# leavesnight/VIEO_SLAM

Measured on AMD Instinct MI355X. Metric: frontend+localBA frames/sec on EuRoC MH05 stereo-VIO; ATE vs ref, higher is better.
Workload: dtype u8 (extract/match) + f64 (pose optimisation)

## Files before the change

include/vieo_hot.h:

```cpp
#ifndef VIEO_HOT_H
#define VIEO_HOT_H

#include <stddef.h>
#include <stdint.h>

#ifdef __cplusplus
extern "C" {
#endif

#define VIEO_OK 0
#define VIEO_E_INVALID (-1)
#define VIEO_E_NO_DEVICE (-2)
#define VIEO_E_HIP (-3)
#define VIEO_E_CAPACITY (-4)
#define VIEO_E_EMPTY (-5)

const char* vieo_last_error(void);
int vieo_device_available(void);
int vieo_set_device(int device);
int vieo_get_device(void);
const char* vieo_version(void);

int vieo_dev_malloc(void** d_ptr, size_t bytes);
int vieo_dev_free(void* d_ptr);
// ... 191 lines not shown
  float Xw[3];
  int32_t octave;
  float angle;
  int32_t flags;
  int32_t reserved[2];
  uint8_t desc[32];
} vieo_last_frame_point;

typedef struct vieo_sbp_camera {
  double Tcw_cur[12], Tcw_last[12];
  float fx, fy, cx, cy;
  float bounds[4];
  float bf, baseline;
  float th, th_far;
  int32_t mono, nlevels;
  float scale[16];
} vieo_sbp_camera;

#define VIEO_SBP_LAST_FRAME 0
#define VIEO_SBP_LOCAL_MAP 1
#define VIEO_SBP_RELOC 2
#define VIEO_SBP_UNCHANGED (-1)
#define VIEO_SBP_ERASED (-2)

int vieo_sbp_project_last_frame(const vieo_last_frame_point* h_points, int n,
                                const vieo_sbp_camera* h_cam, vieo_proj_query* h_queries);
int vieo_search_by_projection(int mode, const vieo_proj_query* h_queries, int nq,
                              const vieo_keypoint* h_keys, const float* h_uright,
                              const uint8_t* h_desc, const uint8_t* h_taken, int n_keys,
                              const float* h_bounds , float nn_ratio, int check_orientation,
                              int32_t* h_assign, int32_t* nmatches);
int vieo_search_by_projection_batch_device(int mode, const vieo_proj_query* d_queries,
                                           const int32_t* d_nq, int q_cap, int n_frames,
                                           const vieo_keypoint* d_keys, const float* d_uright,
                                           const uint8_t* d_desc, const uint8_t* d_taken,
                                           const int32_t* d_counts, int key_cap, int img_first,
                                           int img_step, const float* h_bounds, float nn_ratio,
                                           int check_orientation, int32_t* d_assign,
                                           int32_t* d_nmatches, void* stream);
int vieo_sbp_project_last_frame_batch_device(const vieo_last_frame_point* d_points,
                                             const int32_t* d_n, int p_cap, int n_frames,
                                             const vieo_sbp_camera* d_cams,
                                             vieo_proj_query* d_queries, void* stream);

typedef struct vieo_sbp_rig {
  int32_t n_cams;
  int32_t use_distort;
  vieo_camera cams[4];
  double Tcr[4][12];
  double trc[4][3];
  float bounds[4][4];
} vieo_sbp_rig;

typedef struct vieo_keyframe_point {
  float Xw[3];
  int32_t octave;
  float angle;
  int32_t flags;
  float max_distance, min_distance;
  uint8_t desc[32];
} vieo_keyframe_point;

int vieo_sbp_project_last_frame_rig(const vieo_last_frame_point* h_points, int n, const vieo_sbp_camera* h_cam,
                                    const vieo_sbp_rig* h_rig, vieo_proj_query* h_queries );
int vieo_sbp_project_keyframe(const vieo_keyframe_point* h_points, int n, const vieo_sbp_camera* h_cam,
                              const vieo_sbp_rig* h_rig, float log_scale_factor,
                              vieo_proj_query* h_queries );
int vieo_search_by_projection_rig(int mode, const vieo_proj_query* h_queries, int nq, const vieo_keypoint* h_keys,
                                  const float* h_uright, const uint8_t* h_desc, const uint8_t* h_taken, int n_keys,
                                  const int32_t* h_cam_first , const float* h_bounds, int n_cams,
                                  float nn_ratio, int check_orientation, int32_t* h_assign, int32_t* nmatches);
int vieo_sbp_project_last_frame_rig_batch_device(const vieo_last_frame_point* d_points, const int32_t* d_n,
                                                 int p_cap, int n_frames, const vieo_sbp_camera* d_cams,
                                                 const vieo_sbp_rig* d_rigs, int n_cams,
                                                 vieo_proj_query* d_queries ,
                                                 void* stream);
int vieo_search_by_projection_rig_batch_device(int mode, const vieo_proj_query* d_queries, const int32_t* d_nq,
                                               int q_cap, int n_frames, const vieo_keypoint* d_keys,
                                               const float* d_uright, const uint8_t* d_desc,
                                               const uint8_t* d_taken, const int32_t* d_cam_first, int key_cap,
                                               const float* h_bounds, int n_cams, float nn_ratio,
                                               int check_orientation, int32_t* d_assign, int32_t* d_nmatches,
                                               void* stream);

int vieo_sbp_keep_grid(int on);

int vieo_orb_holds(const vieo_orb* e, const vieo_keypoint* h_keys, int n_keys);
int vieo_orb_resident_keys(const vieo_orb* e);
int vieo_stereo_match_rectified_resident(vieo_orb* left, vieo_orb* right, float baseline, float bf,
                                         float* h_uright, float* h_depth);
int vieo_search_by_projection_last_frame_resident(vieo_orb* frame, const vieo_last_frame_point* h_points, int n_points,
                                                  const vieo_sbp_camera* h_cam, const float* h_uright, float nn_ratio,
                                                  int check_orientation, int32_t* h_assign, int32_t* nmatches);
int vieo_search_by_projection_resident(int mode, vieo_orb* frame, const vieo_proj_query* h_queries, int nq,
                                       const float* h_uright, const uint8_t* h_taken, const float* h_bounds ,
                                       float nn_ratio, int check_orientation, int32_t* h_assign, int32_t* nmatches);


typedef struct vieo_navstate {
  double p[3];
  double q[4];
  double v[3];
  double bg[3], ba[3], dbg[3], dba[3];
} vieo_navstate;


typedef struct vieo_pose_obs {
  float Xw[3];
  float u, v, ur;
  float inv_sigma2;
  int32_t flags;
} vieo_pose_obs;

typedef struct vieo_enc_preint {
  double dt;
  double delx[6];
  double Sigma[36];
} vieo_enc_preint;
typedef struct vieo_pose_enc {
  vieo_enc_preint enc;
  double qRbe[4], pbe[3];
  double p_last[3], q_last[4];
} vieo_pose_enc;

typedef struct vieo_pose_frame {
  vieo_navstate nav;
  double Rcb[9], tcb[3];
  float fx, fy, cx, cy;
  float bf;
  int32_t obs_begin;
  int32_t n_obs;
  int32_t n_cams;
  const vieo_camera* cams;
  const vieo_pose_enc* enc;
} vieo_pose_frame;

#define VIEO_POSE_CAMS_AUTO 0
#define VIEO_POSE_CAMS_RECTIFIED 1
#define VIEO_POSE_CAMS_RIG 2
int vieo_pose_set_camera_mode(int mode);
#define VIEO_POSE_ENC_AUTO 0
#define VIEO_POSE_ENC_NONE 1
#define VIEO_POSE_ENC_ALL 2
int vieo_pose_set_encoder_mode(int mode);

#define VIEO_POSE_OK 0
#define VIEO_POSE_TOO_FEW 1
typedef struct vieo_pose_result {
  vieo_navstate nav;
  int32_t n_inliers;
  int32_t status;
  int32_t lm_iterations;
  int32_t reserved;
} vieo_pose_result;

int vieo_pose_optimization(const vieo_pose_frame* h_frame, const vieo_pose_obs* h_obs,
                           uint8_t* h_outlier, vieo_pose_result* h_result);
int vieo_pose_optimization_batch_device(const vieo_pose_frame* d_frames, int n_frames,
                                        const vieo_pose_obs* d_obs, uint8_t* d_outlier,
                                        vieo_pose_result* d_results, void* stream);

typedef struct vieo_imu_preint {
  double dt;
  double Rij[9];
  double vij[3], pij[3];
  double JgR[9], Jgv[9], Jav[9], Jgp[9], Jap[9];
// ... 218 lines not shown
                                            const void* d_frames, const void* d_results, int frames_are_vio, int key_cap,
                                            int n_frames, void* d_next_frames, uint8_t* d_taken, const int32_t* d_counts,
                                            int img_first, int img_step, uint8_t* d_held, int p_cap, void* stream);
int vieo_track_merge_build_obs_batch_device(const int32_t* d_assign, int32_t* d_mp_ref, int point_offset, int reset, int query_div,
                                            const vieo_last_frame_point* d_same_point, const int32_t* d_query_src, int q_cap,
                                            const float* d_point_xyz, const float* d_point_depth, float close_depth, int p_cap,
                                            const vieo_keypoint* d_keys, const float* d_uright, const int32_t* d_counts,
                                            const int32_t* d_cam_first, int n_cams, int key_cap, int n_frames, int img_first,
                                            int img_step, const float* d_inv_sigma2, vieo_pose_obs* d_obs, int32_t* d_obs_key,
                                            void* d_frames, int frames_are_vio, void* stream);
int vieo_track_build_obs_depth_batch_device(const int32_t* d_mp_ref, const float* d_point_xyz,
                                            const float* d_point_depth, float close_depth, int p_cap,
                                            const vieo_keypoint* d_keys, const float* d_uright,
                                            const int32_t* d_counts, int key_cap, int n_frames,
                                            int img_first, int img_step, const float* d_inv_sigma2,
                                            vieo_pose_obs* d_obs, int32_t* d_obs_key, void* d_frames,
                                            int frames_are_vio, void* stream);
int vieo_track_merge_assign_rig_batch_device(const int32_t* d_assign, int32_t* d_mp_ref, const int32_t* d_counts,
                                             int key_cap, int n_frames, int img_first, int img_step, int point_offset,
                                             int reset, int query_div,
                                             const vieo_last_frame_point* d_same_point ,
                                             const int32_t* d_query_src , int q_cap, void* stream);
int vieo_track_compact_queries_batch_device(const vieo_proj_query* d_queries, const int32_t* d_nq, int q_cap, int n_frames,
                                            vieo_proj_query* d_queries_out, int32_t* d_src, int32_t* d_nq_out, void* stream);
int vieo_track_build_obs_rig_batch_device(const int32_t* d_mp_ref, const float* d_point_xyz,
                                          const float* d_point_depth, float close_depth, int p_cap,
                                          const vieo_keypoint* d_keys, const float* d_uright,
                                          const int32_t* d_counts, const int32_t* d_cam_first, int n_cams, int key_cap,
                                          int n_frames, const float* d_inv_sigma2, vieo_pose_obs* d_obs,
                                          int32_t* d_obs_key, void* d_frames, int frames_are_vio, void* stream);
int vieo_track_mark_held_batch_device(const int32_t* d_mp_ref, const int32_t* d_counts, int key_cap,
                                      int n_frames, int img_first, int img_step, uint8_t* d_held, int p_cap,
                                      void* stream);
void* vieo_orb_stream(vieo_orb* e);

int vieo_orb_tap_plane(vieo_orb* e, int image_index, int level, int which, uint8_t* h_dst,
                       int dst_stride);
int vieo_orb_tap_candidates(vieo_orb* e, int image_index, int level, int32_t* h_dst, int cap);
int vieo_orb_tap_level_keys(vieo_orb* e, int image_index, int level, vieo_keypoint* h_dst,
                            int cap);


typedef struct vieo_frustum_frame {
  float Rcrw[9], tcrw[3];
  float Ow[3];
  int32_t n_cams;
  int32_t use_distort;
  const struct vieo_camera* cams;
  float Tcr[4][12];
  float trc[4][3];
  float bounds[4][4];
  float bf;
  float log_scale_factor;
  int32_t n_levels;
  float viewing_cos_limit;
} vieo_frustum_frame;

typedef struct vieo_frustum_point {
  float Xw[3], normal[3];
  float max_distance, min_distance;
} vieo_frustum_point;

typedef struct vieo_track_info {
  float u[4], v[4], ur[4], viewcos[4];
  int32_t level[4], cam[4];
  int32_t n;
  float track_depth;
} vieo_track_info;

int vieo_is_in_frustum_batch(const vieo_frustum_frame* h_frame, const vieo_frustum_point* h_points, int n_points,
                             vieo_track_info* h_info);
int vieo_track_local_queries_device(const vieo_frustum_frame* h_frame, const vieo_vio_frame* d_frame,
                                    const vieo_vio_result* d_result, const vieo_frustum_point* d_points,
                                    const uint8_t* d_desc, const int32_t* d_alias, const uint8_t* d_held, int held_cap,
                                    int n_points, float th, float th_far, const float* d_scale, vieo_proj_query* d_queries,
                                    float* d_track_depth, int32_t* d_nq, void* stream);

int vieo_track_local_queries_batch_device(const vieo_frustum_frame* h_frame, const vieo_vio_frame* d_frames,
                                          const vieo_vio_result* d_results, int n_frames, const vieo_frustum_point* d_points,
                                          const uint8_t* d_desc, const int32_t* d_alias, const int32_t* d_counts, int p_cap,
                                          const uint8_t* d_held, int held_cap, float th, float th_far, const float* d_scale,
                                          vieo_proj_query* d_queries, float* d_track_depth, size_t depth_stride,
                                          int32_t* d_nq, void* stream);
int vieo_track_local_queries_slot_batch_device(const vieo_frustum_frame* h_frame, const void* d_frames, size_t frame_stride,
                                               const void* d_results, size_t result_stride, int n_frames,
                                               const int32_t* d_pos_slot, const vieo_frustum_point* d_points,
                                               const uint8_t* d_desc, const int32_t* d_alias, const int32_t* d_counts,
                                               int p_cap, const uint8_t* d_held, int held_cap, float th, float th_far,
                                               const float* d_scale, vieo_proj_query* d_queries, float* d_track_depth,
                                               size_t depth_stride, int32_t* d_nq, void* stream);

int vieo_distinctive_descriptors_batch(const uint8_t* h_descriptors, const int32_t* h_first, int n_points,
                                       int32_t* h_best);

int vieo_update_normal_and_depth_batch(const float* h_points , const int32_t* h_first,
                                       const int32_t* h_obs_centre, const float* h_centres, int n_centres,
                                       const int32_t* h_ref_centre, const float* h_ref_scale,
                                       float scale_last_level, int n_points, float* h_normal ,
                                       float* h_max_distance, float* h_min_distance);

typedef struct vieo_fuse_frame {
  vieo_frustum_frame base;
  float scale_factors[16];
  float inv_level_sigma2[16];
  float th_radius;
  int32_t check_viewing_angle;
  int32_t use_bf;
  int32_t reserved;
} vieo_fuse_frame;

typedef struct vieo_fuse_point {
  float Xw[3], normal[3];
  float max_distance, min_distance;
  uint8_t desc[32];
  int32_t skip_mask;
  int32_t reserved;
} vieo_fuse_point;

int vieo_fuse_search(const vieo_fuse_frame* h_frame, const vieo_keypoint* const* h_keys ,
                     const float* const* h_uright ,
                     const uint8_t* const* h_descriptors , const int32_t* n_keys ,
                     const vieo_fuse_point* h_points, int n_points, int32_t* h_best_idx ,
                     int32_t* h_best_dist );

#define VIEO_PREINT_OK 0
#define VIEO_PREINT_EMPTY 1
#define VIEO_PREINT_GAP 2
#define VIEO_PREINT_UNSUPPORTED 3
typedef struct vieo_imu_sample {
  double t;
  double w[3], a[3];
} vieo_imu_sample;
typedef struct vieo_imu_noise {
  double sigma_g[9], sigma_a[9];
  double freq_ref;
  int32_t dt_cov_noise_fixed;
  int32_t reserved;
} vieo_imu_noise;
int vieo_imu_preintegrate_batch(const vieo_imu_noise* noise, const vieo_imu_sample* h_samples,
                                const int32_t* h_first, const double* h_ti, const double* h_tj,
                                const double* h_bg , const double* h_ba , int n,
                                vieo_imu_preint* h_out, double* h_sigma_prv ,
                                int32_t* h_status);

int vieo_imu_preintegrate_batch_device(const vieo_imu_noise* d_noise, const vieo_imu_sample* d_samples,
                                       const int32_t* d_first, const double* d_ti, const double* d_tj,
                                       const double* d_bg, const double* d_ba, int n, vieo_imu_preint* d_out,
                                       double* d_sigma_prv, int32_t* d_status, void* stream);

int vieo_imu_preintegrate_batch_ex(const vieo_imu_noise* noise, const vieo_imu_sample* h_samples,
                                   const int32_t* h_first, const double* h_ti, const double* h_tj,
                                   const double* h_bg , const double* h_ba , int n,
                                   const vieo_imu_preint* h_seed ,
                                   const double* h_seed_sigma_prv , const int32_t* h_breset ,
                                   vieo_imu_preint* h_out, double* h_sigma_prv ,
                                   int32_t* h_status);
int vieo_imu_preintegrate_batch_device_ex(const vieo_imu_noise* d_noise, const vieo_imu_sample* d_samples,
                                          const int32_t* d_first, const double* d_ti, const double* d_tj,
                                          const double* d_bg, const double* d_ba, int n,
                                          const vieo_imu_preint* d_seed, const double* d_seed_sigma_prv,
                                          const int32_t* d_breset, vieo_imu_preint* d_out, double* d_sigma_prv,
                                          int32_t* d_status, void* stream);

typedef struct vieo_tracker vieo_tracker;
typedef struct vieo_tracker_params {
  int32_t width, height;
// ... 354 lines not shown
```

vieo_slam_amd/_lib.py:

```python
import ctypes
import os

_HERE = os.path.dirname(os.path.abspath(__file__))
LIB_PATH = os.environ.get("VIEO_LIB_PATH") or os.path.join(_HERE, "libvieo_hot.so")

VIEO_OK = 0
VIEO_E_INVALID, VIEO_E_NO_DEVICE, VIEO_E_HIP, VIEO_E_CAPACITY, VIEO_E_EMPTY = -1, -2, -3, -4, -5

c_p = ctypes.c_void_p
c_i = ctypes.c_int
c_f = ctypes.c_float
c_sz = ctypes.c_size_t
P = ctypes.POINTER

_SIGS = {
    "vieo_last_error": (ctypes.c_char_p, []),
    "vieo_device_available": (c_i, []),
    "vieo_set_device": (c_i, [c_i]),
    "vieo_pose_set_camera_mode": (c_i, [c_i]),
    "vieo_pose_set_replicas": (c_i, [c_i]),
    "vieo_search_for_triangulation": (c_i, [c_p, c_p, c_i, c_i, c_i, c_i, c_i, c_p, c_p, c_p]),
    "vieo_pose_set_encoder_mode": (c_i, [c_i]),
    "vieo_triangulate_new_points": (c_i, [c_p, c_p, c_p, c_p, c_i, c_f, c_i, c_i, c_p, c_p, c_p, c_p, c_p, c_p]),
    "vieo_create_new_map_points": (c_i, [c_p, c_p, c_p, c_p, c_i, c_i, c_i, c_f, c_i, c_i, c_p, c_p, c_p, c_p, c_p, c_p, c_p]),
    "vieo_is_in_frustum_batch": (c_i, [c_p, c_p, c_i, c_p]),
    "vieo_imu_preintegrate_batch": (c_i, [c_p, c_p, c_p, c_p, c_p, c_p, c_p, c_i, c_p, c_p, c_p]),
    "vieo_imu_preintegrate_batch_ex": (c_i, [c_p] * 7 + [c_i] + [c_p] * 6),
    "vieo_fuse_search": (c_i, [c_p, c_p, c_p, c_p, c_p, c_p, c_i, c_p, c_p]),
    "vieo_distinctive_descriptors_batch": (c_i, [c_p, c_p, c_i, c_p]),
    "vieo_update_normal_and_depth_batch": (c_i, [c_p, c_p, c_p, c_p, c_i, c_p, c_p, ctypes.c_float, c_i, c_p, c_p,
                                                 c_p]),
    "vieo_bundle_adjustment": (c_i, [c_p, c_i, c_i, c_p, c_i, c_p, c_i, c_p, c_i, c_p, c_p, c_p, c_p]),
    "vieo_bundle_adjustment_enc": (c_i, [c_p, c_i, c_i, c_p, c_i, c_p, c_i, c_p, c_i, c_p, c_p, c_p, c_p, c_p]),
    "vieo_local_bundle_adjustment_batch_enc": (c_i, [c_i, c_p, c_p, c_p, c_p, c_p, c_p, c_p, c_p, c_p, c_p, c_p, c_p,
                                                      c_p]),
    "vieo_local_bundle_adjustment_enc": (c_i, [c_p, c_p, c_i, c_p, c_i, c_p, c_i, c_p, c_p, c_p, c_p, c_p, c_p]),
    "vieo_global_bundle_adjustment_vio": (c_i, [c_p, c_i, c_i, c_p, c_i, c_p, c_i, c_p, c_i, c_p, c_i, c_p, c_p, c_p,
                                                c_p]),
    "vieo_global_bundle_adjustment_vio_scale": (c_i, [c_p, c_i, c_i, c_i, c_p, c_i, c_p, c_i, c_p, c_i, c_p, c_i, c_p, c_p,
                                                      c_p, c_p, c_p]),
    "vieo_global_bundle_adjustment_vio_sharded_scale": (c_i, [c_p, c_i, c_i, c_i, c_p, c_i, c_p, c_i, c_p, c_i, c_p, c_i,
                                                              c_p, ctypes.c_size_t, c_p, c_p, c_p, c_p, c_p, c_p]),
    "vieo_track_local_queries_batch_device": (c_i, [c_p, c_p, c_p, c_i, c_p, c_p, c_p, c_p, c_i, c_p, c_i, c_f, c_f, c_p, c_p,
                                                    c_p, c_sz, c_p, c_p]),
    "vieo_pose_optimization_vio_batch_device_ex": (c_i, [c_p, c_i, c_p, c_p, c_p, c_i, c_i, c_p]),
    "vieo_pose_optimization_batch_device_ex": (c_i, [c_p, c_i, c_p, c_p, c_p, c_i, c_p]),
    "vieo_get_device": (c_i, []),
    "vieo_version": (ctypes.c_char_p, []),
    "vieo_dev_malloc": (c_i, [P(c_p), c_sz]),
    "vieo_dev_free": (c_i, [c_p]),
    "vieo_memcpy_h2d": (c_i, [c_p, c_p, c_sz]),
    "vieo_memcpy_d2h": (c_i, [c_p, c_p, c_sz]),
    "vieo_device_synchronize": (c_i, []),
    "vieo_stream_create": (c_i, [P(c_p)]),
    "vieo_stream_destroy": (c_i, [c_p]),
    "vieo_stream_synchronize": (c_i, [c_p]),
    "vieo_stream_wait_event": (c_i, [c_p, c_p]),
    "vieo_host_alloc_pinned": (c_i, [P(c_p), c_sz]),
    "vieo_host_free_pinned": (c_i, [c_p]),
    "vieo_memcpy_h2d_async": (c_i, [c_p, c_p, c_sz, c_p]),
    "vieo_memcpy_d2h_async": (c_i, [c_p, c_p, c_sz, c_p]),
    "vieo_event_create": (c_i, [P(c_p)]),
    "vieo_event_destroy": (c_i, [c_p]),
    "vieo_event_record": (c_i, [c_p, c_p]),
    "vieo_event_elapsed_ms": (c_i, [c_p, c_p, P(c_f)]),
    "vieo_orb_create": (c_i, [P(c_p), c_i, c_f, c_i, c_i, c_i]),
    "vieo_orb_destroy": (None, [c_p]),
    "vieo_orb_levels": (c_i, [c_p]),
    "vieo_orb_scale_factor": (c_f, [c_p]),
    "vieo_orb_scale_factors": (c_i, [c_p, c_p]),
    "vieo_orb_inv_scale_factors": (c_i, [c_p, c_p]),
    "vieo_orb_level_sigma2": (c_i, [c_p, c_p]),
    "vieo_orb_inv_level_sigma2": (c_i, [c_p, c_p]),
    "vieo_orb_features_per_level": (c_i, [c_p, c_p]),
    "vieo_orb_max_keypoints": (c_i, [c_p]),
    "vieo_orb_extract": (c_i, [c_p, c_p, c_i, c_i, c_i, c_p, c_p, c_p, c_i, P(c_i), P(c_i)]),
    "vieo_orb_extract_batch_device": (c_i, [c_p, c_p, c_i, c_i, c_i, c_i, c_sz, c_p, c_p, c_p, c_i, c_p]),
    "vieo_orb_sync": (c_i, [c_p]),
    "vieo_orb_level_size": (c_i, [c_p, c_i, P(c_i), P(c_i)]),
    "vieo_orb_get_level": (c_i, [c_p, c_i, c_i, c_i, c_p, c_i]),
    "vieo_orb_level_device": (c_i, [c_p, c_i, c_i, P(c_p), P(c_i)]),
    "vieo_orb_last_stage_ms": (c_i, [c_p, c_p]),
    "vieo_orb_enable_timing": (c_i, [c_p, c_i]),
    "vieo_orb_timed_steps": (c_i, [c_p]),
    "vieo_orb_stage_ms": (c_i, [c_p, c_i, c_p]),
    "vieo_hamming_knn2": (c_i, [c_p, c_i, c_p, c_i, c_p, c_p]),
    "vieo_stereo_fisheye_match": (c_i, [c_p, c_p, c_p, c_p, c_p, c_i, c_p, c_p, c_p, c_p, c_p, c_p, c_p]),
    "vieo_hamming_knn2_rig_batch_device": (c_i, [c_p, c_p, c_i, c_i, c_i, c_p, c_p, c_p]),
    "vieo_fisheye_create": (c_i, [P(c_p), c_p, c_i, c_i]),
    "vieo_fisheye_destroy": (None, [c_p]),
    "vieo_fisheye_group_capacity": (c_i, [c_p]),
    "vieo_stereo_fisheye_match_batch_device": (c_i, [c_p, c_p, c_p, c_p, c_i] + [c_p] * 12),
    "vieo_stereo_fisheye_match_batch_device_part": (c_i, [c_p, c_p, c_p, c_p, c_i] + [c_p] * 11 + [c_i, c_p]),
    "vieo_track_merge_assign_rig_batch_device": (c_i, [c_p, c_p, c_p, c_i, c_i, c_i, c_i, c_i, c_i, c_i, c_p, c_p, c_i, c_p]),
    "vieo_track_compact_queries_batch_device": (c_i, [c_p, c_p, c_i, c_i, c_p, c_p, c_p, c_p]),
    "vieo_track_build_obs_rig_batch_device": (c_i, [c_p, c_p, c_p, c_f, c_i, c_p, c_p, c_p, c_p, c_i, c_i, c_i, c_p, c_p, c_p,
                                                     c_p, c_i, c_p]),
    "vieo_fisheye_last_walk": (None, [c_p, c_p]),
    "vieo_hamming_knn2_batch_device": (c_i, [c_p, c_p, c_i, c_p, c_i, c_p, c_p, c_p]),
    "vieo_stereo_match_rectified": (c_i, [c_p, c_p, c_p, c_p, c_i, c_p, c_p, c_i, c_f, c_f, c_p, c_p]),
    "vieo_stereo_match_rectified_batch_device": (c_i, [c_p, c_i, c_p, c_p, c_p, c_i, c_f, c_f, c_p, c_p]),
    "vieo_sbp_project_last_frame": (c_i, [c_p, c_i, c_p, c_p]),
    "vieo_sbp_project_last_frame_rig": (c_i, [c_p, c_i, c_p, c_p, c_p]),
    "vieo_sbp_project_keyframe": (c_i, [c_p, c_i, c_p, c_p, c_f, c_p]),
    "vieo_search_by_projection_rig": (c_i, [c_i, c_p, c_i, c_p, c_p, c_p, c_p, c_i, c_p, c_p, c_i, c_f, c_i, c_p, c_p]),
    "vieo_sbp_keep_grid": (c_i, [c_i]),
    "vieo_orb_holds": (c_i, [c_p, c_p, c_i]),
    "vieo_orb_resident_keys": (c_i, [c_p]),
    "vieo_stereo_match_rectified_resident": (c_i, [c_p, c_p, c_f, c_f, c_p, c_p]),
    "vieo_search_by_projection_last_frame_resident": (c_i, [c_p, c_p, c_i, c_p, c_p, c_f, c_i, c_p, c_p]),
    "vieo_search_by_projection_resident": (c_i, [c_i, c_p, c_p, c_i, c_p, c_p, c_p, c_f, c_i, c_p, c_p]),
    "vieo_sbp_project_last_frame_rig_batch_device": (c_i, [c_p, c_p, c_i, c_i, c_p, c_p, c_i, c_p, c_p]),
    "vieo_search_by_projection_rig_batch_device": (c_i, [c_i, c_p, c_p, c_i, c_i, c_p, c_p, c_p, c_p, c_p, c_i, c_p, c_i,
                                                          c_f, c_i, c_p, c_p, c_p]),
    "vieo_search_by_projection": (c_i, [c_i, c_p, c_i, c_p, c_p, c_p, c_p, c_i, c_p, c_f, c_i, c_p, c_p]),
    "vieo_search_by_projection_batch_device": (c_i, [c_i, c_p, c_p, c_i, c_i, c_p, c_p, c_p, c_p, c_p, c_i, c_i, c_i, c_p, c_f, c_i, c_p, c_p, c_p]),
    "vieo_sbp_project_last_frame_batch_device": (c_i, [c_p, c_p, c_i, c_i, c_p, c_p, c_p]),
    "vieo_pose_optimization": (c_i, [c_p, c_p, c_p, c_p]),
    "vieo_pose_optimization_batch_device": (c_i, [c_p, c_i, c_p, c_p, c_p, c_p]),
    "vieo_pose_optimization_vio": (c_i, [c_p, c_p, c_p, c_p]),
    "vieo_pose_optimization_vio_batch_device": (c_i, [c_p, c_i, c_p, c_p, c_p, c_p]),
    "vieo_track_merge_assign_batch_device": (c_i, [c_p, c_p, c_p, c_i, c_i, c_i, c_i, c_i, c_i, c_p]),
    "vieo_track_build_obs_batch_device": (c_i, [c_p, c_p, c_i, c_p, c_p, c_p, c_i, c_i, c_i, c_i, c_p, c_p, c_p, c_p, c_i, c_p]),
    "vieo_track_after_pose_batch_device": (c_i, [c_p, c_p, c_p, c_p, c_p, c_i, c_i, c_i, c_p, c_p, c_p]),
    "vieo_track_build_obs_depth_batch_device": (c_i, [c_p, c_p, c_p, c_f, c_i, c_p, c_p, c_p, c_i, c_i, c_i, c_i, c_p, c_p, c_p,
                                                       c_p, c_i, c_p]),
    "vieo_track_mark_held_batch_device": (c_i, [c_p, c_p, c_i, c_i, c_i, c_i, c_p, c_i, c_p]),
    "vieo_track_after_pose_held_batch_device": (c_i, [c_p, c_p, c_p, c_p, c_p, c_i, c_i, c_i, c_p, c_p, c_p, c_i, c_i, c_p, c_i, c_p]),
    "vieo_track_merge_build_obs_batch_device": (c_i, [c_p, c_p, c_i, c_i, c_i, c_p, c_p, c_i, c_p, c_p, c_f, c_i, c_p, c_p, c_p, c_p, c_i,
                                                       c_i, c_i, c_i, c_i, c_p, c_p, c_p, c_p, c_i, c_p]),
    "vieo_track_local_queries_device": (c_i, [c_p, c_p, c_p, c_p, c_p, c_p, c_p, c_i, c_i, c_f, c_f, c_p, c_p, c_p, c_p, c_p]),
    "vieo_orb_stream": (c_p, [c_p]),
    "vieo_local_bundle_adjustment": (c_i, [c_p, c_p, c_i, c_p, c_i, c_p, c_i, c_p, c_p, c_p, c_p, c_p]),
    "vieo_local_bundle_adjustment_batch": (c_i, [c_i, c_p, c_p, c_p, c_p, c_p, c_p, c_p, c_p, c_p, c_p, c_p,
                                                  c_p]),
    "vieo_local_bundle_adjustment_vio": (c_i, [c_p, c_p, c_i, c_p, c_p, c_i, c_p, c_i, c_p, c_i, c_p, c_p, c_p,
                                                c_p, c_p]),
    "vieo_local_bundle_adjustment_vio_batch": (c_i, [c_i] + [c_p] * 15),
    "vieo_lba_sharded_buffer_doubles": (ctypes.c_size_t, [c_i, c_p]),
    "vieo_lba_enable_timing": (None, [c_i]),
    "vieo_lba_set_stream_priority": (c_i, [c_i]),
    "vieo_lba_kernel_classes": (c_i, []),
    "vieo_lba_kernel_class_name": (ctypes.c_char_p, [c_i]),
    "vieo_lba_kernel_times": (None, [c_p, c_p, c_p]),
    "vieo_lba_sparse_stats": (None, [c_p]),
    "vieo_rccl_available": (c_i, []),
    "vieo_rccl_unique_id": (c_i, [c_p]),
    "vieo_rccl_comm_create": (c_i, [P(c_p), c_p, c_i, c_i]),
    "vieo_rccl_comm_destroy": (c_i, [c_p]),
    "vieo_global_bundle_adjustment_vio_sharded": (c_i, [c_p, c_i, c_i, c_p, c_i, c_p, c_i, c_p, c_i, c_p, c_i, c_p,
                                                        ctypes.c_size_t, c_p, c_p, c_p, c_p, c_p]),
    "vieo_local_bundle_adjustment_vio_sharded": (c_i, [c_i] + [c_p] * 10 + [c_p, ctypes.c_size_t, c_p, c_p] +
                                                 [c_p] * 4),
    "vieo_local_bundle_adjustment_vio_sharded_stop": (c_i, [c_i] + [c_p] * 10 + [c_p, ctypes.c_size_t, c_p, c_p, c_p] +
                                                      [c_p] * 4),
    "vieo_orb_tap_plane": (c_i, [c_p, c_i, c_i, c_i, c_p, c_i]),
    "vieo_orb_tap_candidates": (c_i, [c_p, c_i, c_i, c_p, c_i]),
    "vieo_orb_tap_level_keys": (c_i, [c_p, c_i, c_i, c_p, c_i]),
    "vieo_imu_preintegrate_batch_device": (c_i, [c_p] * 7 + [c_i] + [c_p] * 4),
    "vieo_imu_preintegrate_batch_device_ex": (c_i, [c_p] * 7 + [c_i] + [c_p] * 7),
    "vieo_tracker_create": (c_i, [P(c_p), c_p]),
    "vieo_tracker_create_rig": (c_i, [P(c_p), c_p, c_p]),
    "vieo_tracker_key_capacity": (c_i, [c_p]),
    "vieo_tracker_group_capacity": (c_i, [c_p]),
    "vieo_tracker_image_buffer": (c_i, [c_p, c_i, P(c_p)]),
    "vieo_tracker_destroy": (None, [c_p]),
    "vieo_tracker_image_buffers": (c_i, [c_p, P(c_p), P(c_p)]),
    "vieo_tracker_scale_factors": (c_i, [c_p, c_p]),
    "vieo_track_frame": (c_i, [c_p, c_p, c_p]),
    "vieo_tracker_get_stats": (c_i, [c_p, c_p]),
    "vieo_tracker_reprobe": (c_i, [c_p]),
    "vieo_tracker_get_level": (c_i, [c_p, c_i, c_i, c_i, c_p, c_i]),
    "vieo_tracker_multi_create": (c_i, [P(c_p), c_p, c_i]),
    "vieo_tracker_multi_destroy": (None, [c_p]),
    "vieo_tracker_multi_image_buffer": (c_i, [c_p, c_i, c_i, P(c_p)]),
    "vieo_tracker_multi_reset_slot": (c_i, [c_p, c_i]),
    "vieo_track_frames": (c_i, [c_p, c_i, c_p, c_p, c_p]),
    "vieo_track_local_queries_slot_batch_device": (c_i, [c_p, c_p, c_sz, c_p, c_sz, c_i, c_p, c_p, c_p, c_p, c_p, c_i, c_p, c_i,
                                                         c_f, c_f, c_p, c_p, c_p, c_sz, c_p, c_p]),
    "vieo_search_by_bow": (c_i, [c_p, c_p, c_i, c_f, c_i, c_p, c_p]),
    "vieo_relocalize": (c_i, [c_p, c_p, c_i, c_p, c_i, ctypes.c_uint64, c_p, c_p, c_p, c_p, c_i]),
    "vieo_pnp_create": (c_i, [P(c_p), c_p, c_i, c_p, c_p, c_i, ctypes.c_uint64]),
    "vieo_pnp_destroy": (None, [c_p]),
    "vieo_pnp_get_info": (c_i, [c_p, c_i, c_p]),
    "vieo_pnp_iterate": (c_i, [c_p, c_i, c_i, c_p, c_p, c_p, c_p, c_p, c_p]),
    "vieo_pnp_tap_rows": (c_i, [c_p, c_i, c_p, c_p, c_p, c_p]),
    "vieo_pnp_tap_records": (c_i, [c_p, c_i, c_p, c_p, c_p, c_p]),
    "vieo_pnp_tap_refine": (c_i, [c_p, c_p, c_p, c_i, c_p, c_p, c_p]),
    "vieo_vocabulary_create": (c_i, [P(c_p), c_i, c_i, c_i, c_i, c_p, c_i]),
    "vieo_vocabulary_load": (c_i, [P(c_p), ctypes.c_char_p]),
    "vieo_vocabulary_info": (c_i, [c_p, c_p]),
    "vieo_vocabulary_destroy": (None, [c_p]),
    "vieo_bow_transform": (c_i, [c_p, c_p, c_i, c_i, c_p]),
    "vieo_kfdb_create": (c_i, [P(c_p), c_p]),
    "vieo_kfdb_destroy": (None, [c_p]),
    "vieo_kfdb_clear": (c_i, [c_p]),
    "vieo_kfdb_size": (c_i, [c_p]),
    "vieo_kfdb_add": (c_i, [c_p, ctypes.c_int64, c_p, c_p, c_i]),
    "vieo_kfdb_erase": (c_i, [c_p, ctypes.c_int64]),
    "vieo_kfdb_set_covisible": (c_i, [c_p, ctypes.c_int64, c_p, c_i]),
# ... 80 lines not shown
```

vieo_slam_amd/csrc/mappoint.hip:

```cpp
#include <climits>

#include "ba_device.h"

namespace vieo {

struct FrustumDev {
  vieo_frustum_frame F;
  CamD cams[4];
};

__device__ __forceinline__ void frustum_eval(const vieo_frustum_frame& F, const CamD* cams, const vieo_frustum_point& P,
                                             vieo_track_info& T) {
  memset(&T, 0, sizeof(T));
  const float maxDistance = 1.2f * P.max_distance, minDistance = 0.8f * P.min_distance;
  const float* R = F.Rcrw;
  float Pcr[3];
  for (int r = 0; r < 3; ++r) Pcr[r] = (R[r * 3] * P.Xw[0] + R[r * 3 + 1] * P.Xw[1] + R[r * 3 + 2] * P.Xw[2]) + F.tcrw[r];
  float sum_depth = 0;
  int cnt = 0;
  for (int cami = 0; cami < F.n_cams; ++cami) {
    const float* Tc = F.Tcr[cami];
    float Pc[3], twc[3];
    for (int r = 0; r < 3; ++r)
      Pc[r] = (Tc[r * 4] * Pcr[0] + Tc[r * 4 + 1] * Pcr[1] + Tc[r * 4 + 2] * Pcr[2]) + Tc[r * 4 + 3];
    const float* t = F.trc[cami];
    for (int r = 0; r < 3; ++r) twc[r] = F.Ow[r] + (R[r] * t[0] + R[3 + r] * t[1] + R[6 + r] * t[2]);
    const float PcZ = Pc[2];
    if (PcZ < 0.0f) continue;
    const float invz = 1.0f / PcZ;
    float u, v;
    const CamD& C = cams[cami];
    if (!F.use_distort) {
      const float fx = (float)C.fx, fy = (float)C.fy, cx = (float)C.cx, cy = (float)C.cy;
      const float p0 = Pc[0] * invz, p1 = Pc[1] * invz;
      u = (fx * p0 + 0.f * p1) + cx * 1.f;
      v = (0.f * p0 + fy * p1) + cy * 1.f;
    } else {
      const double Pd[3] = {Pc[0], Pc[1], Pc[2]};
      double uv[2];
      cam_project(C, Pd, uv, nullptr);
      u = (float)uv[0], v = (float)uv[1];
    }
    const float* b = F.bounds[cami];
    if (u < b[0] || u > b[1]) continue;
    if (v < b[2] || v > b[3]) continue;
    const float PO[3] = {P.Xw[0] - twc[0], P.Xw[1] - twc[1], P.Xw[2] - twc[2]};
    const float dist3D = sqrtf(PO[0] * PO[0] + PO[1] * PO[1] + PO[2] * PO[2]);
    if (dist3D < minDistance || dist3D > maxDistance) continue;
    const float viewCos = (PO[0] * P.normal[0] + PO[1] * P.normal[1] + PO[2] * P.normal[2]) / dist3D;
    if (viewCos < F.viewing_cos_limit) continue;
    const float ratio = P.max_distance / dist3D;
    int nscale = (int)ceilf((float)log((double)ratio) / F.log_scale_factor);
    if (nscale < 0)
      nscale = 0;
    else if (nscale >= F.n_levels)
      nscale = F.n_levels - 1;
#pragma unroll
    for (int k = 0; k < 4; ++k)
      if (k == cnt) {
        T.u[k] = u, T.v[k] = v, T.ur[k] = u - F.bf * invz;
        T.level[k] = nscale, T.viewcos[k] = viewCos, T.cam[k] = cami;
      }
    ++cnt;
    sum_depth += dist3D;
  }
  T.n = cnt;
  T.track_depth = cnt ? sum_depth / cnt : -1.f;
}

__global__ void __launch_bounds__(256)
k_in_frustum(const FrustumDev* __restrict__ fd, const vieo_frustum_point* __restrict__ pts, int n,
             vieo_track_info* __restrict__ out) {
  const int m = blockIdx.x * 256 + threadIdx.x;
  if (m >= n) return;
  const vieo_frustum_point P = pts[m];
  vieo_track_info T;
  frustum_eval(fd->F, fd->cams, P, T);
  out[m] = T;
}

__device__ __forceinline__ void track_local_queries_body(vieo_frustum_frame& sF, const FrustumDev& tmpl,
                                                         const vieo_pose_frame* __restrict__ frame,
                                                         const vieo_pose_result* __restrict__ result,
                                                         const vieo_frustum_point* __restrict__ pts, const uint8_t* __restrict__ desc,
                                                         const int32_t* __restrict__ alias, const uint8_t* __restrict__ held,
                                                         int held_cap, int n, float th, float th_far, const float* __restrict__ scale,
                                                         vieo_proj_query* __restrict__ queries, float* __restrict__ track_depth,
                                                         int32_t* __restrict__ nq) {
  if (threadIdx.x == 0) {
    sF = tmpl.F;
    const vieo_navstate& nav = result->status == 0 ? result->nav : frame->nav;
    double Rwb[9];
    {
      const double qw = nav.q[0], qx = nav.q[1], qy = nav.q[2], qz = nav.q[3];
      const double tx = 2 * qx, ty = 2 * qy, tz = 2 * qz;
      const double twx = tx * qw, twy = ty * qw, twz = tz * qw, txx = tx * qx, txy = ty * qx, txz = tz * qx;
      const double tyy = ty * qy, tyz = tz * qy, tzz = tz * qz;
      Rwb[0] = 1 - (tyy + tzz), Rwb[1] = txy - twz, Rwb[2] = txz + twy;
      Rwb[3] = txy + twz, Rwb[4] = 1 - (txx + tzz), Rwb[5] = tyz - twx;
      Rwb[6] = txz - twy, Rwb[7] = tyz + twx, Rwb[8] = 1 - (txx + tyy);
    }
    const double* Rcb = frame->Rcb;
    double Rcw[9], tcw[3];
    for (int r = 0; r < 3; ++r)
      for (int c = 0; c < 3; ++c) Rcw[r * 3 + c] = Rcb[r * 3] * Rwb[c * 3] + Rcb[r * 3 + 1] * Rwb[c * 3 + 1] + Rcb[r * 3 + 2] * Rwb[c * 3 + 2];
    for (int r = 0; r < 3; ++r)
      tcw[r] = frame->tcb[r] - (Rcw[r * 3] * nav.p[0] + Rcw[r * 3 + 1] * nav.p[1] + Rcw[r * 3 + 2] * nav.p[2]);
    for (int i = 0; i < 9; ++i) sF.Rcrw[i] = (float)Rcw[i];
    for (int r = 0; r < 3; ++r) {
      sF.tcrw[r] = (float)tcw[r];
      sF.Ow[r] = (float)(-(Rcw[r] * tcw[0] + Rcw[3 + r] * tcw[1] + Rcw[6 + r] * tcw[2]));
    }
    if (blockIdx.x == 0) *nq = n * tmpl.F.n_cams;
  }
  __syncthreads();
  const int m = blockIdx.x * 256 + threadIdx.x;
  if (m >= n) return;
  const vieo_frustum_point P = pts[m];
  vieo_track_info T;
  frustum_eval(sF, tmpl.cams, P, T);
  const int S = sF.n_cams;
  int cnt = T.n;
  if (th_far > 0.f && T.track_depth > th_far) cnt = 0;
  if (alias && alias[m] >= 0 && alias[m] < held_cap && held[alias[m]]) cnt = 0;
  track_depth[m] = T.track_depth;
  const uint4* d = (const uint4*)(desc + (size_t)m * 32);
  const uint4 d0 = d[0], d1 = d[1];
  for (int k = 0; k < S; ++k) {
    vieo_proj_query q;
    memset(&q, 0, sizeof(q));
    if (k < cnt) {
      float u = 0, v = 0, ur = 0, vc = 0;
      int lvl = 0, cam = 0;
#pragma unroll
      for (int j = 0; j < 4; ++j)
        if (j == k) u = T.u[j], v = T.v[j], ur = T.ur[j], vc = T.viewcos[j], lvl = T.level[j], cam = T.cam[j];
      float r = vc > 0.998f ? 2.5f : 4.0f;
      if (th != 1.0f) r = r * th;
      q.u = u, q.v = v, q.ur = ur;
      q.radius = r * scale[lvl];
      q.level_min = lvl - 1, q.level_max = lvl, q.angle = 0.f;
      q.flags = 3 | (cam << 8);
      ((uint4*)q.desc)[0] = d0, ((uint4*)q.desc)[1] = d1;
    }
    queries[(size_t)m * S + k] = q;
  }
}

__global__ void __launch_bounds__(256)
k_track_local_queries(FrustumDev tmpl, const vieo_vio_frame* __restrict__ frame, const vieo_vio_result* __restrict__ result,
                      const vieo_frustum_point* __restrict__ pts, const uint8_t* __restrict__ desc,
                      const int32_t* __restrict__ alias, const uint8_t* __restrict__ held, int held_cap, int n, float th, float th_far,
                      const float* __restrict__ scale, vieo_proj_query* __restrict__ queries,
                      float* __restrict__ track_depth, int32_t* __restrict__ nq, int p_cap, const int32_t* __restrict__ counts,
                      size_t depth_stride) {
  __shared__ vieo_frustum_frame sF;
  {
    const size_t f = blockIdx.y;
    frame += f, result += f, nq += f;
    pts += f * p_cap, desc += f * p_cap * 32;
    if (alias) alias += f * p_cap, held += f * held_cap;
    queries += f * p_cap * tmpl.F.n_cams, track_depth += f * depth_stride;
    if (counts) n = min(counts[f], p_cap);
    if (blockIdx.x * 256 >= (unsigned)max(n, 1)) return;
  }
  track_local_queries_body(sF, tmpl, &frame->base, &result->base, pts, desc, alias, held, held_cap, n, th, th_far, scale,
                           queries, track_depth, nq);
}

__global__ void __launch_bounds__(256)
k_track_local_queries_slot(FrustumDev tmpl, const uint8_t* __restrict__ frames, size_t frame_stride,
                           const uint8_t* __restrict__ results, size_t result_stride, const int32_t* __restrict__ pos_slot,
                           const vieo_frustum_point* __restrict__ pts, const uint8_t* __restrict__ desc,
                           const int32_t* __restrict__ alias, const uint8_t* __restrict__ held, int held_cap, float th,
                           float th_far, const float* __restrict__ scale, vieo_proj_query* __restrict__ queries,
                           float* __restrict__ track_depth, int32_t* __restrict__ nq, int p_cap,
                           const int32_t* __restrict__ counts, size_t depth_stride) {
  __shared__ vieo_frustum_frame sF;
  const size_t f = blockIdx.y, s = (size_t)pos_slot[f];
  const int n = min(counts[f], p_cap);
  if (blockIdx.x * 256 >= (unsigned)max(n, 1)) return;
  track_local_queries_body(sF, tmpl, (const vieo_pose_frame*)(frames + f * frame_stride),
                           (const vieo_pose_result*)(results + f * result_stride), pts + s * p_cap, desc + s * p_cap * 32,
                           alias ? alias + f * p_cap : nullptr, alias ? held + f * held_cap : held, held_cap, n, th, th_far,
                           scale, queries + f * p_cap * tmpl.F.n_cams, track_depth + f * depth_stride, nq + f);
}

static const int kMaxObsLds = 128;
static const int kMaxObsPerPoint = 65535;

__device__ __forceinline__ int hamming256(const uint4& a0, const uint4& a1, const uint4& b0, const uint4& b1) {
  return __popc(a0.x ^ b0.x) + __popc(a0.y ^ b0.y) + __popc(a0.z ^ b0.z) + __popc(a0.w ^ b0.w) +
         __popc(a1.x ^ b1.x) + __popc(a1.y ^ b1.y) + __popc(a1.z ^ b1.z) + __popc(a1.w ^ b1.w);
}

__global__ void __launch_bounds__(256)
k_distinctive(const uint8_t* __restrict__ desc, const int32_t* __restrict__ first, int n, int32_t* __restrict__ best,
              int cap, int slice) {
  extern __shared__ unsigned short s_all[];
  const int wv = __builtin_amdgcn_readfirstlane((int)(threadIdx.x >> 6)), lane = threadIdx.x & 63;
  const int p = blockIdx.x * 4 + wv;
  if (p >= n) return;
  const int N = first[p + 1] - first[p];
  if (N <= 0) {
    if (lane == 0) best[p] = -1;
    return;
  }
  unsigned short* sd = s_all + (size_t)wv * slice;
  const uint8_t* D = desc + (size_t)first[p] * 32;
  const int k = (int)(0.5 * (N - 1));
  int bm = INT_MAX, bi = INT_MAX;
  if (N <= cap) {
    for (int i = lane; i < N; i += 64) {
      const uint4 a0 = ((const uint4*)(D + (size_t)i * 32))[0], a1 = ((const uint4*)(D + (size_t)i * 32))[1];
      for (int j = 0; j < N; ++j) {
        const uint4 b0 = ((const uint4*)(D + (size_t)j * 32))[0], b1 = ((const uint4*)(D + (size_t)j * 32))[1];
        sd[i * N + j] = (unsigned short)hamming256(a0, a1, b0, b1);
      }
    }
    for (int i = lane; i < N; i += 64) {
      int lo = 0, hi = 256;
      while (lo < hi) {
        const int mid = (lo + hi) >> 1;
        int c = 0;
        for (int j = 0; j < N; ++j) c += sd[i * N + j] <= mid;
        if (c >= k + 1)
          hi = mid;
        else
          lo = mid + 1;
      }
      if (lo < bm) bm = lo, bi = i;
    }
  } else {
    unsigned short* h = sd + lane * 258;
    for (int i = lane; i < N; i += 64) {
      for (int v = 0; v < 257; ++v) h[v] = 0;
      const uint4 a0 = ((const uint4*)(D + (size_t)i * 32))[0], a1 = ((const uint4*)(D + (size_t)i * 32))[1];
      for (int j = 0; j < N; ++j) {
        const uint4 b0 = ((const uint4*)(D + (size_t)j * 32))[0], b1 = ((const uint4*)(D + (size_t)j * 32))[1];
        h[hamming256(a0, a1, b0, b1)]++;
      }
      int c = 0, v = 0;
      for (; v < 257; ++v) {
        c += h[v];
        if (c >= k + 1) break;
      }
      if (v < bm) bm = v, bi = i;
    }
  }
#pragma unroll
  for (int o = 32; o > 0; o >>= 1) {
    const int m2 = __shfl_xor(bm, o), i2 = __shfl_xor(bi, o);
// ... 57 lines not shown
  }
  int rc = require_device();
  if (rc != VIEO_OK) return rc;
  if (n_points == 0) return VIEO_OK;
  FrustumDev fd;
  memset(&fd, 0, sizeof(fd));
  fd.F = *h_frame;
  fd.F.cams = nullptr;
  for (int c = 0; c < h_frame->n_cams; ++c)
    if (!cam_from_abi(h_frame->cams[c], fd.cams[c])) {
      set_error("isInFrustum: camera %d has an unknown model or coefficient count", c);
      return VIEO_E_INVALID;
    }
  MpScratch& S = g_mp;
  ENS(S.a, sizeof(fd));
  ENS(S.b, (size_t)n_points * sizeof(vieo_frustum_point));
  ENS(S.c, (size_t)n_points * sizeof(vieo_track_info));
  H2D(S.a, &fd, sizeof(fd));
  H2D(S.b, h_points, (size_t)n_points * sizeof(vieo_frustum_point));
  hipLaunchKernelGGL(k_in_frustum, dim3((n_points + 255) / 256), dim3(256), 0, 0, S.a.as<FrustumDev>(),
                     S.b.as<vieo_frustum_point>(), n_points, S.c.as<vieo_track_info>());
  VIEO_HIP_CHECK(hipGetLastError());
  VIEO_HIP_CHECK(hipMemcpy(h_info, S.c.p, (size_t)n_points * sizeof(vieo_track_info), hipMemcpyDeviceToHost));
  return VIEO_OK;
}

int vieo_track_local_queries_device(const vieo_frustum_frame* h_frame, const vieo_vio_frame* d_frame,
                                    const vieo_vio_result* d_result, const vieo_frustum_point* d_points,
                                    const uint8_t* d_desc, const int32_t* d_alias, const uint8_t* d_held, int held_cap,
                                    int n_points, float th, float th_far, const float* d_scale, vieo_proj_query* d_queries,
                                    float* d_track_depth, int32_t* d_nq, void* stream) {
  if (!h_frame || !d_frame || !d_result || n_points < 0 || !d_scale || !d_nq ||
      (n_points > 0 && (!d_points || !d_desc || !d_queries || !d_track_depth)) || (d_alias && (!d_held || held_cap <= 0)))
    return VIEO_E_INVALID;
  if (h_frame->n_cams < 1 || h_frame->n_cams > 4 || !h_frame->cams || h_frame->n_levels <= 0) {
    set_error("SearchLocalPoints: n_cams = %d (1..4) with cameras and n_levels > 0", h_frame->n_cams);
    return VIEO_E_INVALID;
  }
  int rc = require_device();
  if (rc != VIEO_OK) return rc;
  FrustumDev fd;
  memset(&fd, 0, sizeof(fd));
  fd.F = *h_frame;
  fd.F.cams = nullptr;
  for (int c = 0; c < h_frame->n_cams; ++c)
    if (!cam_from_abi(h_frame->cams[c], fd.cams[c])) {
      set_error("SearchLocalPoints: camera %d has an unknown model or coefficient count", c);
      return VIEO_E_INVALID;
    }
  hipLaunchKernelGGL(k_track_local_queries, dim3(std::max(1, (n_points + 255) / 256)), dim3(256), 0, (hipStream_t)stream, fd,
                     d_frame, d_result, d_points, d_desc, d_alias, d_held, held_cap, n_points, th, th_far, d_scale, d_queries,
                     d_track_depth, d_nq, n_points, (const int32_t*)nullptr, (size_t)0);
  VIEO_HIP_CHECK(hipGetLastError());
  return VIEO_OK;
}

int vieo_track_local_queries_batch_device(const vieo_frustum_frame* h_frame, const vieo_vio_frame* d_frames,
                                          const vieo_vio_result* d_results, int n_frames, const vieo_frustum_point* d_points,
                                          const uint8_t* d_desc, const int32_t* d_alias, const int32_t* d_counts, int p_cap,
                                          const uint8_t* d_held, int held_cap, float th, float th_far, const float* d_scale,
                                          vieo_proj_query* d_queries, float* d_track_depth, size_t depth_stride,
                                          int32_t* d_nq, void* stream) {
  if (!h_frame || !d_frames || !d_results || n_frames <= 0 || p_cap <= 0 || !d_counts || !d_scale || !d_nq || !d_points ||
      !d_desc || !d_queries || !d_track_depth || (d_alias && (!d_held || held_cap <= 0)))
    return VIEO_E_INVALID;
  if (h_frame->n_cams < 1 || h_frame->n_cams > 4 || !h_frame->cams || h_frame->n_levels <= 0) {
    set_error("SearchLocalPoints: n_cams = %d (1..4) with cameras and n_levels > 0", h_frame->n_cams);
    return VIEO_E_INVALID;
  }
  int rc = require_device();
  if (rc != VIEO_OK) return rc;
  FrustumDev fd;
  memset(&fd, 0, sizeof(fd));
  fd.F = *h_frame;
  fd.F.cams = nullptr;
  for (int c = 0; c < h_frame->n_cams; ++c)
    if (!cam_from_abi(h_frame->cams[c], fd.cams[c])) {
      set_error("SearchLocalPoints: camera %d has an unknown model or coefficient count", c);
      return VIEO_E_INVALID;
    }
  hipLaunchKernelGGL(k_track_local_queries, dim3((p_cap + 255) / 256, n_frames), dim3(256), 0, (hipStream_t)stream, fd, d_frames,
                     d_results, d_points, d_desc, d_alias, d_held, held_cap, 0, th, th_far, d_scale, d_queries, d_track_depth,
                     d_nq, p_cap, d_counts, depth_stride);
  VIEO_HIP_CHECK(hipGetLastError());
  return VIEO_OK;
}

int vieo_track_local_queries_slot_batch_device(const vieo_frustum_frame* h_frame, const void* d_frames, size_t frame_stride,
                                               const void* d_results, size_t result_stride, int n_frames,
                                               const int32_t* d_pos_slot, const vieo_frustum_point* d_points,
                                               const uint8_t* d_desc, const int32_t* d_alias, const int32_t* d_counts,
                                               int p_cap, const uint8_t* d_held, int held_cap, float th, float th_far,
                                               const float* d_scale, vieo_proj_query* d_queries, float* d_track_depth,
                                               size_t depth_stride, int32_t* d_nq, void* stream) {
  if (!h_frame || !d_frames || !d_results || n_frames <= 0 || p_cap <= 0 || !d_pos_slot || !d_counts || !d_scale || !d_nq ||
      !d_points || !d_desc || !d_queries || !d_track_depth || (d_alias && (!d_held || held_cap <= 0)) ||
      frame_stride < sizeof(vieo_pose_frame) || result_stride < sizeof(vieo_pose_result))
    return VIEO_E_INVALID;
  if (h_frame->n_cams < 1 || h_frame->n_cams > 4 || !h_frame->cams || h_frame->n_levels <= 0) {
    set_error("SearchLocalPoints: n_cams = %d (1..4) with cameras and n_levels > 0", h_frame->n_cams);
    return VIEO_E_INVALID;
  }
  int rc = require_device();
  if (rc != VIEO_OK) return rc;
  FrustumDev fd;
  memset(&fd, 0, sizeof(fd));
  fd.F = *h_frame;
  fd.F.cams = nullptr;
  for (int c = 0; c < h_frame->n_cams; ++c)
    if (!cam_from_abi(h_frame->cams[c], fd.cams[c])) {
      set_error("SearchLocalPoints: camera %d has an unknown model or coefficient count", c);
      return VIEO_E_INVALID;
    }
  hipLaunchKernelGGL(k_track_local_queries_slot, dim3((p_cap + 255) / 256, n_frames), dim3(256), 0, (hipStream_t)stream, fd,
                     (const uint8_t*)d_frames, frame_stride, (const uint8_t*)d_results, result_stride, d_pos_slot, d_points,
                     d_desc, d_alias, d_held, held_cap, th, th_far, d_scale, d_queries, d_track_depth, d_nq, p_cap, d_counts,
                     depth_stride);
  VIEO_HIP_CHECK(hipGetLastError());
  return VIEO_OK;
}

int vieo_distinctive_descriptors_batch(const uint8_t* h_descriptors, const int32_t* h_first, int n_points,
                                       int32_t* h_best) {
  if (n_points < 0 || (n_points > 0 && (!h_first || !h_best))) return VIEO_E_INVALID;
  int rc = require_device();
  if (rc != VIEO_OK) return rc;
  if (n_points == 0) return VIEO_OK;
  const int total = h_first[n_points];
  if (total < 0 || (total > 0 && !h_descriptors)) return VIEO_E_INVALID;
  int n_max = 0;
  for (int p = 0; p < n_points; ++p) {
    const int N = h_first[p + 1] - h_first[p];
    if (N < 0) return VIEO_E_INVALID;
    if (N > kMaxObsPerPoint) {
      set_error("ComputeDistinctiveDescriptors: point %d has %d observations (limit %d)", p, N, kMaxObsPerPoint);
      return VIEO_E_CAPACITY;
    }
    n_max = std::max(n_max, N);
  }
  MpScratch& S = g_mp;
  ENS(S.a, (size_t)total * 32);
  ENS(S.b, (size_t)(n_points + 1) * 4);
  ENS(S.c, (size_t)n_points * 4);
  H2D(S.a, h_descriptors, (size_t)total * 32);
  H2D(S.b, h_first, (size_t)(n_points + 1) * 4);
  const int cap = std::min(n_max, kMaxObsLds);
  const int slice = std::max(cap * cap, n_max > kMaxObsLds ? 64 * 258 : 0);
  const size_t lds = (size_t)4 * slice * sizeof(unsigned short);
  VIEO_HIP_CHECK(hipFuncSetAttribute((const void*)k_distinctive, hipFuncAttributeMaxDynamicSharedMemorySize, (int)lds));
  hipLaunchKernelGGL(k_distinctive, dim3((n_points + 3) / 4), dim3(256), lds, 0, S.a.as<uint8_t>(),
                     S.b.as<int32_t>(), n_points, S.c.as<int32_t>(), cap, slice);
  VIEO_HIP_CHECK(hipGetLastError());
  VIEO_HIP_CHECK(hipMemcpy(h_best, S.c.p, (size_t)n_points * 4, hipMemcpyDeviceToHost));
  return VIEO_OK;
}

int vieo_update_normal_and_depth_batch(const float* h_points, const int32_t* h_first, const int32_t* h_obs_centre,
                                       const float* h_centres, int n_centres, const int32_t* h_ref_centre,
                                       const float* h_ref_scale, float scale_last_level, int n_points,
                                       float* h_normal, float* h_max_distance, float* h_min_distance) {
  if (n_points < 0 || n_centres < 0 ||
      (n_points > 0 && (!h_points || !h_first || !h_ref_centre || !h_ref_scale || !h_normal || !h_max_distance ||
                        !h_min_distance)))
    return VIEO_E_INVALID;
  int rc = require_device();
  if (rc != VIEO_OK) return rc;
// ... 38 lines not shown
```

vieo_slam_amd/csrc/proj_search.hip:

```cpp
#include <climits>
#include <cstring>

#include "ba_device.h"
#include "orb_internal.h"
#include "wave_ops.h"

namespace vieo {

static const int kGridRows = 48, kGridCols = 64;
static const int kThHigh = 100, kHistoLen = 30;
static const int kCandCap = 128;
static const int kMaxKeys = 8192;
static const int kMaxCams = 4;

__device__ __forceinline__ void rig_uv(const vieo_sbp_rig& R, int cam, const double* x3Dc, float invzc, float* u, float* v) {
  const vieo_camera& c = R.cams[cam];
  if (R.use_distort) {
    CamD d;
    cam_from_abi(c, d);
    double uv[2];
    cam_project(d, x3Dc, uv, nullptr);
    *u = (float)uv[0], *v = (float)uv[1];
  } else {
    const float xc = (float)x3Dc[0], yc = (float)x3Dc[1];
    const float pnx = xc * invzc, pny = yc * invzc;
    *u = c.fx * pnx + 0.f * pny + c.cx * 1.f;
    *v = 0.f * pnx + c.fy * pny + c.cy * 1.f;
  }
}

__global__ void __launch_bounds__(256)
k_sbp_project(const vieo_last_frame_point* __restrict__ pts, const int* __restrict__ n_pts,
              int p_cap, const vieo_sbp_camera* __restrict__ cams, const vieo_sbp_rig* __restrict__ rigs,
              int n_cams, vieo_proj_query* __restrict__ out) {
  const int f = blockIdx.y;
  const int t = blockIdx.x * blockDim.x + threadIdx.x;
  if (t >= p_cap * n_cams) return;
  const int i = t / n_cams, camj = t - i * n_cams;
  vieo_proj_query q;
  memset(&q, 0, sizeof(q));
  vieo_proj_query* dst = out + (size_t)f * p_cap * n_cams + t;
  if (i >= n_pts[f]) {
    *dst = q;
    return;
  }
  const vieo_sbp_camera& C = cams[f];
  const vieo_last_frame_point p = pts[(size_t)f * p_cap + i];
  bool ok = p.flags & 1;
  const double* Tc = C.Tcw_cur;
  const double* Tl = C.Tcw_last;
  const double r6 = Tl[8] * Tc[0] + Tl[9] * Tc[1] + Tl[10] * Tc[2];
  const double r7 = Tl[8] * Tc[4] + Tl[9] * Tc[5] + Tl[10] * Tc[6];
  const double r8 = Tl[8] * Tc[8] + Tl[9] * Tc[9] + Tl[10] * Tc[10];
  const double tz = Tl[11] - (r6 * Tc[3] + r7 * Tc[7] + r8 * Tc[11]);
  const bool bForward = tz > C.baseline && !C.mono;
  const bool bBackward = -tz > C.baseline && !C.mono;
  const double X = p.Xw[0], Y = p.Xw[1], Z = p.Xw[2];
  double x3[3];
  x3[0] = Tc[0] * X + Tc[1] * Y + Tc[2] * Z + Tc[3];
  x3[1] = Tc[4] * X + Tc[5] * Y + Tc[6] * Z + Tc[7];
  x3[2] = Tc[8] * X + Tc[9] * Y + Tc[10] * Z + Tc[11];
  if (C.th_far > 0 && x3[2] > C.th_far) ok = false;
  float u, v, invzc;
  const float* bnd = C.bounds;
  if (!rigs) {
    const float xc = (float)x3[0], yc = (float)x3[1];
    invzc = (float)(1.0 / x3[2]);
    const float pnx = xc * invzc, pny = yc * invzc;
    u = C.fx * pnx + 0.f * pny + C.cx * 1.f;
    v = 0.f * pnx + C.fy * pny + C.cy * 1.f;
  } else {
    const vieo_sbp_rig& R = rigs[f];
    const double* T = R.Tcr[camj];
    double xc[3];
    for (int r = 0; r < 3; ++r) xc[r] = T[r * 4] * x3[0] + T[r * 4 + 1] * x3[1] + T[r * 4 + 2] * x3[2] + T[r * 4 + 3];
    invzc = (float)(1.0 / xc[2]);
    u = v = 0.f;
    if (!(invzc < 0)) rig_uv(R, camj, xc, invzc, &u, &v);
    bnd = R.bounds[camj];
  }
  if (invzc < 0) ok = false;
  if (!(u >= bnd[0] && u < bnd[1] && v >= bnd[2] && v < bnd[3])) ok = false;
  if (ok) {
    const int oct = p.octave;
    q.u = u, q.v = v;
    q.ur = u - C.bf * invzc;
    q.radius = C.th * C.scale[oct];
    if (bForward)
      q.level_min = 0, q.level_max = oct;
    else if (bBackward)
      q.level_min = oct, q.level_max = -1;
    else
      q.level_min = oct - 1, q.level_max = oct + 1;
    q.angle = p.angle;
    q.flags = 1 | (p.flags & 2) | (camj << 8);
    for (int k = 0; k < 32; k++) q.desc[k] = p.desc[k];
  }
  *dst = q;
}

__global__ void __launch_bounds__(256)
k_sbp_project_kf(const vieo_keyframe_point* __restrict__ pts, int n, const vieo_sbp_camera* __restrict__ cam,
                 const vieo_sbp_rig* __restrict__ rig, int n_cams, float log_scale_factor,
                 vieo_proj_query* __restrict__ out) {
  const int t = blockIdx.x * blockDim.x + threadIdx.x;
  if (t >= n * n_cams) return;
  const int i = t / n_cams, cami = t - i * n_cams;
  vieo_proj_query q;
  memset(&q, 0, sizeof(q));
  const vieo_sbp_camera& C = *cam;
  const vieo_keyframe_point p = pts[i];
  bool ok = p.flags & 1;
  const double* Tc = C.Tcw_cur;
  const double Xw[3] = {p.Xw[0], p.Xw[1], p.Xw[2]};
  double x3[3];
  for (int r = 0; r < 3; ++r) x3[r] = Tc[r * 4] * Xw[0] + Tc[r * 4 + 1] * Xw[1] + Tc[r * 4 + 2] * Xw[2] + Tc[r * 4 + 3];
  if (C.th_far > 0 && x3[2] > C.th_far) ok = false;
  double tw[3];
  for (int r = 0; r < 3; ++r) tw[r] = Tc[r] * (Tc[3] * -1.0) + Tc[4 + r] * (Tc[7] * -1.0) + Tc[8 + r] * (Tc[11] * -1.0);
  double Pc[3], twc[3];
  float u, v, invzc;
  const float* bnd = C.bounds;
  if (!rig) {
    for (int r = 0; r < 3; ++r) Pc[r] = x3[r], twc[r] = tw[r];
    invzc = (float)(1.0 / Pc[2]);
    const float xc = (float)Pc[0], yc = (float)Pc[1];
    const float pnx = xc * invzc, pny = yc * invzc;
    u = C.fx * pnx + 0.f * pny + C.cx * 1.f;
    v = 0.f * pnx + C.fy * pny + C.cy * 1.f;
  } else {
    const double* T = rig->Tcr[cami];
    for (int r = 0; r < 3; ++r) Pc[r] = T[r * 4] * x3[0] + T[r * 4 + 1] * x3[1] + T[r * 4 + 2] * x3[2] + T[r * 4 + 3];
    const double* tr = rig->trc[cami];
    for (int r = 0; r < 3; ++r) twc[r] = tw[r] + (Tc[r] * tr[0] + Tc[4 + r] * tr[1] + Tc[8 + r] * tr[2]);
    invzc = (float)(1.0 / Pc[2]);
    rig_uv(*rig, cami, Pc, invzc, &u, &v);
    bnd = rig->bounds[cami];
  }
  if (!(u >= bnd[0] && u < bnd[1] && v >= bnd[2] && v < bnd[3])) ok = false;
  const double PO[3] = {Xw[0] - twc[0], Xw[1] - twc[1], Xw[2] - twc[2]};
  const float dist3D = (float)sqrt(PO[0] * PO[0] + PO[1] * PO[1] + PO[2] * PO[2]);
  if (dist3D < 0.8f * p.min_distance || dist3D > 1.2f * p.max_distance) ok = false;
  if (ok) {
    const float ratio = p.max_distance / dist3D;
    int lvl = (int)ceilf((float)log((double)ratio) / log_scale_factor);
    if (lvl < 0)
      lvl = 0;
    else if (lvl >= C.nlevels)
      lvl = C.nlevels - 1;
    q.u = u, q.v = v, q.ur = u - C.bf * invzc;
    q.radius = C.th * C.scale[lvl];
    q.level_min = lvl - 1, q.level_max = lvl + 1;
    q.angle = p.angle;
    q.flags = 1 | (p.flags & 2) | (cami << 8);
    for (int k = 0; k < 32; k++) q.desc[k] = p.desc[k];
  }
  out[t] = q;
}

struct SbpArgs {
  int mode;
  const vieo_proj_query* queries;
  const int* nq;
  int q_cap;
  const vieo_keypoint* keys;
  const float* uright;
  const uint8_t* desc;
  const uint8_t* taken;
  const int* counts;
  int key_cap, img_first, img_step;
  int n_cams;
  const int* cam_first;
  float bounds[kMaxCams][4];
  float nn_ratio;
  int check_ori;
  const int* cell_start;
  const float4* cell_rec;
  const float* cell_ang;
  unsigned* pool;
  int* cursor;
  int2* qrec;
  int pool_cap, pool_lds;
  int* assign;
  int* nmatches;
  int* claim;
  int* need_seq;
  int max_rounds;
};

__device__ __forceinline__ int hamming32q(const uint4 a0, const uint4 a1, const uint8_t* b) {
  const uint4 b0 = ((const uint4*)b)[0], b1 = ((const uint4*)b)[1];
  return __popc(a0.x ^ b0.x) + __popc(a0.y ^ b0.y) + __popc(a0.z ^ b0.z) + __popc(a0.w ^ b0.w) +
         __popc(a1.x ^ b1.x) + __popc(a1.y ^ b1.y) + __popc(a1.z ^ b1.z) + __popc(a1.w ^ b1.w);
}

static const int kGridCells = kGridCols * kGridRows;

__device__ __forceinline__ void cam_range(const SbpArgs& A, int f, int cam, int* k0, int* k1) {
  if (A.cam_first) {
    const int* cf = A.cam_first + (size_t)f * (A.n_cams + 1);
    *k0 = min(cf[cam], A.key_cap), *k1 = min(cf[cam + 1], A.key_cap);
  } else {
    *k0 = 0, *k1 = min(A.counts[2 * (A.img_first + f * A.img_step)], A.key_cap);
  }
}

template <int NT>
__global__ void __launch_bounds__(NT) k_sbp_grid(SbpArgs A, int* __restrict__ cell_start,
                                                  float4* __restrict__ cell_rec,
                                                  float* __restrict__ cell_ang) {
  __shared__ int s_cnt[kGridCells + 1];
  __shared__ int s_cur[kGridCells];
  __shared__ unsigned short s_list[kMaxKeys];
  __shared__ int s_part[16];
  const int f = blockIdx.x / A.n_cams, cam = blockIdx.x - f * A.n_cams, tid = threadIdx.x;
  const int img = A.img_first + f * A.img_step;
  int k0, k1;
  cam_range(A, f, cam, &k0, &k1);
  const int N = k1 - k0;
  const vieo_keypoint* K = A.keys + (size_t)img * A.key_cap + k0;
  const float minx = A.bounds[cam][0], miny = A.bounds[cam][2];
  const float winv = (float)kGridCols / (A.bounds[cam][1] - minx), hinv = (float)kGridRows / (A.bounds[cam][3] - miny);
  for (int c = tid; c <= kGridCells; c += NT) s_cnt[c] = 0;
  __syncthreads();
  for (int j = tid; j < N; j += NT) {
    const int posX = (int)roundf((K[j].x - minx) * winv), posY = (int)roundf((K[j].y - miny) * hinv);
    if (posX >= 0 && posX < kGridCols && posY >= 0 && posY < kGridRows) atomicAdd(&s_cnt[posX * kGridRows + posY], 1);
  }
  __syncthreads();
  const int per = kGridCells / NT, c0 = tid * per;
  int sum = 0;
  for (int c = c0; c < c0 + per; c++) sum += s_cnt[c];
  int inc = sum;
  for (int o = 1; o < 64; o <<= 1) {
    const int t = __shfl_up(inc, o);
    if ((tid & 63) >= o) inc += t;
  }
  if ((tid & 63) == 63) s_part[tid >> 6] = inc;
  __syncthreads();
  int acc = inc - sum;
  for (int w = 0; w < (tid >> 6); w++) acc += s_part[w];
  int* cs = cell_start + (size_t)blockIdx.x * (kGridCells + 1);
  for (int c = c0; c < c0 + per; c++) {
    const int v = s_cnt[c];
    cs[c] = acc, s_cur[c] = acc;
    acc += v;
  }
  if (tid == NT - 1) {
    cs[kGridCells] = acc;
    if (cam == 0) A.cursor[f] = 0;
  }
  __syncthreads();
  for (int j = tid; j < N; j += NT) {
    const int posX = (int)roundf((K[j].x - minx) * winv), posY = (int)roundf((K[j].y - miny) * hinv);
    if (posX >= 0 && posX < kGridCols && posY >= 0 && posY < kGridRows)
      s_list[atomicAdd(&s_cur[posX * kGridRows + posY], 1)] = (unsigned short)j;
  }
  __syncthreads();
  for (int c = c0; c < c0 + per; c++) {
    const int e = s_cur[c], b = e - s_cnt[c];
    for (int i = b + 1; i < e; i++) {
      const unsigned short v = s_list[i];
      int k = i - 1;
      while (k >= b && s_list[k] > v) s_list[k + 1] = s_list[k], k--;
      s_list[k + 1] = v;
    }
  }
  __syncthreads();
  const int n_in = s_cur[kGridCells - 1];
  const float* uright = A.uright + (size_t)f * A.key_cap + k0;
  float4* rec = cell_rec + (size_t)f * A.key_cap + k0;
  float* ang = cell_ang + (size_t)f * A.key_cap + k0;
  for (int i = tid; i < n_in; i += NT) {
    const int j = s_list[i];
    const vieo_keypoint k = K[j];
    rec[i] = make_float4(k.x, k.y, uright[j], __int_as_float((j + k0) | (k.octave << 16)));
    ang[i] = k.angle;
  }
}

__device__ __forceinline__ int wave_excl_scan_i(int v, int lane, int* total) {
  int x = v;
  x += __builtin_amdgcn_update_dpp(0, x, 0x111, 0xF, 0xF, true);
  x += __builtin_amdgcn_update_dpp(0, x, 0x112, 0xF, 0xF, true);
  x += __builtin_amdgcn_update_dpp(0, x, 0x114, 0xF, 0xF, true);
  x += __builtin_amdgcn_update_dpp(0, x, 0x118, 0xF, 0xF, true);
  x += VIEO_DPP(0, x, VIEO_DPP_ROW_BCAST15, 0xA);
  x += VIEO_DPP(0, x, VIEO_DPP_ROW_BCAST31, 0xC);
  (void)lane;
  *total = __builtin_amdgcn_readlane(x, 63);
  return x - v;
}

static const int kSbpBlocks = 8;
static const int kSbpBlocksFew = 128;

__global__ void __launch_bounds__(256) k_sbp_candidates(SbpArgs A) {
  extern __shared__ unsigned short s_cs[];
  constexpr int kBigCap = 1024;
  __shared__ int s_big[kBigCap];
  __shared__ int s_nbig;
  if (threadIdx.x == 0) s_nbig = 0;
  const int f = blockIdx.y, wave = __builtin_amdgcn_readfirstlane((int)(threadIdx.x >> 6)), lane = threadIdx.x & 63;
  const int nq = min(A.nq[f], A.q_cap);
  const int img = A.img_first + f * A.img_step;
  {
    const int* cs = A.cell_start + (size_t)f * A.n_cams * (kGridCells + 1);
    for (int i = threadIdx.x; i < A.n_cams * (kGridCells + 1); i += 256) s_cs[i] = (unsigned short)cs[i];
  }
  const int n_blocks = gridDim.x;
  for (int q = nq + blockIdx.x * 256 + threadIdx.x; q < A.q_cap; q += n_blocks * 256)
    A.qrec[(size_t)f * A.q_cap + q] = make_int2(0, 0);
  __syncthreads();
  const uint8_t* D = A.desc + (size_t)img * A.key_cap * 32;
  const float4* rec_f = A.cell_rec + (size_t)f * A.key_cap;
  const float* ang_f = A.cell_ang + (size_t)f * A.key_cap;
  unsigned* pool = A.pool + (size_t)f * A.pool_cap;
  const float factor = 1.0f / kHistoLen;
  const uint4* QQ = (const uint4*)(A.queries + (size_t)f * A.q_cap);
  int slab_cur = 0, slab_end = 0;
  auto reserve = [&](int total) -> int {
    if (slab_cur + total > slab_end) {
      int b = 0;
      if (lane == 0) b = atomicAdd(&A.cursor[f], kCandCap);
      slab_cur = __builtin_amdgcn_readfirstlane(b), slab_end = slab_cur + kCandCap;
    }
    const int base = slab_cur;
    slab_cur += total;
    return base;
  };
  {
    const int g = lane >> 4, gl = lane & 15;
    const int stride4 = n_blocks * 16;
    uint4 n0 = {0, 0, 0, 0}, n1 = n0, n2 = n0, n3 = n0;
    {
      const int qf = (blockIdx.x * 4 + wave) * 4 + g;
      if (qf < nq) n0 = QQ[4 * (size_t)qf], n1 = QQ[4 * (size_t)qf + 1], n2 = QQ[4 * (size_t)qf + 2], n3 = QQ[4 * (size_t)qf + 3];
    }
    for (int q0 = (blockIdx.x * 4 + wave) * 4; q0 < nq; q0 += stride4) {
      const int qg = q0 + g;
      const bool qin = qg < nq;
      const uint4 g0 = n0, g1 = n1, e0 = n2, e1 = n3;
      {
        const int qn = qg + stride4;
        if (qn < nq) n0 = QQ[4 * (size_t)qn], n1 = QQ[4 * (size_t)qn + 1], n2 = QQ[4 * (size_t)qn + 2], n3 = QQ[4 * (size_t)qn + 3];
      }
      const float x = __uint_as_float(g0.x), y = __uint_as_float(g0.y), q_ur = __uint_as_float(g0.z);
      const float r = __uint_as_float(g0.w);
      const int minlevel = (int)g1.x, maxlevel = (int)g1.y, flags = (int)g1.w;
      const float q_angle = __uint_as_float(g1.z);
      const int cam = (flags >> 8) & 15;
      bool valid = qin && (flags & 1) && cam < A.n_cams;
      const int camc = valid ? cam : 0;
      const float minx = A.bounds[camc][0], miny = A.bounds[camc][2];
      const float winv = (float)kGridCols / (A.bounds[camc][1] - minx), hinv = (float)kGridRows / (A.bounds[camc][3] - miny);
      int k0 = 0;
      if (A.cam_first) k0 = min(A.cam_first[(size_t)f * (A.n_cams + 1) + camc], A.key_cap);
      const unsigned short* cs = s_cs + camc * (kGridCells + 1);
      const int min_cellx = max(0, (int)floorf((x - minx - r) * winv));
      const int max_cellx = min(kGridCols - 1, (int)ceilf((x - minx + r) * winv));
      const int min_celly = max(0, (int)floorf((y - miny - r) * hinv));
      const int max_celly = min(kGridRows - 1, (int)ceilf((y - miny + r) * hinv));
      const bool empty = min_cellx >= kGridCols || max_cellx < 0 || min_celly >= kGridRows || max_celly < 0 ||
                         min_cellx > max_cellx || min_celly > max_celly;
      const int nx = max_cellx - min_cellx + 1;
      const bool narrow = valid && !empty && nx <= 16;
      int seg_s = 0, seg_l = 0;
      if (narrow && gl < nx) {
        const int col = (min_cellx + gl) * kGridRows;
        seg_s = cs[col + min_celly];
        seg_l = cs[col + max_celly + 1] - seg_s;
      }
      int inc = seg_l;
      inc += __builtin_amdgcn_update_dpp(0, inc, 0x111, 0xF, 0xF, true);
// ... 54 lines not shown
          base = __builtin_amdgcn_readfirstlane(bb);
        } else
          base = reserve(tot_all);
        over = base + tot_all > A.pool_cap;
      }
      int wpos = base + off_g;
#pragma unroll
      for (int it = 0; it < 4; it++) {
        if (it >= nit) continue;
        const unsigned gm = (unsigned)((m_it[it] >> sh) & 0xFFFFull);
        if (((gm >> gl) & 1u) && !over) {
          const int packed = pk_it[it], sl = sl_it[it];
          const int j = packed & 0xFFFF, oct = packed >> 16;
          const int d = hamming32q(e0, e1, D + (size_t)j * 32);
          float rot = q_angle - (ang_f + k0)[sl];
          if (rot < 0.0f) rot += 360.0f;
          int bin = (int)roundf(rot * factor);
          if (bin == kHistoLen) bin = 0;
          pool[wpos + __popc(gm & ((1u << gl) - 1u))] =
              (unsigned)j | ((unsigned)d << 13) | ((unsigned)(oct & 15) << 22) | ((unsigned)(bin & 31) << 26);
        }
        wpos += tg[it];
      }
      if (gl == 0 && qin) {
        int2* out = A.qrec + (size_t)f * A.q_cap + qg;
        if (!valid || empty)
          *out = make_int2(0, 0);
        else if (small)
          *out = tot_g == 0 ? make_int2(0, 0) : (over ? make_int2(0, -1) : make_int2(base + off_g, tot_g | ((flags & 2) ? 1 << 16 : 0)));
        else {
          const int k = atomicAdd(&s_nbig, 1);
          if (k < kBigCap) s_big[k] = qg;
        }
      }
    }
  }
  __syncthreads();
  const int nbig = s_nbig;
  const bool listed = nbig <= kBigCap;
  const int own0 = (blockIdx.x * 4 + wave) * 4;
  for (int k2 = listed ? wave : 0;; k2 += listed ? 4 : 1) {
    int q;
    if (listed) {
      if (k2 >= nbig) break;
      q = s_big[k2];
    } else {
      const int q0 = own0 + (k2 >> 2) * (n_blocks * 16);
      if (q0 >= nq) break;
      q = q0 + (k2 & 3);
      if (q >= nq) continue;
    }
    const uint4 h0 = QQ[4 * (size_t)q], h1 = QQ[4 * (size_t)q + 1];
    const uint4 d0 = QQ[4 * (size_t)q + 2], d1 = QQ[4 * (size_t)q + 3];
    const float x = __uint_as_float(h0.x), y = __uint_as_float(h0.y), q_ur = __uint_as_float(h0.z);
    const float r = __uint_as_float(h0.w);
    const int minlevel = (int)h1.x, maxlevel = (int)h1.y, flags = (int)h1.w;
    const float q_angle = __uint_as_float(h1.z);
    int2* out = A.qrec + (size_t)f * A.q_cap + q;
    const int cam = (flags >> 8) & 15;
    if (!(flags & 1) || cam >= A.n_cams) continue;
    const float minx = A.bounds[cam][0], miny = A.bounds[cam][2];
    const float winv = (float)kGridCols / (A.bounds[cam][1] - minx), hinv = (float)kGridRows / (A.bounds[cam][3] - miny);
    int k0 = 0;
    if (A.cam_first) k0 = min(A.cam_first[(size_t)f * (A.n_cams + 1) + cam], A.key_cap);
    const float4* rec = rec_f + k0;
    const float* ang = ang_f + k0;
    const unsigned short* cs = s_cs + cam * (kGridCells + 1);
    const int min_cellx = max(0, (int)floorf((x - minx - r) * winv));
    const int max_cellx = min(kGridCols - 1, (int)ceilf((x - minx + r) * winv));
    const int min_celly = max(0, (int)floorf((y - miny - r) * hinv));
    const int max_celly = min(kGridRows - 1, (int)ceilf((y - miny + r) * hinv));
    if (min_cellx >= kGridCols || max_cellx < 0 || min_celly >= kGridRows || max_celly < 0 ||
        min_cellx > max_cellx || min_celly > max_celly)
      continue;
    const bool bchecklevel = (minlevel > 0) || (maxlevel >= 0);
    const int nx = max_cellx - min_cellx + 1;
    int seg_s = 0, seg_l = 0;
    if (lane < nx) {
      const int col = (min_cellx + lane) * kGridRows;
      seg_s = cs[col + min_celly];
      seg_l = cs[col + max_celly + 1] - seg_s;
    }
    int n_ent;
    const int seg_o = wave_excl_scan_i(seg_l, lane, &n_ent);
    if (nx <= 16 && n_ent <= 64) continue;
    auto test = [&](int t, int* slot, int* packed) -> bool {
      int sl = -1;
      for (int i = 0; i < nx; i++) {
        const int o = __builtin_amdgcn_readlane(seg_o, i), l = __builtin_amdgcn_readlane(seg_l, i), s0 = __builtin_amdgcn_readlane(seg_s, i);
        if (t >= o && t < o + l) sl = s0 + (t - o);
      }
      *slot = sl;
      if (t >= n_ent || sl < 0) return false;
      const float4 k = rec[sl];
      const int pk = __float_as_int(k.w), oct = pk >> 16;
      *packed = pk;
      if (bchecklevel) {
        if (oct < minlevel) return false;
        if (maxlevel >= 0 && oct > maxlevel) return false;
      }
      if (!(fabsf(k.x - x) < r && fabsf(k.y - y) < r)) return false;
      if (A.mode != VIEO_SBP_RELOC && k.z > 0 && fabsf(q_ur - k.z) > r) return false;
      return true;
    };
    auto encode = [&](int slot, int packed) -> unsigned {
      const int j = packed & 0xFFFF, oct = packed >> 16;
      const int d = hamming32q(d0, d1, D + (size_t)j * 32);
      float rot = q_angle - ang[slot];
      if (rot < 0.0f) rot += 360.0f;
      int bin = (int)roundf(rot * factor);
      if (bin == kHistoLen) bin = 0;
      return (unsigned)j | ((unsigned)d << 13) | ((unsigned)(oct & 15) << 22) | ((unsigned)(bin & 31) << 26);
    };
    const int obs_bit = (flags & 2) ? 1 << 16 : 0;
    if (n_ent <= 64) {
      int slot, packed = 0;
      const bool pass = test(lane, &slot, &packed);
      const unsigned long long m = __ballot(pass);
      const int total = __popcll(m);
      if (total == 0) {
        if (lane == 0) *out = make_int2(0, 0);
        continue;
      }
      const int base = reserve(total);
      if (base + total > A.pool_cap) {
        if (lane == 0) *out = make_int2(0, -1);
        continue;
      }
      if (pass) pool[base + __popcll(m & ((1ull << lane) - 1ull))] = encode(slot, packed);
      if (lane == 0) *out = make_int2(base, total | obs_bit);
      continue;
    }
    int total = 0;
    for (int t0 = 0; t0 < n_ent; t0 += 64) {
      int slot, packed = 0;
      total += __popcll(__ballot(test(t0 + lane, &slot, &packed)));
    }
    if (total == 0 || total > kCandCap) {
      if (lane == 0) *out = make_int2(0, total == 0 ? 0 : -1);
      continue;
    }
    const int base = reserve(total);
    if (base + total > A.pool_cap) {
      if (lane == 0) *out = make_int2(0, -1);
      continue;
    }
    int w = base;
    for (int t0 = 0; t0 < n_ent; t0 += 64) {
      int slot, packed = 0;
      const bool pass = test(t0 + lane, &slot, &packed);
      const unsigned long long m = __ballot(pass);
      if (pass) pool[w + __popcll(m & ((1ull << lane) - 1ull))] = encode(slot, packed);
      w += __popcll(m);
    }
    if (lane == 0) *out = make_int2(base, total | obs_bit);
  }
}

__global__ void __launch_bounds__(1024) k_sbp_assign_par(SbpArgs A) {
  extern __shared__ unsigned s_pool[];
  int* s_min0 = (int*)(s_pool + A.pool_lds);
  int* s_min1 = s_min0 + A.key_cap;
  unsigned* s_bins = (unsigned*)(s_min1 + A.key_cap);
  uint8_t* s_taken = (uint8_t*)(s_bins + A.key_cap);
  __shared__ int s_hist[kHistoLen];
  __shared__ int s_changed[2], s_nm, s_overflow;
  const int f = blockIdx.x, tid = threadIdx.x;
// ... 40 lines not shown
      else if (key < b1)
        b1 = key, c1 = c;
    }
    if (b0 == 0xFFFFFFFFu) return -1;
    const int bestDist = b0 >> 8, bestLevel = (c0 >> 22) & 15;
    if (bestDist > (reloc ? (int)A.nn_ratio : kThHigh)) return -1;
    if (A.mode == VIEO_SBP_LOCAL_MAP && b1 != 0xFFFFFFFFu) {
      const int bestDist2 = b1 >> 8, bestLevel2 = (c1 >> 22) & 15;
      if (bestLevel == bestLevel2 && (float)bestDist > A.nn_ratio * (float)bestDist2) return -1;
    }
    *word = c0;
    *blocker = reloc || (ny >> 16);
    return (int)(c0 & 0x1FFF);
  };
  bool settled = false;
  for (int round = 0; round < A.max_rounds; round++) {
    int* prev = (round & 1) ? s_min1 : s_min0;
    int* cur = (round & 1) ? s_min0 : s_min1;
    int changed = 0;
    for (int q = tid; q < nq; q += 1024) {
      unsigned w;
      int blk = 0;
      const int k = eval(q, prev, &w, &blk);
      if (k != claim[q]) claim[q] = k, changed = 1;
      if (k >= 0 && blk) atomicMin(&cur[k], q);
    }
    if (changed) s_changed[round & 1] = 1;
    __syncthreads();
    const int any = s_changed[round & 1];
    if (tid == 0) s_changed[(round + 1) & 1] = 0;
    for (int i = tid; i < N; i += 1024) prev[i] = INT_MAX;
    __syncthreads();
    if (!any) {
      settled = true;
      const bool ori = A.mode != VIEO_SBP_LOCAL_MAP && A.check_ori;
      int* s_asg = prev;
      for (int i = tid; i < N; i += 1024) s_asg[i] = -1;
      __syncthreads();
      int nm = 0;
      for (int q = tid; q < nq; q += 1024) {
        const int k = claim[q];
        if (k < 0) continue;
        unsigned w = 0;
        int blk = 0;
        (void)eval(q, cur, &w, &blk);
        atomicMax(&s_asg[k], q);
        nm++;
        if (ori) {
          const int bin = (w >> 26) & 31;
          atomicOr(&s_bins[k], 1u << bin);
          atomicAdd(&s_hist[bin], 1);
        }
      }
      if (nm) atomicAdd(&s_nm, nm);
      __syncthreads();
      int nmatches = s_nm;
      unsigned losers = 0;
      if (ori) {
        int max1 = 0, max2 = 0, max3 = 0, ind1 = -1, ind2 = -1, ind3 = -1;
        for (int i = 0; i < kHistoLen; i++) {
          const int sv = s_hist[i];
          if (sv > max1) {
            max3 = max2, max2 = max1, max1 = sv;
            ind3 = ind2, ind2 = ind1, ind1 = i;
          } else if (sv > max2) {
            max3 = max2, max2 = sv;
            ind3 = ind2, ind2 = i;
          } else if (sv > max3) {
            max3 = sv, ind3 = i;
          }
        }
        if (max2 < 0.1f * (float)max1) {
          ind2 = -1, ind3 = -1;
        } else if (max3 < 0.1f * (float)max1) {
          ind3 = -1;
        }
        losers = (1u << kHistoLen) - 1u;
        if (ind1 >= 0) losers &= ~(1u << ind1);
        if (ind2 >= 0) losers &= ~(1u << ind2);
        if (ind3 >= 0) losers &= ~(1u << ind3);
        for (int i = 0; i < kHistoLen; i++)
          if (i != ind1 && i != ind2 && i != ind3) nmatches -= s_hist[i];
      }
      for (int k = tid; k < N; k += 1024) assign[k] = (s_bins[k] & losers) ? VIEO_SBP_ERASED : s_asg[k];
      if (tid == 0) A.nmatches[f] = s_overflow ? -1 : nmatches;
      break;
    }
  }
  if (tid == 0) A.need_seq[f] = settled ? 0 : 1;
}

__device__ __forceinline__ void seq_sync() {
  __builtin_amdgcn_fence(__ATOMIC_ACQ_REL, "workgroup");
  __builtin_amdgcn_wave_barrier();
}
__device__ void sbp_assign_seq(const SbpArgs& A, int f, unsigned* s_pool, int lane) {
  unsigned* s_bins = s_pool + A.pool_lds;
  uint8_t* s_state = (uint8_t*)(s_bins + A.key_cap);
  __shared__ int s_hist[kHistoLen];
  int N;
  {
    int k0;
    cam_range(A, f, A.n_cams - 1, &k0, &N);
  }
  const int nq = min(A.nq[f], A.q_cap);
  int* assign = A.assign + (size_t)f * A.key_cap;
  const uint8_t* taken = A.taken ? A.taken + (size_t)f * A.key_cap : nullptr;
  const unsigned* pool = A.pool + (size_t)f * A.pool_cap;
  const int2* qrec = A.qrec + (size_t)f * A.q_cap;
  const int n_lds = min(min(A.cursor[f], A.pool_cap), A.pool_lds);
  for (int i0 = lane; i0 < n_lds; i0 += 16 * 64) {
    unsigned v[16];
#pragma unroll
    for (int u = 0; u < 16; u++) v[u] = i0 + 64 * u < n_lds ? pool[i0 + 64 * u] : 0u;
#pragma unroll
    for (int u = 0; u < 16; u++)
      if (i0 + 64 * u < n_lds) s_pool[i0 + 64 * u] = v[u];
  }
  for (int i0 = lane; i0 < N; i0 += 8 * 64) {
    uint8_t t[8];
#pragma unroll
    for (int u = 0; u < 8; u++) t[u] = (taken && i0 + 64 * u < N) ? taken[i0 + 64 * u] : (uint8_t)0;
#pragma unroll
    for (int u = 0; u < 8; u++)
      if (i0 + 64 * u < N) {
        assign[i0 + 64 * u] = VIEO_SBP_UNCHANGED;
        s_state[i0 + 64 * u] = t[u] ? 3 : 0;
        s_bins[i0 + 64 * u] = 0u;
      }
  }
  if (lane < kHistoLen) s_hist[lane] = 0;
  seq_sync();
  int nmatches = 0, overflow = 0;
  const bool ori = A.mode != VIEO_SBP_LOCAL_MAP && A.check_ori;
  for (int q0 = 0; q0 < nq; q0 += 64) {
    const int2 mine = q0 + lane < nq ? qrec[q0 + lane] : make_int2(0, 0);
    const int qn = min(64, nq - q0);
    for (int qq = 0; qq < qn; qq++) {
      const int off = __builtin_amdgcn_readlane(mine.x, qq), ny = __builtin_amdgcn_readlane(mine.y, qq);
      if (ny == 0) continue;
      if (ny < 0) {
        overflow = 1;
        continue;
      }
      const int n = ny & 0xFFFF, q = q0 + qq;
      unsigned b0 = 0xFFFFFFFFu, b1 = 0xFFFFFFFFu;
      unsigned cand2[2] = {0u, 0u};
#pragma unroll
      for (int h = 0; h < 2; h++) {
        const int pos = lane + 64 * h;
        if (pos < n) {
          const unsigned c = off + pos < n_lds ? s_pool[off + pos] : pool[off + pos];
          cand2[h] = c;
          const int idx = c & 0x1FFF, d = (c >> 13) & 0x1FF;
          const int st = s_state[idx];
          if (A.mode == VIEO_SBP_RELOC ? !(st & 1) : !((st & 1) && (st & 2))) {
            const unsigned key = ((unsigned)d << 8) | (unsigned)pos;
            if (key < b0)
              b1 = b0, b0 = key;
            else
              b1 = key;
          }
        }
      }
      const unsigned m0 = wave_min_u32(b0);
      const unsigned m1 = wave_min_u32(b0 == m0 ? b1 : b0);
      b0 = m0, b1 = m1;
      unsigned c0 = 0, c1 = 0;
      if (b0 != 0xFFFFFFFFu) c0 = (unsigned)__builtin_amdgcn_readlane((int)((b0 & 64u) ? cand2[1] : cand2[0]), (int)(b0 & 63u));
      if (b1 != 0xFFFFFFFFu) c1 = (unsigned)__builtin_amdgcn_readlane((int)((b1 & 64u) ? cand2[1] : cand2[0]), (int)(b1 & 63u));
      if (b0 == 0xFFFFFFFFu) continue;
      const int bestDist = b0 >> 8;
      const int bestIdx = c0 & 0x1FFF, bestLevel = (c0 >> 22) & 15;
      if (bestDist > (A.mode == VIEO_SBP_RELOC ? (int)A.nn_ratio : kThHigh)) continue;
      if (A.mode == VIEO_SBP_LOCAL_MAP && b1 != 0xFFFFFFFFu) {
        const int bestDist2 = b1 >> 8;
        const int bestLevel2 = (c1 >> 22) & 15;
        if (bestLevel == bestLevel2 && (float)bestDist > A.nn_ratio * (float)bestDist2) continue;
      }
      if (lane == 0) {
        s_state[bestIdx] = 1 | ((ny >> 16) ? 2 : 0);
        assign[bestIdx] = q;
      }
      nmatches++;
      if (ori) {
        const int bin = (c0 >> 26) & 31;
        if (lane == 0) {
          s_bins[bestIdx] |= 1u << bin;
          s_hist[bin]++;
        }
      }
      seq_sync();
    }
  }
  if (ori) {
    seq_sync();
    int max1 = 0, max2 = 0, max3 = 0, ind1 = -1, ind2 = -1, ind3 = -1;
    for (int i = 0; i < kHistoLen; i++) {
      const int s = s_hist[i];
      if (s > max1) {
        max3 = max2, max2 = max1, max1 = s;
        ind3 = ind2, ind2 = ind1, ind1 = i;
      } else if (s > max2) {
        max3 = max2, max2 = s;
        ind3 = ind2, ind2 = i;
      } else if (s > max3) {
        max3 = s, ind3 = i;
      }
    }
    if (max2 < 0.1f * (float)max1) {
      ind2 = -1, ind3 = -1;
    } else if (max3 < 0.1f * (float)max1) {
      ind3 = -1;
    }
    unsigned losers = (1u << kHistoLen) - 1u;
    if (ind1 >= 0) losers &= ~(1u << ind1);
    if (ind2 >= 0) losers &= ~(1u << ind2);
    if (ind3 >= 0) losers &= ~(1u << ind3);
    for (int k = lane; k < N; k += 64)
      if (s_bins[k] & losers) assign[k] = VIEO_SBP_ERASED;
    for (int i = 0; i < kHistoLen; i++)
      if (i != ind1 && i != ind2 && i != ind3) nmatches -= s_hist[i];
  }
  if (lane == 0) A.nmatches[f] = overflow ? -1 : nmatches;
}

static const int kFinStride = 48, kCamQ = 4096;
__global__ void __launch_bounds__(1024) k_sbp_assign_cam(SbpArgs A, int cam_cap, int* __restrict__ fin, unsigned* __restrict__ kbins,
                                                        int lds_bytes) {
  extern __shared__ unsigned s_pool[];
  unsigned* s_best = s_pool + A.pool_lds;
  unsigned* s_second = s_best + kCamQ;
  int* s_min0 = (int*)(s_second + kCamQ);
  int* s_min1 = s_min0 + cam_cap;
  unsigned* s_bins = (unsigned*)(s_min1 + cam_cap);
  unsigned short* s_qof = (unsigned short*)(s_bins + cam_cap);
  unsigned short* s_qid = s_qof + A.pool_lds;
  unsigned short* s_qstart = s_qid + kCamQ;
  uint8_t* s_taken = (uint8_t*)(s_qstart + kCamQ);
  __shared__ int s_hist[kHistoLen];
  __shared__ int s_changed[2], s_nm, s_overflow, s_fill, s_nql, s_last;
  const int f = blockIdx.x, cam = blockIdx.y, tid = threadIdx.x;
  int k0, k1;
  cam_range(A, f, cam, &k0, &k1);
  const int Nc = k1 - k0;
  const int nq = min(A.nq[f], A.q_cap);
  int* assign = A.assign + (size_t)f * A.key_cap;
  const uint8_t* taken = A.taken ? A.taken + (size_t)f * A.key_cap : nullptr;
  const unsigned* pool = A.pool + (size_t)f * A.pool_cap;
  const int2* qrec = A.qrec + (size_t)f * A.q_cap;
  int* F = fin + (size_t)f * kFinStride;
  unsigned* KB = kbins + (size_t)f * A.key_cap;
  const bool ori = A.mode != VIEO_SBP_LOCAL_MAP && A.check_ori;
  const bool reloc = A.mode == VIEO_SBP_RELOC, second = A.mode == VIEO_SBP_LOCAL_MAP;
  constexpr int kOwn = kCamQ / 1024;
  bool settled = false;
  if (Nc <= cam_cap && nq < 65536) {
    for (int i = tid; i < Nc; i += 1024) {
      s_taken[i] = taken ? taken[k0 + i] : (uint8_t)0;
      s_min0[i] = INT_MAX, s_min1[i] = INT_MAX, s_bins[i] = 0u;
    }
    for (int i = tid; i < kCamQ; i += 1024) s_best[i] = 0xFFFFFFFFu, s_second[i] = 0xFFFFFFFFu;
    if (tid < kHistoLen) s_hist[tid] = 0;
    if (tid == 0) s_nm = 0, s_overflow = 0, s_fill = 0, s_nql = 0, s_changed[0] = s_changed[1] = 0;
    __syncthreads();
// ... 30 lines not shown
    }
    __syncthreads();
    int lq[kOwn], cny[kOwn], cl[kOwn];
    unsigned wl[kOwn];
    {
      const int nql = min(s_nql, kCamQ);
#pragma unroll
      for (int j = 0; j < kOwn; j++) {
        const int me = tid + 1024 * j;
        cl[j] = -1, wl[j] = 0, lq[j] = me < nql ? me : -1, cny[j] = 0;
        if (me < nql) cny[j] = (int)s_second[me], s_second[me] = 0xFFFFFFFFu;
      }
    }
    __syncthreads();
    const int n_pairs = s_fill;
    const bool fits = n_pairs <= A.pool_lds && s_nql <= kCamQ && n_pairs < 65536;
    for (int round = 0; fits && round < A.max_rounds; round++) {
      int* prev = (round & 1) ? s_min1 : s_min0;
      int* cur = (round & 1) ? s_min0 : s_min1;
      for (int p = tid; p < n_pairs; p += 1024) {
        const unsigned c = s_pool[p];
        const int me = s_qof[p], idx = (int)(c & 0x1FFF) - k0;
        const int q = s_qid[me], pos = p - s_qstart[me];
        if (!(s_taken[idx] || prev[idx] < q)) atomicMin(&s_best[me], (((c >> 13) & 0x1FFu) << 8) | (unsigned)pos);
      }
      __syncthreads();
      if (second) {
        for (int p = tid; p < n_pairs; p += 1024) {
          const unsigned c = s_pool[p];
          const int me = s_qof[p], idx = (int)(c & 0x1FFF) - k0;
          const int q = s_qid[me], pos = p - s_qstart[me];
          const unsigned key = (((c >> 13) & 0x1FFu) << 8) | (unsigned)pos;
          if (key != s_best[me] && !(s_taken[idx] || prev[idx] < q)) atomicMin(&s_second[me], key);
        }
        __syncthreads();
      }
      int changed = 0;
#pragma unroll
      for (int j = 0; j < kOwn; j++)
        if (lq[j] >= 0) {
          const int me = lq[j], q = s_qid[me], ny = cny[j];
          const unsigned b0 = s_best[me], b1 = s_second[me];
          s_best[me] = 0xFFFFFFFFu, s_second[me] = 0xFFFFFFFFu;
          int k = -1;
          if (b0 != 0xFFFFFFFFu) {
            const unsigned c0 = s_pool[s_qstart[me] + (b0 & 0xFF)];
            const int bestDist = b0 >> 8, bestLevel = (c0 >> 22) & 15;
            bool ok = bestDist <= (reloc ? (int)A.nn_ratio : kThHigh);
            if (ok && second && b1 != 0xFFFFFFFFu) {
              const unsigned c1 = s_pool[s_qstart[me] + (b1 & 0xFF)];
              const int bestDist2 = b1 >> 8, bestLevel2 = (c1 >> 22) & 15;
              if (bestLevel == bestLevel2 && (float)bestDist > A.nn_ratio * (float)bestDist2) ok = false;
            }
            if (ok) k = (int)(c0 & 0x1FFF) - k0, wl[j] = c0;
          }
          if (k != cl[j]) cl[j] = k, changed = 1;
          if (k >= 0 && (reloc || (ny >> 16))) atomicMin(&cur[k], q);
        }
      if (changed) s_changed[round & 1] = 1;
      __syncthreads();
      const int any = s_changed[round & 1];
      if (tid == 0) s_changed[(round + 1) & 1] = 0;
      for (int i = tid; i < Nc; i += 1024) prev[i] = INT_MAX;
      __syncthreads();
      if (!any) {
        settled = true;
        int* s_asg = prev;
        for (int i = tid; i < Nc; i += 1024) s_asg[i] = -1;
        __syncthreads();
        int nm = 0;
#pragma unroll
        for (int j = 0; j < kOwn; j++)
          if (lq[j] >= 0 && cl[j] >= 0) {
            atomicMax(&s_asg[cl[j]], (int)s_qid[lq[j]]);
            nm++;
            if (ori) {
              const int bin = (wl[j] >> 26) & 31;
              atomicOr(&s_bins[cl[j]], 1u << bin);
              atomicAdd(&s_hist[bin], 1);
            }
          }
        if (nm) atomicAdd(&s_nm, nm);
        __syncthreads();
        for (int i = tid; i < Nc; i += 1024) assign[k0 + i] = s_asg[i], KB[k0 + i] = s_bins[i];
        if (ori && tid < kHistoLen && s_hist[tid]) atomicAdd(&F[tid], s_hist[tid]);
        if (tid == 0 && s_nm) atomicAdd(&F[32], s_nm);
        break;
      }
    }
    if (tid == 0 && s_overflow == 1) atomicOr(&F[33], 1);
  }
  if (tid == 0 && !settled) atomicOr(&F[34], 1);
  asm volatile("s_waitcnt vmcnt(0)" ::: "memory");
  __syncthreads();
  if (A.n_cams > 1) {
    if (tid == 0) {
      __builtin_amdgcn_fence(__ATOMIC_RELEASE, "agent");
      asm volatile("s_waitcnt vmcnt(0)" ::: "memory");
      const int old = __hip_atomic_fetch_add(&F[35], 1, __ATOMIC_RELAXED, __HIP_MEMORY_SCOPE_AGENT);
      s_last = old == A.n_cams - 1;
      if (s_last) __builtin_amdgcn_fence(__ATOMIC_ACQUIRE, "agent");
    }
    __syncthreads();
    if (!s_last) return;
  }
  if (tid < kHistoLen) s_hist[tid] = __hip_atomic_load(&F[tid], __ATOMIC_RELAXED, __HIP_MEMORY_SCOPE_AGENT);
  if (tid == 0) {
    s_nm = __hip_atomic_load(&F[32], __ATOMIC_RELAXED, __HIP_MEMORY_SCOPE_AGENT);
    s_overflow = __hip_atomic_load(&F[33], __ATOMIC_RELAXED, __HIP_MEMORY_SCOPE_AGENT);
    s_fill = __hip_atomic_load(&F[34], __ATOMIC_RELAXED, __HIP_MEMORY_SCOPE_AGENT);
  }
  __syncthreads();
  int nmatches = s_nm;
  if (ori && !s_fill) {
    int max1 = 0, max2 = 0, max3 = 0, ind1 = -1, ind2 = -1, ind3 = -1;
    for (int i = 0; i < kHistoLen; i++) {
      const int sv = s_hist[i];
      if (sv > max1) {
        max3 = max2, max2 = max1, max1 = sv;
        ind3 = ind2, ind2 = ind1, ind1 = i;
      } else if (sv > max2) {
        max3 = max2, max2 = sv;
        ind3 = ind2, ind2 = i;
      } else if (sv > max3) {
        max3 = sv, ind3 = i;
      }
    }
    if (max2 < 0.1f * (float)max1) {
      ind2 = -1, ind3 = -1;
    } else if (max3 < 0.1f * (float)max1) {
      ind3 = -1;
    }
    unsigned losers = (1u << kHistoLen) - 1u;
    if (ind1 >= 0) losers &= ~(1u << ind1);
    if (ind2 >= 0) losers &= ~(1u << ind2);
    if (ind3 >= 0) losers &= ~(1u << ind3);
    for (int i = 0; i < kHistoLen; i++)
      if (i != ind1 && i != ind2 && i != ind3) nmatches -= s_hist[i];
    int kend;
    {
      int kb;
      cam_range(A, f, A.n_cams - 1, &kb, &kend);
    }
    for (int k = tid; k < kend; k += 1024)
      if (KB[k] & losers) assign[k] = VIEO_SBP_ERASED;
  }
  const bool replay = s_fill != 0;
  if (tid == 0) {
    A.nmatches[f] = s_overflow ? -1 : nmatches;
    A.need_seq[f] = 0;
  }
  if (tid < kFinStride) F[tid] = 0;
  __syncthreads();
  if (replay && tid < 64) {
    SbpArgs S = A;
    S.pool_lds = max(0, min(A.pool_cap, (lds_bytes - A.key_cap * 5 - 64) / 4));
    sbp_assign_seq(S, f, s_pool, tid);
  }
}

__global__ void __launch_bounds__(64) k_sbp_assign(SbpArgs A) {
  extern __shared__ unsigned s_pool[];
  if (A.need_seq && !A.need_seq[blockIdx.x]) return;
  sbp_assign_seq(A, blockIdx.x, s_pool, threadIdx.x);
}

struct FuseDev {
// ... 43 lines not shown
  const float* b = F.bounds[cami];
  if (!(u >= b[0] && u < b[1] && v >= b[2] && v < b[3])) return;
  const float PO[3] = {X0 - twc[0], X1 - twc[1], X2 - twc[2]};
  const float dist3D = sqrtf(PO[0] * PO[0] + PO[1] * PO[1] + PO[2] * PO[2]);
  if (dist3D < 0.8f * P.min_distance || dist3D > 1.2f * P.max_distance) return;
  if (FF.check_viewing_angle &&
      (double)(PO[0] * P.normal[0] + PO[1] * P.normal[1] + PO[2] * P.normal[2]) < 0.5 * (double)dist3D)
    return;
  const float ratio = P.max_distance / dist3D;
  int lvl = (int)ceilf((float)log((double)ratio) / F.log_scale_factor);
  if (lvl < 0)
    lvl = 0;
  else if (lvl >= F.n_levels)
    lvl = F.n_levels - 1;
  const float radius = FF.th_radius * FF.scale_factors[lvl];
  const float winv = (float)kGridCols / (b[1] - b[0]), hinv = (float)kGridRows / (b[3] - b[2]);
  const int min_cellx = max(0, (int)floorf((u - b[0] - radius) * winv));
  const int max_cellx = min(kGridCols - 1, (int)ceilf((u - b[0] + radius) * winv));
  const int min_celly = max(0, (int)floorf((v - b[2] - radius) * hinv));
  const int max_celly = min(kGridRows - 1, (int)ceilf((v - b[2] + radius) * hinv));
  if (min_cellx >= kGridCols || max_cellx < 0 || min_celly >= kGridRows || max_celly < 0) return;
  const uint4 d0 = ((const uint4*)P.desc)[0], d1 = ((const uint4*)P.desc)[1];
  unsigned best = 0xFFFFFFFFu;
  int bidx = -1, order = 0;
  for (int ix = min_cellx; ix <= max_cellx; ++ix) {
    const int s0 = cell_start[ix * kGridRows + min_celly], s1 = cell_start[ix * kGridRows + max_celly + 1];
    for (int e0 = s0; e0 < s1; e0 += 64) {
      const int e = e0 + lane;
      if (e < s1) {
        const float4 k = cell_rec[e];
        const int pk = __float_as_int(k.w), j = pk & 0xFFFF, oct = pk >> 16;
        bool ok = fabsf(k.x - u) < radius && fabsf(k.y - v) < radius && oct >= lvl - 1 && oct <= lvl;
        if (ok && FF.use_bf) {
          const float ex = u - k.x, ey = v - k.y;
          if (k.z >= 0) {
            const float er = (u - F.bf * invz) - k.z;
            ok = !((double)((ex * ex + ey * ey + er * er) * FF.inv_level_sigma2[oct]) > 7.8);
          } else
            ok = !((double)((ex * ex + ey * ey) * FF.inv_level_sigma2[oct]) > 5.99);
        }
        if (ok) {
          const unsigned d = (unsigned)hamming32q(d0, d1, desc + (size_t)j * 32);
          const unsigned key = (d << 20) | (unsigned)min(order + (e - s0), (1 << 20) - 1);
          if (key < best) best = key, bidx = j;
        }
      }
    }
    order += s1 - s0;
  }
#pragma unroll
  for (int o = 32; o > 0; o >>= 1) {
    const unsigned e = __shfl_xor(best, o);
    const int j = __shfl_xor(bidx, o);
    if (e < best) best = e, bidx = j;
  }
  if (lane == 0 && bidx >= 0) *oi = bidx, *od = (int)(best >> 20);
}

struct SbpScratch {
  DevBuf pool, cursor, qrec, q, nq, keys, ur, desc, taken, counts, assign, nm, pts, cam, cell_start, cell_rec, cell_ang, claim, need, fin, kbins;
};
static thread_local SbpScratch g_sbp;
static thread_local struct {
  bool valid = false;
  const void *keys = nullptr, *ur = nullptr, *counts = nullptr, *rec = nullptr;
  int n_frames = 0, key_cap = 0, n_cams = 0;
  hipStream_t st = nullptr;
  float bounds[kMaxCams][4] = {};
} g_grid;
static thread_local bool g_grid_keep = false;
static bool take_grid_keep() {
  const bool k = g_grid_keep;
  g_grid_keep = false;
  return k;
}

struct SbpGridRef {
  int* cell_start;
  float4* cell_rec;
  float* cell_ang;
  bool built;
};

static int run_search(SbpArgs& A, int n_frames, hipStream_t st, bool keep_grid, SbpGridRef* ext_grid = nullptr) {
  int rc;
  SbpScratch& S = g_sbp;
  if (A.n_cams < 1 || A.n_cams > kMaxCams) {
    set_error("search_by_projection: n_cams = %d (1..%d)", A.n_cams, kMaxCams);
    return VIEO_E_INVALID;
  }
  A.pool_cap = std::max(std::min(A.q_cap, 2 * kMaxKeys) * 32, 2 * kCandCap) + kSbpBlocksFew * 4 * kCandCap;
  static const int pool_lds_env = [] {
    const char* e = getenv("VIEO_SBP_POOL_LDS");
    return e ? atoi(e) : 0;
  }();
  A.pool_lds = std::min(A.pool_cap, pool_lds_env > 0 ? pool_lds_env : 5120);
  if ((rc = S.pool.ensure((size_t)n_frames * A.pool_cap * 4)) != VIEO_OK) return rc;
  if ((rc = S.cursor.ensure((size_t)n_frames * 4)) != VIEO_OK) return rc;
  if ((rc = S.qrec.ensure((size_t)n_frames * A.q_cap * sizeof(int2))) != VIEO_OK) return rc;
  A.pool = S.pool.as<unsigned>(), A.cursor = S.cursor.as<int>(), A.qrec = S.qrec.as<int2>();
  if (A.q_cap > (1 << 20)) {
    set_error("search_by_projection: more than %d queries per frame", 1 << 20);
    return VIEO_E_CAPACITY;
  }
  if (A.key_cap > kMaxKeys) {
    set_error("search_by_projection: more than %d keypoints per frame", kMaxKeys);
    return VIEO_E_CAPACITY;
  }
  if (ext_grid) {
    A.cell_start = ext_grid->cell_start, A.cell_rec = ext_grid->cell_rec, A.cell_ang = ext_grid->cell_ang;
  } else {
    if ((rc = S.cell_start.ensure((size_t)n_frames * A.n_cams * (kGridCells + 1) * 4)) != VIEO_OK) return rc;
    if ((rc = S.cell_rec.ensure((size_t)n_frames * A.key_cap * sizeof(float4))) != VIEO_OK) return rc;
    if ((rc = S.cell_ang.ensure((size_t)n_frames * A.key_cap * 4)) != VIEO_OK) return rc;
    A.cell_start = S.cell_start.as<int>(), A.cell_rec = S.cell_rec.as<float4>(), A.cell_ang = S.cell_ang.as<float>();
  }
  const bool same = ext_grid ? ext_grid->built
                             : (keep_grid && g_grid.valid && g_grid.keys == (const void*)A.keys && g_grid.ur == (const void*)A.uright &&
                                g_grid.counts == (const void*)(A.cam_first ? (const void*)A.cam_first : (const void*)A.counts) &&
                                g_grid.n_frames == n_frames && g_grid.key_cap == A.key_cap && g_grid.n_cams == A.n_cams &&
                                g_grid.st == st && g_grid.rec == S.cell_rec.p && !memcmp(g_grid.bounds, A.bounds, sizeof(g_grid.bounds)));
  if (!same) {
    if (n_frames * A.n_cams <= 16)
      hipLaunchKernelGGL(k_sbp_grid<1024>, dim3(n_frames * A.n_cams), dim3(1024), 0, st, A, (int*)A.cell_start, (float4*)A.cell_rec,
                         (float*)A.cell_ang);
    else
      hipLaunchKernelGGL(k_sbp_grid<256>, dim3(n_frames * A.n_cams), dim3(256), 0, st, A, (int*)A.cell_start, (float4*)A.cell_rec,
                         (float*)A.cell_ang);
  }
  else if (ext_grid)
    VIEO_HIP_CHECK(hipMemsetAsync(A.cursor, 0, (size_t)n_frames * 4, st));
  if (!ext_grid) {
    g_grid.valid = true, g_grid.keys = A.keys, g_grid.ur = A.uright;
    g_grid.counts = A.cam_first ? (const void*)A.cam_first : (const void*)A.counts;
    g_grid.n_frames = n_frames, g_grid.key_cap = A.key_cap, g_grid.n_cams = A.n_cams, g_grid.st = st, g_grid.rec = S.cell_rec.p;
    memcpy(g_grid.bounds, A.bounds, sizeof(g_grid.bounds));
  }
  const char* e_blocks = getenv("VIEO_SBP_BLOCKS");
  const int n_blocks = e_blocks && atoi(e_blocks) > 0 ? std::min(atoi(e_blocks), kSbpBlocksFew) : (n_frames <= 2 ? kSbpBlocksFew : kSbpBlocks);
  hipLaunchKernelGGL(k_sbp_candidates, dim3(n_blocks, n_frames), dim3(256),
                     (size_t)A.n_cams * (kGridCells + 1) * sizeof(unsigned short), st, A);
  const char* e_mode = getenv("VIEO_SBP_ASSIGN");
  const bool seq_only = e_mode && !strcmp(e_mode, "seq");
  const char* e_rounds = getenv("VIEO_SBP_MAX_ROUNDS");
  const int max_rounds = e_rounds && atoi(e_rounds) > 0 ? atoi(e_rounds) : 48;
  const size_t lds = (size_t)A.pool_lds * 4 + (size_t)A.key_cap * 5;
  A.need_seq = nullptr, A.claim = nullptr, A.max_rounds = max_rounds;
  if (!seq_only) {
    if ((rc = S.claim.ensure((size_t)n_frames * A.q_cap * 4)) != VIEO_OK) return rc;
    if ((rc = S.need.ensure((size_t)n_frames * 4)) != VIEO_OK) return rc;
    A.claim = S.claim.as<int>(), A.need_seq = S.need.as<int>();
    SbpArgs P = A;
    size_t lds_par = (size_t)P.pool_lds * 4 + (size_t)P.key_cap * 13;
    if (lds_par > 150 * 1024) P.pool_lds = 0, lds_par = (size_t)P.key_cap * 13;
    if (lds_par > 64 * 1024)
      VIEO_HIP_CHECK(hipFuncSetAttribute((const void*)k_sbp_assign_par, hipFuncAttributeMaxDynamicSharedMemorySize, 150 * 1024));
    const char* e_flat = getenv("VIEO_SBP_FLAT");
    const int cam_cap = (((A.key_cap + A.n_cams - 1) / A.n_cams) + 3) & ~3;
    const size_t state = (size_t)cam_cap * 13 + (size_t)kCamQ * 12;
    const bool flat = (e_flat ? atoi(e_flat) != 0 : (P.n_cams > 1 || n_frames <= 16)) && state + 64 + 6 * 4096 <= 150 * 1024;
    if (flat) {
      P.pool_lds = (int)(std::min<size_t>((size_t)P.pool_cap, (150 * 1024 - state - 64) / 6) & ~(size_t)1);
      const size_t lds_cam = (size_t)P.pool_lds * 6 + state;
      const void* fin_was = S.fin.p;
      if ((rc = S.fin.ensure((size_t)n_frames * kFinStride * 4)) != VIEO_OK) return rc;
      if ((rc = S.kbins.ensure((size_t)n_frames * A.key_cap * 4)) != VIEO_OK) return rc;
      if (S.fin.p != fin_was) VIEO_HIP_CHECK(hipMemsetAsync(S.fin.p, 0, S.fin.cap, st));
      VIEO_HIP_CHECK(hipFuncSetAttribute((const void*)k_sbp_assign_cam, hipFuncAttributeMaxDynamicSharedMemorySize, 150 * 1024));
      hipLaunchKernelGGL(k_sbp_assign_cam, dim3(n_frames, P.n_cams), dim3(1024), lds_cam, st, P, cam_cap, S.fin.as<int>(),
                         S.kbins.as<unsigned>(), (int)lds_cam);
      VIEO_HIP_CHECK(hipGetLastError());
      return VIEO_OK;
    }
    hipLaunchKernelGGL(k_sbp_assign_par, dim3(n_frames), dim3(1024), lds_par, st, P);
  }
  hipLaunchKernelGGL(k_sbp_assign, dim3(n_frames), dim3(64), lds, st, A);
  VIEO_HIP_CHECK(hipGetLastError());
  return VIEO_OK;
}

}

using namespace vieo;

extern "C" {

int vieo_sbp_keep_grid(int on) {
  g_grid_keep = on != 0;
  return VIEO_OK;
}

int vieo_sbp_project_last_frame_rig_batch_device(const vieo_last_frame_point* d_points, const int32_t* d_n,
                                                 int p_cap, int n_frames, const vieo_sbp_camera* d_cams,
                                                 const vieo_sbp_rig* d_rigs, int n_cams,
                                                 vieo_proj_query* d_queries, void* stream) {
  if (!d_points || !d_n || p_cap <= 0 || n_frames <= 0 || !d_cams || !d_queries || n_cams < 1 || n_cams > kMaxCams ||
      (!d_rigs && n_cams != 1))
    return VIEO_E_INVALID;
  int rc = require_device();
  if (rc != VIEO_OK) return rc;
  hipLaunchKernelGGL(k_sbp_project, dim3((p_cap * n_cams + 255) / 256, n_frames), dim3(256), 0,
                     (hipStream_t)stream, d_points, d_n, p_cap, d_cams, d_rigs, n_cams, d_queries);
  VIEO_HIP_CHECK(hipGetLastError());
  return VIEO_OK;
}

int vieo_sbp_project_last_frame_batch_device(const vieo_last_frame_point* d_points,
                                             const int32_t* d_n, int p_cap, int n_frames,
                                             const vieo_sbp_camera* d_cams,
                                             vieo_proj_query* d_queries, void* stream) {
  return vieo_sbp_project_last_frame_rig_batch_device(d_points, d_n, p_cap, n_frames, d_cams, nullptr, 1, d_queries,
                                                      stream);
}

static int search_batch(int mode, const vieo_proj_query* d_queries, const int32_t* d_nq, int q_cap, int n_frames,
                        const vieo_keypoint* d_keys, const float* d_uright, const uint8_t* d_desc,
                        const uint8_t* d_taken, const int32_t* d_counts, const int32_t* d_cam_first, int key_cap,
                        int img_first, int img_step, const float* h_bounds, int n_cams, float nn_ratio,
                        int check_orientation, int32_t* d_assign, int32_t* d_nmatches, void* stream) {
  const bool keep_grid = take_grid_keep();
  if (!d_queries || !d_nq || q_cap <= 0 || n_frames <= 0 || !d_keys || !d_uright || !d_desc ||
      (!d_counts && !d_cam_first) || !h_bounds || !d_assign || !d_nmatches || key_cap <= 0 ||
      (mode != VIEO_SBP_LAST_FRAME && mode != VIEO_SBP_LOCAL_MAP && mode != VIEO_SBP_RELOC))
    return VIEO_E_INVALID;
  int rc = require_device();
  if (rc != VIEO_OK) return rc;
  SbpArgs A;
  memset(&A, 0, sizeof(A));
  A.mode = mode;
  A.queries = d_queries, A.nq = d_nq, A.q_cap = q_cap;
  A.keys = d_keys, A.uright = d_uright, A.desc = d_desc, A.taken = d_taken, A.counts = d_counts;
  A.key_cap = key_cap, A.img_first = img_first, A.img_step = img_step;
  A.n_cams = n_cams, A.cam_first = d_cam_first;
  if (n_cams >= 1 && n_cams <= kMaxCams) memcpy(A.bounds, h_bounds, sizeof(float) * 4 * n_cams);
  A.nn_ratio = nn_ratio, A.check_ori = check_orientation;
  A.assign = d_assign, A.nmatches = d_nmatches;
  return run_search(A, n_frames, (hipStream_t)stream, keep_grid);
}

int vieo_search_by_projection_batch_device(int mode, const vieo_proj_query* d_queries,
                                           const int32_t* d_nq, int q_cap, int n_frames,
                                           const vieo_keypoint* d_keys, const float* d_uright,
                                           const uint8_t* d_desc, const uint8_t* d_taken,
                                           const int32_t* d_counts, int key_cap, int img_first,
                                           int img_step, const float* h_bounds, float nn_ratio,
                                           int check_orientation, int32_t* d_assign,
                                           int32_t* d_nmatches, void* stream) {
  if (!d_counts) return VIEO_E_INVALID;
  return search_batch(mode, d_queries, d_nq, q_cap, n_frames, d_keys, d_uright, d_desc, d_taken, d_counts, nullptr,
                      key_cap, img_first, img_step, h_bounds, 1, nn_ratio, check_orientation, d_assign, d_nmatches,
                      stream);
}

int vieo_search_by_projection_rig_batch_device(int mode, const vieo_proj_query* d_queries, const int32_t* d_nq,
                                               int q_cap, int n_frames, const vieo_keypoint* d_keys,
                                               const float* d_uright, const uint8_t* d_desc,
                                               const uint8_t* d_taken, const int32_t* d_cam_first, int key_cap,
                                               const float* h_bounds, int n_cams, float nn_ratio,
                                               int check_orientation, int32_t* d_assign, int32_t* d_nmatches,
                                               void* stream) {
  if (!d_cam_first) return VIEO_E_INVALID;
  return search_batch(mode, d_queries, d_nq, q_cap, n_frames, d_keys, d_uright, d_desc, d_taken, nullptr, d_cam_first,
                      key_cap, 0, 1, h_bounds, n_cams, nn_ratio, check_orientation, d_assign, d_nmatches, stream);
}

static int project_host(const void* h_points, int n, const vieo_sbp_camera* h_cam, const vieo_sbp_rig* h_rig,
                        int keyframe, float log_scale_factor, vieo_proj_query* h_queries) {
  if (n < 0 || !h_cam || (n > 0 && (!h_points || !h_queries))) return VIEO_E_INVALID;
  const int nc = h_rig ? h_rig->n_cams : 1;
  if (nc < 1 || nc > kMaxCams) {
    set_error("sbp_project: n_cams = %d (1..%d)", nc, kMaxCams);
    return VIEO_E_INVALID;
  }
  if (h_rig)
    for (int c = 0; c < nc; ++c) {
      CamD d;
      if (!cam_from_abi(h_rig->cams[c], d)) {
        set_error("sbp_project: camera %d has an unknown model or coefficient count", c);
        return VIEO_E_INVALID;
      }
    }
  if (h_cam->nlevels < 1 || h_cam->nlevels > 16) {
    set_error("sbp_project: nlevels = %d (1..16)", h_cam->nlevels);
    return VIEO_E_INVALID;
  }
  int rc = require_device();
  if (rc != VIEO_OK) return rc;
  if (n == 0) return VIEO_OK;
  SbpScratch& S = g_sbp;
  static thread_local DevBuf dRig;
  if ((rc = S.pts.ensure((size_t)n * 64)) != VIEO_OK) return rc;
  if ((rc = S.cam.ensure(sizeof(vieo_sbp_camera))) != VIEO_OK) return rc;
  if ((rc = S.q.ensure((size_t)n * nc * sizeof(vieo_proj_query))) != VIEO_OK) return rc;
  if ((rc = S.nq.ensure(4)) != VIEO_OK) return rc;
  if ((rc = dRig.ensure(sizeof(vieo_sbp_rig))) != VIEO_OK) return rc;
  VIEO_HIP_CHECK(hipMemcpy(S.pts.p, h_points, (size_t)n * 64, hipMemcpyHostToDevice));
  VIEO_HIP_CHECK(hipMemcpy(S.cam.p, h_cam, sizeof(vieo_sbp_camera), hipMemcpyHostToDevice));
  VIEO_HIP_CHECK(hipMemcpy(S.nq.p, &n, 4, hipMemcpyHostToDevice));
  if (h_rig) VIEO_HIP_CHECK(hipMemcpy(dRig.p, h_rig, sizeof(vieo_sbp_rig), hipMemcpyHostToDevice));
  const vieo_sbp_rig* d_rig = h_rig ? dRig.as<vieo_sbp_rig>() : nullptr;
  if (keyframe) {
    hipLaunchKernelGGL(k_sbp_project_kf, dim3((n * nc + 255) / 256), dim3(256), 0, 0, S.pts.as<vieo_keyframe_point>(),
                       n, S.cam.as<vieo_sbp_camera>(), d_rig, nc, log_scale_factor, S.q.as<vieo_proj_query>());
    VIEO_HIP_CHECK(hipGetLastError());
  } else {
    rc = vieo_sbp_project_last_frame_rig_batch_device(S.pts.as<vieo_last_frame_point>(), S.nq.as<int>(), n, 1,
                                                      S.cam.as<vieo_sbp_camera>(), d_rig, nc,
                                                      S.q.as<vieo_proj_query>(), nullptr);
    if (rc != VIEO_OK) return rc;
  }
  VIEO_HIP_CHECK(hipMemcpy(h_queries, S.q.p, (size_t)n * nc * sizeof(vieo_proj_query), hipMemcpyDeviceToHost));
  return VIEO_OK;
}

int vieo_sbp_project_last_frame(const vieo_last_frame_point* h_points, int n,
                                const vieo_sbp_camera* h_cam, vieo_proj_query* h_queries) {
  return project_host(h_points, n, h_cam, nullptr, 0, 0.f, h_queries);
}

int vieo_sbp_project_last_frame_rig(const vieo_last_frame_point* h_points, int n, const vieo_sbp_camera* h_cam,
                                    const vieo_sbp_rig* h_rig, vieo_proj_query* h_queries) {
  if (!h_rig) return VIEO_E_INVALID;
  return project_host(h_points, n, h_cam, h_rig, 0, 0.f, h_queries);
}

int vieo_sbp_project_keyframe(const vieo_keyframe_point* h_points, int n, const vieo_sbp_camera* h_cam,
                              const vieo_sbp_rig* h_rig, float log_scale_factor, vieo_proj_query* h_queries) {
  if (!(log_scale_factor > 0)) return VIEO_E_INVALID;
  return project_host(h_points, n, h_cam, h_rig, 1, log_scale_factor, h_queries);
}

int vieo_search_by_projection_rig(int mode, const vieo_proj_query* h_queries, int nq, const vieo_keypoint* h_keys,
                                  const float* h_uright, const uint8_t* h_desc, const uint8_t* h_taken, int n_keys,
                                  const int32_t* h_cam_first, const float* h_bounds, int n_cams, float nn_ratio,
                                  int check_orientation, int32_t* h_assign, int32_t* nmatches) {
  if (nq < 0 || n_keys < 0 || !h_bounds || !nmatches || n_cams < 1 || n_cams > kMaxCams || !h_cam_first ||
      (n_keys > 0 && (!h_keys || !h_uright || !h_desc || !h_assign)) || (nq > 0 && !h_queries))
    return VIEO_E_INVALID;
  if (h_cam_first[0] != 0 || h_cam_first[n_cams] != n_keys) {
    set_error("search_by_projection: cam_first must run from 0 to n_keys");
    return VIEO_E_INVALID;
  }
  for (int c = 0; c < n_cams; ++c)
    if (h_cam_first[c] > h_cam_first[c + 1]) {
      set_error("search_by_projection: cam_first is not ascending");
      return VIEO_E_INVALID;
// ... 231 lines not shown
```

vieo_slam_amd/csrc/wave_ops.h:

```cpp
#pragma once
#include <hip/hip_runtime.h>

namespace vieo {

#define VIEO_DPP_QUAD_XOR1 0xB1
#define VIEO_DPP_QUAD_XOR2 0x4E
#define VIEO_DPP_ROW_HALF_MIRROR 0x141
#define VIEO_DPP_ROW_MIRROR 0x140
#define VIEO_DPP_ROW_BCAST15 0x142
#define VIEO_DPP_ROW_BCAST31 0x143

#define VIEO_DPP(old, v, ctrl, row_mask) __builtin_amdgcn_update_dpp((int)(old), (int)(v), ctrl, row_mask, 0xF, false)

__device__ __forceinline__ int wave_sum_i32(int v) {
  v += VIEO_DPP(0, v, VIEO_DPP_QUAD_XOR1, 0xF);
  v += VIEO_DPP(0, v, VIEO_DPP_QUAD_XOR2, 0xF);
  v += VIEO_DPP(0, v, VIEO_DPP_ROW_HALF_MIRROR, 0xF);
  v += VIEO_DPP(0, v, VIEO_DPP_ROW_MIRROR, 0xF);
  v += VIEO_DPP(0, v, VIEO_DPP_ROW_BCAST15, 0xA);
  v += VIEO_DPP(0, v, VIEO_DPP_ROW_BCAST31, 0xC);
  return __builtin_amdgcn_readlane(v, 63);
}

__device__ __forceinline__ unsigned wave_min_u32(unsigned v) {
  v = min(v, (unsigned)VIEO_DPP(v, v, VIEO_DPP_QUAD_XOR1, 0xF));
  v = min(v, (unsigned)VIEO_DPP(v, v, VIEO_DPP_QUAD_XOR2, 0xF));
  v = min(v, (unsigned)VIEO_DPP(v, v, VIEO_DPP_ROW_HALF_MIRROR, 0xF));
  v = min(v, (unsigned)VIEO_DPP(v, v, VIEO_DPP_ROW_MIRROR, 0xF));
  v = min(v, (unsigned)VIEO_DPP(v, v, VIEO_DPP_ROW_BCAST15, 0xA));
  v = min(v, (unsigned)VIEO_DPP(v, v, VIEO_DPP_ROW_BCAST31, 0xC));
  return (unsigned)__builtin_amdgcn_readlane((int)v, 63);
}

__device__ __forceinline__ double wave_sum_f64(double v) {
#define VIEO_DPP_ADD_F64(ctrl, row_mask)                                  \
  {                                                                       \
    const int lo = __double2loint(v), hi = __double2hiint(v);             \
    const int l2 = VIEO_DPP(0, lo, ctrl, row_mask), h2 = VIEO_DPP(0, hi, ctrl, row_mask); \
    v += __hiloint2double(h2, l2);                                        \
  }
  VIEO_DPP_ADD_F64(VIEO_DPP_QUAD_XOR1, 0xF)
  VIEO_DPP_ADD_F64(VIEO_DPP_QUAD_XOR2, 0xF)
  VIEO_DPP_ADD_F64(VIEO_DPP_ROW_HALF_MIRROR, 0xF)
  VIEO_DPP_ADD_F64(VIEO_DPP_ROW_MIRROR, 0xF)
  VIEO_DPP_ADD_F64(VIEO_DPP_ROW_BCAST15, 0xA)
  VIEO_DPP_ADD_F64(VIEO_DPP_ROW_BCAST31, 0xC)
#undef VIEO_DPP_ADD_F64
  return __hiloint2double(__builtin_amdgcn_readlane(__double2hiint(v), 63), __builtin_amdgcn_readlane(__double2loint(v), 63));
}

__device__ __forceinline__ double quad_sum_f64(double v) {
  {
    const int l2 = VIEO_DPP(0, __double2loint(v), VIEO_DPP_QUAD_XOR1, 0xF), h2 = VIEO_DPP(0, __double2hiint(v), VIEO_DPP_QUAD_XOR1, 0xF);
    v += __hiloint2double(h2, l2);
  }
  {
    const int l2 = VIEO_DPP(0, __double2loint(v), VIEO_DPP_QUAD_XOR2, 0xF), h2 = VIEO_DPP(0, __double2hiint(v), VIEO_DPP_QUAD_XOR2, 0xF);
    v += __hiloint2double(h2, l2);
  }
  return v;
}

__device__ __forceinline__ double wave_max_f64(double v) {
#define VIEO_DPP_MAX_F64(ctrl, row_mask)                                                      \
  {                                                                                           \
    const int lo = __double2loint(v), hi = __double2hiint(v);                                 \
    const int l2 = VIEO_DPP(lo, lo, ctrl, row_mask), h2 = VIEO_DPP(hi, hi, ctrl, row_mask);   \
    v = fmax(v, __hiloint2double(h2, l2));                                                    \
  }
  VIEO_DPP_MAX_F64(VIEO_DPP_QUAD_XOR1, 0xF)
  VIEO_DPP_MAX_F64(VIEO_DPP_QUAD_XOR2, 0xF)
  VIEO_DPP_MAX_F64(VIEO_DPP_ROW_HALF_MIRROR, 0xF)
  VIEO_DPP_MAX_F64(VIEO_DPP_ROW_MIRROR, 0xF)
  VIEO_DPP_MAX_F64(VIEO_DPP_ROW_BCAST15, 0xA)
  VIEO_DPP_MAX_F64(VIEO_DPP_ROW_BCAST31, 0xC)
#undef VIEO_DPP_MAX_F64
  return __hiloint2double(__builtin_amdgcn_readlane(__double2hiint(v), 63), __builtin_amdgcn_readlane(__double2loint(v), 63));
}

}
```

vieo_slam_amd/pipeline.py:

```python
import ctypes

import numpy as np

from . import frontend, synth, synth_ba
from . import synth_scene as sc
from ._lib import DeviceBuffer, check, lib
from .ba_types import (LAST_FRAME_POINT_DTYPE, POSE_OBS_DTYPE, PROJ_QUERY_DTYPE, SBP_CAMERA_DTYPE,
                       VIO_FRAME_DTYPE, VIO_RESULT_DTYPE)
from .orb_extractor import KEYPOINT_DTYPE, ORBextractor

W, H = sc.W, sc.H
K = (sc.FX, sc.FY, sc.CX, sc.CY)
BOUNDS = np.array([0, W, 0, H], np.float32)
NFEAT, SCALE, NLEVELS, INI_TH, MIN_TH = 1200, 1.2, 8, 20, 7


def make_cases(n_base, seed0=1, verbose=False, workload="r2"):
    if workload == "r2":
        scene = sc.Scene(seed0)
        return [sc.make_tracking_case(seed0 + i, scene=scene) for i in range(n_base)]
    n_tex = min(8, n_base)
    texs = [sc.Scene(seed0 + 100 * t, relief=(seed0 + 100 * t, 12), low_contrast=True) for t in range(n_tex)]
    cases = []
    for i in range(n_base):
        scene = texs[i % n_tex] if i < n_tex else texs[i % n_tex].with_relief((seed0 + 7 * i, 12))
        c = sc.make_tracking_case(seed0 + i, scene=scene)
        c["scene"] = scene
        cases.append(c)
    return cases

N_EXTRA = 3072


class FramePipeline:
    STAGES = ("extract", "stereo", "sbp_last", "pose1", "sbp_local", "pose2", "total")

    def __init__(self, cases, batch, seed=0, noise=True, workload="r2"):
        self.workload = workload
        self.B = B = batch
        self.ext = ORBextractor(NFEAT, SCALE, NLEVELS, INI_TH, MIN_TH)
        self.stream = lib().vieo_orb_stream(self.ext._h)
        self.cap = cap = self.ext.max_keypoints()
        ext0 = [ORBextractor(NFEAT, SCALE, NLEVELS, INI_TH, MIN_TH) for _ in range(2)]
        scf = self.ext.GetScaleFactors()
        self.inv_sigma2 = (np.float32(1.0) / (scf * scf)).astype(np.float32)
        rng = np.random.default_rng(seed)
        imgs = np.zeros((B, 2, H, W), np.uint8)
        pts = np.zeros((B, cap), LAST_FRAME_POINT_DTYPE)
        npts = np.zeros(B, np.int32)
        cams = np.zeros(B, SBP_CAMERA_DTYPE)
        q2 = np.zeros((B, cap), PROJ_QUERY_DTYPE)
        xyz = np.zeros((B, 2 * cap, 3), np.float32)
        f1 = np.zeros(B, VIO_FRAME_DTYPE)
        self.truth = []
        from .matching import compute_stereo_matches
        for b in range(B):
            case = cases[b % len(cases)]

            def jitter(im):
                if not noise or b < len(cases):
                    return im
                return np.clip(im.astype(np.int16) + rng.integers(-2, 3, im.shape), 0, 255).astype(np.uint8)
            L0, R0 = [jitter(x) for x in case["images0"]]
            imgs[b, 0], imgs[b, 1] = [jitter(x) for x in case["images1"]]
            _, k0, d0 = ext0[0](L0)
            _, k0r, d0r = ext0[1](R0)
            ur0, dp0 = compute_stereo_matches(ext0[0], ext0[1], k0, d0, k0r, d0r, sc.BASELINE, sc.BF)
            Ri, pi, Rwc0, twc0 = case["pose0"]
            Xw, valid = frontend.unproject_stereo(k0, dp0, K, Rwc0, twc0)
            n0 = len(k0)
            pts[b, :n0] = frontend.make_last_frame_points(k0, d0, Xw, valid, True)
            npts[b] = n0
            xyz[b, :n0] = Xw
            xyz[b, cap:cap + n0] = Xw
            F = case["vio"].copy()
            F[0]["base"]["nav"]["p"] += rng.normal(0, 0.01, 3)
            F[0]["base"]["nav"]["q"] = synth_ba.quat_mul(
                F[0]["base"]["nav"]["q"], synth_ba.quat_from_rotvec(rng.normal(0, 0.003, 3)))
            f1[b] = F[0]
            Rwb = synth_ba.quat_to_R(F[0]["base"]["nav"]["q"])
            Tbc = synth_ba.EUROC_TBC
            Rwc = Rwb @ Tbc[:3, :3]
            twc = F[0]["base"]["nav"]["p"] + Rwb @ Tbc[:3, 3]
            Tcw = frontend.pose_to_Tcw(Rwc, twc)
            cams[b] = frontend.make_sbp_camera(Tcw, frontend.pose_to_Tcw(Rwc0, twc0), K, BOUNDS,
                                               sc.BF, sc.BASELINE, 7.0, scf)[0]
            Xc = Xw.astype(np.float64) @ Tcw[:, :3].T + Tcw[:, 3]
            z = np.where(Xc[:, 2] > 0.1, Xc[:, 2], 1.0)
            u = (sc.FX * Xc[:, 0] / z + sc.CX).astype(np.float32)
            v = (sc.FY * Xc[:, 1] / z + sc.CY).astype(np.float32)
            inimg = valid & (Xc[:, 2] > 0.1) & (u >= 0) & (u < W) & (v >= 0) & (v < H)
            q = q2[b, :n0]
            q["u"], q["v"] = u, v
            q["ur"] = u - np.float32(sc.BF) / z.astype(np.float32)
            q["radius"] = np.float32(4.0) * scf[k0["octave"]]
            q["level_min"], q["level_max"] = k0["octave"] - 1, k0["octave"]
            q["angle"] = k0["angle"]
            q["flags"] = inimg.astype(np.int32) * 3
            q["desc"] = d0
            self.truth.append(case["truth"])
        if workload == "r3":
            self._local_candidates(cases, pts, npts, xyz_last=xyz, rng=rng)
        f2 = f1.copy()
        f2["compute_marg"] = 1
        self.imgs_host = imgs
        self.n_img = 2 * B
        D = DeviceBuffer
        self.d_img = D(imgs.nbytes)
        self.d_img.upload(imgs)
        self.d_kp, self.d_desc, self.d_cnt = D(2 * B * cap * 28), D(2 * B * cap * 32), D(2 * B * 8)
        self.d_ur, self.d_dp = D(B * cap * 4), D(B * cap * 4)
        self.d_pts, self.d_npts, self.d_cams = D(pts.nbytes), D(npts.nbytes), D(cams.nbytes)
        self.d_pts.upload(pts), self.d_npts.upload(npts), self.d_cams.upload(cams)
        if workload == "r3":
            self.d_q1, self.d_q2 = D(B * cap * 64), D(B * self.ccap * 64)
        else:
            self.d_q1, self.d_q2 = D(B * cap * 64), D(q2.nbytes)
            self.d_q2.upload(q2)
        self.d_assign, self.d_nm = D(B * cap * 4), D(B * 4)
        self.d_mpref, self.d_taken = D(B * cap * 4), D(B * cap)
        if workload == "r3":
            xyz = self.xyz3
        self.d_xyz, self.d_isig = D(xyz.nbytes), D(self.inv_sigma2.nbytes)
        self.d_xyz.upload(xyz), self.d_isig.upload(self.inv_sigma2)
        self.d_obs, self.d_obskey, self.d_outl = D(B * cap * 32), D(B * cap * 4), D(B * cap)
        self.d_f1, self.d_f2 = D(f1.nbytes), D(f2.nbytes)
        self.d_f1.upload(f1), self.d_f2.upload(f2)
        self.d_r1, self.d_r2 = D(B * VIO_RESULT_DTYPE.itemsize), D(B * VIO_RESULT_DTYPE.itemsize)
        self.bounds = (ctypes.c_float * 4)(*BOUNDS.tolist())
        self.f1_host, self.pts_host, self.q2_host = f1, pts, q2
        check(lib().vieo_device_synchronize())

    def _local_candidates(self, cases, pts, npts, xyz_last, rng):
        from .ba_types import CAMERA_DTYPE
        from .map_point import FRUSTUM_FRAME_DTYPE, FRUSTUM_POINT_DTYPE
        B, cap = self.B, self.cap
        self.ccap = ccap = cap + N_EXTRA
        self.pcap = cap + ccap
        scf = self.ext.GetScaleFactors()
        cpt = np.zeros((B, ccap), FRUSTUM_POINT_DTYPE)
        cdesc = np.zeros((B, ccap, 32), np.uint8)
        alias = np.full((B, ccap), -1, np.int32)
        ncand = np.zeros(B, np.int32)
        self.xyz3 = np.zeros((B, self.pcap, 3), np.float32)
        for b in range(B):
            case = cases[b % len(cases)]
            n0 = int(npts[b])
            Xw = pts[b, :n0]["Xw"].astype(np.float64)
            valid = (pts[b, :n0]["flags"] & 1) > 0
            Ow0 = case["pose0"][3]
            d = Xw - Ow0
            dist = np.linalg.norm(d, axis=1)
            dist = np.where(valid, dist, 1.0)
            c = cpt[b, :n0]
            c["Xw"], c["normal"] = Xw, (d / dist[:, None])
            maxd = (dist * scf[pts[b, :n0]["octave"]]).astype(np.float32)
            c["max_distance"] = np.where(valid, maxd, 0)
            c["min_distance"] = np.where(valid, maxd / scf[NLEVELS - 1], 0)
            cdesc[b, :n0] = pts[b, :n0]["desc"]
            alias[b, :n0] = np.arange(n0)
            Xe = case["scene"].surface_points(rng, N_EXTRA)
            Ow1 = case["pose1"][3]
            de = Xe - Ow1
            diste = np.linalg.norm(de, axis=1)
            e = cpt[b, n0:n0 + N_EXTRA]
            e["Xw"], e["normal"] = Xe, de / diste[:, None]
            md = (diste * scf[rng.integers(0, NLEVELS, N_EXTRA)]).astype(np.float32)
            e["max_distance"], e["min_distance"] = md, md / scf[NLEVELS - 1]
            cdesc[b, n0:n0 + N_EXTRA] = rng.integers(0, 256, (N_EXTRA, 32), dtype=np.uint8)
            ncand[b] = n0 + N_EXTRA
            self.xyz3[b, :n0] = xyz_last[b, :n0]
            self.xyz3[b, cap:cap + n0 + N_EXTRA] = cpt[b, :n0 + N_EXTRA]["Xw"]
        D = DeviceBuffer
        self.d_cpt, self.d_cdesc, self.d_alias, self.d_ncand = D(cpt.nbytes), D(cdesc.nbytes), D(alias.nbytes), D(ncand.nbytes)
        self.d_cpt.upload(cpt), self.d_cdesc.upload(cdesc), self.d_alias.upload(alias), self.d_ncand.upload(ncand)
        self.d_held, self.d_cdep, self.d_nq = D(B * self.pcap), D(B * ccap * 4), D(B * 4)
        self.d_scale = D(scf.nbytes)
        self.d_scale.upload(np.ascontiguousarray(scf, np.float32))
        self._cam = np.zeros(1, CAMERA_DTYPE)
        self._cam[0]["fx"], self._cam[0]["fy"], self._cam[0]["cx"], self._cam[0]["cy"] = sc.FX, sc.FY, sc.CX, sc.CY
        self.ff = np.zeros(1, FRUSTUM_FRAME_DTYPE)
        ff = self.ff[0]
        ff["n_cams"], ff["use_distort"], ff["cams"] = 1, 0, self._cam.ctypes.data
        ff["Tcr"][0] = np.eye(4)[:3].reshape(-1)
        ff["bounds"][0] = BOUNDS
        ff["bf"], ff["n_levels"], ff["viewing_cos_limit"] = sc.BF, NLEVELS, 0.5
        ff["log_scale_factor"] = np.float32(np.log(np.float32(SCALE)))
        self.ncand_host = ncand

    def enable_timing(self, on=True):
        self._ev = None
        self._ev_steps = 0
        if on:
            self._ev = []
            for _ in range(64):
                row = []
                for _ in range(len(self.STAGES)):
                    e = ctypes.c_void_p()
                    check(lib().vieo_event_create(ctypes.byref(e)))
                    row.append(e)
                self._ev.append(row)

    def _stamp(self, k):
        if getattr(self, "_ev", None):
            check(lib().vieo_event_record(self._ev[self._ev_steps % 64][k], self.stream))

    def stage_ms_all(self):
        out = []
        n = min(self._ev_steps, 64)
        for s in range(self._ev_steps - n, self._ev_steps):
            row = self._ev[s % 64]
            ms = {}
            for k, name in enumerate(self.STAGES[:-1]):
                v = ctypes.c_float()
                check(lib().vieo_event_elapsed_ms(row[k], row[k + 1], ctypes.byref(v)))
                ms[name] = v.value
            v = ctypes.c_float()
            check(lib().vieo_event_elapsed_ms(row[0], row[-1], ctypes.byref(v)))
            ms["total"] = v.value
            out.append(ms)
        return out

    def step(self):
        self._step()

    def _step(self):
        L, B, cap, st = lib(), self.B, self.cap, self.stream
        self._stamp(0)
        self.ext.extract_batch_device(self.d_img.ptr, self.n_img, W, H, W, W * H, self.d_kp.ptr,
                                      self.d_desc.ptr, cap, self.d_cnt.ptr)
        self._stamp(1)
        check(L.vieo_stereo_match_rectified_batch_device(self.ext._h, B, self.d_kp.ptr, self.d_desc.ptr,
                                                         self.d_cnt.ptr, cap, sc.BASELINE, sc.BF,
                                                         self.d_ur.ptr, self.d_dp.ptr), "stereo")
        self._stamp(2)
        check(L.vieo_sbp_project_last_frame_batch_device(self.d_pts.ptr, self.d_npts.ptr, cap, B,
                                                         self.d_cams.ptr, self.d_q1.ptr, st), "project")
        check(L.vieo_search_by_projection_batch_device(0, self.d_q1.ptr, self.d_npts.ptr, cap, B,
                                                       self.d_kp.ptr, self.d_ur.ptr, self.d_desc.ptr,
                                                       None, self.d_cnt.ptr, cap, 0, 2, self.bounds, 0.9,
                                                       1, self.d_assign.ptr, self.d_nm.ptr, st), "sbp1")
        self._stamp(3)
        check(L.vieo_track_merge_assign_batch_device(self.d_assign.ptr, self.d_mpref.ptr, self.d_cnt.ptr,
                                                     cap, B, 0, 2, 0, 1, st))
        check(L.vieo_track_build_obs_batch_device(self.d_mpref.ptr, self.d_xyz.ptr,
                                                  self.pcap if self.workload == "r3" else 2 * cap, self.d_kp.ptr,
                                                  self.d_ur.ptr, self.d_cnt.ptr, cap, B, 0, 2,
                                                  self.d_isig.ptr, self.d_obs.ptr, self.d_obskey.ptr,
                                                  self.d_f1.ptr, 1, st))
        check(L.vieo_pose_optimization_vio_batch_device_ex(self.d_f1.ptr, B, self.d_obs.ptr, self.d_outl.ptr,
                                                           self.d_r1.ptr, 1, 1, st), "pose1")
        self._stamp(4)
        check(L.vieo_track_after_pose_batch_device(self.d_mpref.ptr, self.d_obskey.ptr, self.d_outl.ptr,
                                                   self.d_f1.ptr, self.d_r1.ptr, 1, cap, B, self.d_f2.ptr,
                                                   self.d_taken.ptr, st))
        if self.workload == "r3":
            check(L.vieo_track_mark_held_batch_device(self.d_mpref.ptr, self.d_cnt.ptr, cap, B, 0, 2, self.d_held.ptr,
                                                      self.pcap, st))
            check(L.vieo_track_local_queries_batch_device(self.ff.ctypes.data, self.d_f1.ptr, self.d_r1.ptr, B, self.d_cpt.ptr,
                                                          self.d_cdesc.ptr, self.d_alias.ptr, self.d_ncand.ptr, self.ccap,
                                                          self.d_held.ptr, self.pcap, 2.0, 0.0, self.d_scale.ptr,
                                                          self.d_q2.ptr, self.d_cdep.ptr, self.ccap, self.d_nq.ptr, st),
                  "local queries")
            nq, qcap, ptab = self.d_nq.ptr, self.ccap, self.pcap
        else:
            nq, qcap, ptab = self.d_npts.ptr, cap, 2 * cap
        check(L.vieo_search_by_projection_batch_device(1, self.d_q2.ptr, nq, qcap, B,
                                                       self.d_kp.ptr, self.d_ur.ptr, self.d_desc.ptr,
                                                       self.d_taken.ptr, self.d_cnt.ptr, cap, 0, 2,
                                                       self.bounds, 0.8, 1, self.d_assign.ptr,
                                                       self.d_nm.ptr, st), "sbp2")
        self._stamp(5)
        check(L.vieo_track_merge_assign_batch_device(self.d_assign.ptr, self.d_mpref.ptr, self.d_cnt.ptr,
                                                     cap, B, 0, 2, cap, 0, st))
        check(L.vieo_track_build_obs_batch_device(self.d_mpref.ptr, self.d_xyz.ptr, ptab, self.d_kp.ptr,
                                                  self.d_ur.ptr, self.d_cnt.ptr, cap, B, 0, 2,
                                                  self.d_isig.ptr, self.d_obs.ptr, self.d_obskey.ptr,
                                                  self.d_f2.ptr, 1, st))
        check(L.vieo_pose_optimization_vio_batch_device_ex(self.d_f2.ptr, B, self.d_obs.ptr, self.d_outl.ptr,
                                                           self.d_r2.ptr, 1, 1, st), "pose2")
        self._stamp(6)
        if getattr(self, "_ev", None):
            self._ev_steps += 1

    def sync(self):
        self.ext.sync()

    def results(self):
        self.sync()
        B, cap = self.B, self.cap
        return dict(r1=self.d_r1.download(VIO_RESULT_DTYPE, (B,)),
                    r2=self.d_r2.download(VIO_RESULT_DTYPE, (B,)),
                    counts=self.d_cnt.download(np.int32, (2 * B, 2)),
                    f2=self.d_f2.download(VIO_FRAME_DTYPE, (B,)),
                    mp_ref=self.d_mpref.download(np.int32, (B, cap)),
                    uright=self.d_ur.download(np.float32, (B, cap)),
                    kps=self.d_kp.download(KEYPOINT_DTYPE, (2 * B, cap)),
                    desc=self.d_desc.download(np.uint8, (2 * B, cap, 32)))
```

vieo_slam_amd/pipeline_rig_batch.py:

```python
import ctypes

import numpy as np

from . import frontend, synth_ba
from . import synth_fisheye as sf
from ._lib import DeviceBuffer, check, lib
from .ba_types import (FISHEYE_PARAMS_DTYPE, LAST_FRAME_POINT_DTYPE, SBP_CAMERA_DTYPE, VIO_FRAME_DTYPE, VIO_RESULT_DTYPE)
from .map_point import FRUSTUM_POINT_DTYPE
from .matching import FisheyeStereoDevice
from .orb_extractor import KEYPOINT_DTYPE, ORBextractor
from .pipeline_rig import NLEVELS, RigFrontEnd


class RigFramePipeline:
    STAGES = ("extract", "stereo", "sbp_last", "pose1", "sbp_local", "pose2", "total")

    def __init__(self, scene, cases, nfeatures, batch, seed=0, noise=True, th_depth=35.0):
        L = lib()
        self.scene, self.B, self.nc = scene, batch, len(scene.cams)
        B, nc = self.B, self.nc
        self.fe = fe = RigFrontEnd(scene, nfeatures)
        self.ext = ORBextractor(nfeatures, 1.2, NLEVELS, 20, 7)
        self.stream = L.vieo_orb_stream(self.ext._h)
        self.cap = cap = self.ext.max_keypoints()
        self.kc = kc = nc * cap
        W, H = scene.W, scene.H
        self.lap = fe.lapping
        rng = np.random.default_rng(seed)
        prep = []
        for case in cases:
            fr0 = fe.make_frame(case["images0"])
            mps = fe.make_map_points(fr0, case["pose0"][2], case["pose0"][3])
            pts = fe.last_frame_points(fr0, mps)
            has = mps["key_mp"] >= 0
            pts["reserved"][has, 0] = mps["first_key"][mps["key_mp"][has]] + 1
            z = fr0.fe["group_p3d"][np.nonzero(fr0.fe["group_good"])[0]][:, 2].astype(np.float32)
            ld = np.full(fr0.N, np.inf, np.float32)
            ld[has] = z[mps["key_mp"][has]]
            _, P = fe._frustum(np.eye(3, 4), mps, case["pose0"])
            prep.append(dict(fr0=fr0, mps=mps, pts=pts, last_depth=ld, z=z, P=np.ascontiguousarray(P, FRUSTUM_POINT_DTYPE)))
        self.prep = prep
        self.ccap = ccap = max(len(p["P"]) for p in prep) + 16
        self.pcap = pcap = kc + ccap
        imgs = np.zeros((B, nc, H, W), np.uint8)
        pts = np.zeros((B, kc), LAST_FRAME_POINT_DTYPE)
        n_last, n_q1 = np.zeros(B, np.int32), np.zeros(B, np.int32)
        xyz = np.zeros((B, pcap, 3), np.float32)
        dep = np.full((B, pcap), np.inf, np.float32)
        cpt = np.zeros((B, ccap), FRUSTUM_POINT_DTYPE)
        cdesc = np.zeros((B, ccap, 32), np.uint8)
        alias = np.full((B, ccap), -1, np.int32)
        ncand = np.zeros(B, np.int32)
        f1 = np.zeros(B, VIO_FRAME_DTYPE)
        cams = np.zeros(B, SBP_CAMERA_DTYPE)
        self.d_camarr = DeviceBuffer(scene.cams.nbytes)
        self.d_camarr.upload(scene.cams)
        self.truth, self.case_of = [], []
        for b in range(B):
            ci = b % len(cases)
            case, pr = cases[ci], prep[ci]
            self.case_of.append(ci)
            for c in range(nc):
                im = case["images1"][c]
                if noise and b >= len(cases):
                    im = np.clip(im.astype(np.int16) + rng.integers(-2, 3, im.shape), 0, 255).astype(np.uint8)
                imgs[b, c] = im
            n0 = pr["fr0"].N
            pts[b, :n0] = pr["pts"]
            n_last[b], n_q1[b] = n0, n0 * nc
            has = pr["mps"]["key_mp"] >= 0
            xyz[b, :n0][has] = pr["mps"]["Xw"][pr["mps"]["key_mp"][has]]
            dep[b, :n0] = pr["last_depth"]
            ncl = len(pr["P"])
            cpt[b, :ncl], cdesc[b, :ncl] = pr["P"], pr["mps"]["desc"]
            alias[b, :ncl] = pr["mps"]["first_key"]
            ncand[b] = ncl
            xyz[b, kc:kc + ncl] = pr["mps"]["Xw"]
            F = case["vio"].copy()
            bb = F[0]["base"]
            bb["nav"]["p"] += rng.normal(0, 0.01, 3)
            bb["nav"]["q"] = synth_ba.quat_mul(bb["nav"]["q"], synth_ba.quat_from_rotvec(rng.normal(0, 0.003, 3)))
            bb["n_cams"], bb["cams"] = nc, self.d_camarr.ptr
            F[0]["th_depth"] = th_depth
            f1[b] = F[0]
            Ri, pi, Rwc0, twc0 = case["pose0"]
            cams[b] = fe._sbp_cam(bb["nav"], frontend.pose_to_Tcw(Rwc0, twc0), fe.th_last)[0][0]
            self.truth.append(case["truth"])
        f2 = f1.copy()
        f2["compute_marg"] = 1
        self.f1_host, self.imgs_host = f1, imgs
        rigs = np.repeat(fe.rig, B)
        D = DeviceBuffer
        self.n_img = B * nc
        self.d_img = D(imgs.nbytes)
        self.d_img.upload(imgs)
        self.d_kp, self.d_desc, self.d_cnt = D(self.n_img * cap * KEYPOINT_DTYPE.itemsize), D(self.n_img * cap * 32), D(self.n_img * 8)
        sig2 = fe.sigma2
        fp = np.zeros(1, FISHEYE_PARAMS_DTYPE)
        fp[0]["n_cams"], fp[0]["n_levels"], fp[0]["bf"], fp[0]["th_far_pts"] = nc, NLEVELS, fe.bf, 0.0
        fp[0]["cams"], fp[0]["Trc"], fp[0]["Tcr"], fp[0]["level_sigma2"] = (scene.cams.ctypes.data, fe._Trc.ctypes.data,
                                                                            fe._Tcr.ctypes.data, sig2.ctypes.data)
        self.fish = FisheyeStereoDevice(fp, cap, max_frames=B)
        gcap = self.gcap = self.fish.gcap
        self.d_kcat, self.d_dcat = D(B * kc * KEYPOINT_DTYPE.itemsize), D(B * kc * 32)
        self.d_first, self.d_fcnt = D(B * (nc + 1) * 4), D(B * 8)
        self.d_depth, self.d_ur, self.d_kg = D(B * kc * 4), D(B * kc * 4), D(B * kc * 4)
        self.d_gidx, self.d_good, self.d_p3d, self.d_hdr = D(B * gcap * nc * 4), D(B * gcap), D(B * gcap * 24), D(B * 32)
        self.d_pts, self.d_cams, self.d_rigs = D(pts.nbytes), D(cams.nbytes), D(rigs.nbytes)
        self.d_n_last, self.d_n_q1 = D(n_last.nbytes), D(n_q1.nbytes)
        self.d_pts.upload(pts), self.d_cams.upload(cams), self.d_rigs.upload(rigs)
        self.d_n_last.upload(n_last), self.d_n_q1.upload(n_q1)
        self.d_q1, self.d_q1c, self.d_qsrc, self.d_nq1 = D(B * kc * nc * 64), D(B * kc * nc * 64), D(B * kc * nc * 4), D(B * 4)
        self.d_q2, self.d_nq2 = D(B * ccap * nc * 64), D(B * 4)
        self.d_assign, self.d_nm = D(B * kc * 4), D(B * 4)
        self.d_mpref, self.d_taken, self.d_held = D(B * kc * 4), D(B * kc), D(B * pcap)
        self.d_xyz, self.d_dep = D(xyz.nbytes), D(dep.nbytes)
        self.d_xyz.upload(xyz), self.d_dep.upload(dep)
        self.d_cpt, self.d_cdesc, self.d_alias, self.d_ncand = D(cpt.nbytes), D(cdesc.nbytes), D(alias.nbytes), D(ncand.nbytes)
        self.d_cpt.upload(cpt), self.d_cdesc.upload(cdesc), self.d_alias.upload(alias), self.d_ncand.upload(ncand)
        consts = np.concatenate([np.pad(fe.inv_sigma2, (0, 16 - NLEVELS)), np.pad(fe.scale, (0, 16 - NLEVELS))]).astype(np.float32)
        self.d_consts = D(consts.nbytes)
        self.d_consts.upload(consts)
        self.d_obs, self.d_obskey, self.d_outl = D(B * kc * 32), D(B * kc * 4), D(B * kc)
        self.d_f1, self.d_f2 = D(f1.nbytes), D(f2.nbytes)
        self.d_f1.upload(f1), self.d_f2.upload(f2)
        self.d_r1, self.d_r2 = D(B * VIO_RESULT_DTYPE.itemsize), D(B * VIO_RESULT_DTYPE.itemsize)
        self.bounds = np.ascontiguousarray(fe.bounds, np.float32)
        self.ff = fe._frustum(np.eye(3, 4), prep[0]["mps"], cases[0]["pose0"])[0]
        self.close = float(max(10.0, th_depth))
        check(L.vieo_device_synchronize())
        self._ev = None

    def enable_timing(self, on=True):
        self._ev, self._ev_steps = None, 0
        if on:
            self._ev = []
            for _ in range(64):
                row = []
                for _ in range(len(self.STAGES)):
                    e = ctypes.c_void_p()
                    check(lib().vieo_event_create(ctypes.byref(e)))
                    row.append(e)
                self._ev.append(row)

    def _stamp(self, k):
        if self._ev:
            check(lib().vieo_event_record(self._ev[self._ev_steps % 64][k], self.stream))

    def stage_ms_all(self):
        out = []
        n = min(self._ev_steps, 64)
        for s in range(self._ev_steps - n, self._ev_steps):
            row, ms = self._ev[s % 64], {}
            for k, name in enumerate(self.STAGES[:-1]):
                v = ctypes.c_float()
                check(lib().vieo_event_elapsed_ms(row[k], row[k + 1], ctypes.byref(v)))
                ms[name] = v.value
            v = ctypes.c_float()
            check(lib().vieo_event_elapsed_ms(row[0], row[-1], ctypes.byref(v)))
            ms["total"] = v.value
            out.append(ms)
        return out

    def step(self):
        L, B, nc, cap, kc, st = lib(), self.B, self.nc, self.cap, self.kc, self.stream
        W, H = self.scene.W, self.scene.H
        self._stamp(0)
        self.ext.extract_batch_device(self.d_img.ptr, self.n_img, W, H, W, W * H, self.d_kp.ptr, self.d_desc.ptr, cap,
                                      self.d_cnt.ptr, lapping=self.lap)
        self._stamp(1)
        check(L.vieo_stereo_fisheye_match_batch_device(self.fish.h, self.d_kp.ptr, self.d_desc.ptr, self.d_cnt.ptr, B,
                                                       self.d_kcat.ptr, self.d_dcat.ptr, self.d_first.ptr, self.d_fcnt.ptr,
                                                       self.d_depth.ptr, self.d_ur.ptr, self.d_kg.ptr, self.d_gidx.ptr,
                                                       self.d_good.ptr, self.d_p3d.ptr, self.d_hdr.ptr, st), "fisheye")
        self._stamp(2)
        check(L.vieo_sbp_project_last_frame_rig_batch_device(self.d_pts.ptr, self.d_n_last.ptr, kc, B, self.d_cams.ptr,
                                                             self.d_rigs.ptr, nc, self.d_q1.ptr, st), "project")
        check(L.vieo_track_compact_queries_batch_device(self.d_q1.ptr, self.d_n_q1.ptr, kc * nc, B, self.d_q1c.ptr, self.d_qsrc.ptr,
                                                        self.d_nq1.ptr, st), "compact")
        check(L.vieo_search_by_projection_rig_batch_device(0, self.d_q1c.ptr, self.d_nq1.ptr, kc * nc, B, self.d_kcat.ptr,
                                                           self.d_ur.ptr, self.d_dcat.ptr, None, self.d_first.ptr, kc,
                                                           self.bounds.ctypes.data, nc, 0.9, 1, self.d_assign.ptr, self.d_nm.ptr,
                                                           st), "sbp1")
        self._stamp(3)
        check(L.vieo_track_merge_assign_rig_batch_device(self.d_assign.ptr, self.d_mpref.ptr, self.d_fcnt.ptr, kc, B, 0, 1, 0, 1, nc,
                                                         self.d_pts.ptr, self.d_qsrc.ptr, kc * nc, st))
        check(L.vieo_track_build_obs_rig_batch_device(self.d_mpref.ptr, self.d_xyz.ptr, self.d_dep.ptr, self.close, self.pcap,
                                                      self.d_kcat.ptr, self.d_ur.ptr, self.d_fcnt.ptr, self.d_first.ptr, nc, kc, B,
                                                      self.d_consts.ptr, self.d_obs.ptr, self.d_obskey.ptr, self.d_f1.ptr, 1, st))
        check(L.vieo_pose_optimization_vio_batch_device_ex(self.d_f1.ptr, B, self.d_obs.ptr, self.d_outl.ptr, self.d_r1.ptr,
                                                           2, 1, st), "pose1")
        self._stamp(4)
        check(L.vieo_track_after_pose_batch_device(self.d_mpref.ptr, self.d_obskey.ptr, self.d_outl.ptr, self.d_f1.ptr,
                                                   self.d_r1.ptr, 1, kc, B, self.d_f2.ptr, self.d_taken.ptr, st))
        check(L.vieo_track_mark_held_batch_device(self.d_mpref.ptr, self.d_fcnt.ptr, kc, B, 0, 1, self.d_held.ptr, self.pcap, st))
        check(L.vieo_track_local_queries_batch_device(self.ff.ctypes.data, self.d_f1.ptr, self.d_r1.ptr, B, self.d_cpt.ptr,
                                                      self.d_cdesc.ptr, self.d_alias.ptr, self.d_ncand.ptr, self.ccap,
                                                      self.d_held.ptr, self.pcap, self.fe.th_local, 0.0, self.d_consts.ptr + 64,
                                                      self.d_q2.ptr, self.d_dep.ptr + 4 * kc, self.pcap, self.d_nq2.ptr, st),
              "local queries")
        check(L.vieo_search_by_projection_rig_batch_device(1, self.d_q2.ptr, self.d_nq2.ptr, self.ccap * nc, B, self.d_kcat.ptr,
                                                           self.d_ur.ptr, self.d_dcat.ptr, self.d_taken.ptr, self.d_first.ptr, kc,
                                                           self.bounds.ctypes.data, nc, self.fe.nn_local, 1, self.d_assign.ptr,
                                                           self.d_nm.ptr, st), "sbp2")
        self._stamp(5)
        check(L.vieo_track_merge_assign_rig_batch_device(self.d_assign.ptr, self.d_mpref.ptr, self.d_fcnt.ptr, kc, B, 0, 1, kc, 0, nc,
                                                         None, None, 0, st))
        check(L.vieo_track_build_obs_rig_batch_device(self.d_mpref.ptr, self.d_xyz.ptr, self.d_dep.ptr, self.close, self.pcap,
                                                      self.d_kcat.ptr, self.d_ur.ptr, self.d_fcnt.ptr, self.d_first.ptr, nc, kc, B,
                                                      self.d_consts.ptr, self.d_obs.ptr, self.d_obskey.ptr, self.d_f2.ptr, 1, st))
        check(L.vieo_pose_optimization_vio_batch_device_ex(self.d_f2.ptr, B, self.d_obs.ptr, self.d_outl.ptr, self.d_r2.ptr,
                                                           2, 1, st), "pose2")
        self._stamp(6)
        if self._ev:
            self._ev_steps += 1

    def sync(self):
        self.ext.sync()

    def results(self):
        self.sync()
        B, kc = self.B, self.kc
        return dict(r1=self.d_r1.download(VIO_RESULT_DTYPE, (B,)), r2=self.d_r2.download(VIO_RESULT_DTYPE, (B,)),
                    mp_ref=self.d_mpref.download(np.int32, (B, kc)), first=self.d_first.download(np.int32, (B, self.nc + 1)),
                    hdr=self.d_hdr.download(np.int32, (B, 8)), keys=self.d_kcat.download(KEYPOINT_DTYPE, (B, kc)),
                    depth=self.d_depth.download(np.float32, (B, kc)), nm=self.d_nm.download(np.int32, (B,)))

    def close_all(self):
        self.fish.close()
```

Before: 61160.

## Emit compacted query lists with source indices directly from projection kernels

Projection and local-query kernels now use a block-wide exclusive scan to write only live queries contiguously, along with an index array that maps each one back to its source slot. Indexed search-by-projection kernels consume these compacted lists, so the separate compaction kernel and the searches over empty padded queries are dropped. The pipeline also enables keeping the grid between the two searches by default. In exchange, the compaction work moves inside each block as a serial loop over points, with one block per frame.

```diff
diff --git a/include/vieo_hot.h b/include/vieo_hot.h
--- a/include/vieo_hot.h
+++ b/include/vieo_hot.h
@@ -297,6 +297,30 @@
                                                const float* h_bounds, int n_cams, float nn_ratio,
                                                int check_orientation, int32_t* d_assign, int32_t* d_nmatches,
                                                void* stream);
+
+int vieo_sbp_project_last_frame_compact_batch_device(const vieo_last_frame_point* d_points, const int32_t* d_n, int p_cap,
+                                                     int n_frames, const vieo_sbp_camera* d_cams,
+                                                     vieo_proj_query* d_queries, int32_t* d_qidx, int32_t* d_nq,
+                                                     void* stream);
+int vieo_sbp_project_last_frame_rig_compact_batch_device(const vieo_last_frame_point* d_points, const int32_t* d_n,
+                                                         int p_cap, int n_frames, const vieo_sbp_camera* d_cams,
+                                                         const vieo_sbp_rig* d_rigs, int n_cams,
+                                                         vieo_proj_query* d_queries, int32_t* d_qidx, int32_t* d_nq,
+                                                         void* stream);
+int vieo_search_by_projection_indexed_batch_device(int mode, const vieo_proj_query* d_queries, const int32_t* d_nq,
+                                                   const int32_t* d_qidx, int q_cap, int n_frames,
+                                                   const vieo_keypoint* d_keys, const float* d_uright,
+                                                   const uint8_t* d_desc, const uint8_t* d_taken, const int32_t* d_counts,
+                                                   int key_cap, int img_first, int img_step, const float* h_bounds,
+                                                   float nn_ratio, int check_orientation, int32_t* d_assign,
+                                                   int32_t* d_nmatches, void* stream);
+int vieo_search_by_projection_rig_indexed_batch_device(int mode, const vieo_proj_query* d_queries, const int32_t* d_nq,
+                                                       const int32_t* d_qidx, int q_cap, int n_frames,
+                                                       const vieo_keypoint* d_keys, const float* d_uright,
+                                                       const uint8_t* d_desc, const uint8_t* d_taken,
+                                                       const int32_t* d_cam_first, int key_cap, const float* h_bounds,
+                                                       int n_cams, float nn_ratio, int check_orientation,
+                                                       int32_t* d_assign, int32_t* d_nmatches, void* stream);
 
 int vieo_sbp_keep_grid(int on);
 
@@ -681,6 +705,13 @@
                                           const uint8_t* d_held, int held_cap, float th, float th_far, const float* d_scale,
                                           vieo_proj_query* d_queries, float* d_track_depth, size_t depth_stride,
                                           int32_t* d_nq, void* stream);
+int vieo_track_local_queries_compact_batch_device(const vieo_frustum_frame* h_frame, const vieo_vio_frame* d_frames,
+                                                  const vieo_vio_result* d_results, int n_frames,
+                                                  const vieo_frustum_point* d_points, const uint8_t* d_desc,
+                                                  const int32_t* d_alias, const int32_t* d_counts, int p_cap,
+                                                  const uint8_t* d_held, int held_cap, float th, float th_far,
+                                                  const float* d_scale, vieo_proj_query* d_queries, int32_t* d_qidx,
+                                                  float* d_track_depth, size_t depth_stride, int32_t* d_nq, void* stream);
 int vieo_track_local_queries_slot_batch_device(const vieo_frustum_frame* h_frame, const void* d_frames, size_t frame_stride,
                                                const void* d_results, size_t result_stride, int n_frames,
                                                const int32_t* d_pos_slot, const vieo_frustum_point* d_points,
diff --git a/vieo_slam_amd/_lib.py b/vieo_slam_amd/_lib.py
--- a/vieo_slam_amd/_lib.py
+++ b/vieo_slam_amd/_lib.py
@@ -43,6 +43,8 @@
                                                               c_p, ctypes.c_size_t, c_p, c_p, c_p, c_p, c_p, c_p]),
     "vieo_track_local_queries_batch_device": (c_i, [c_p, c_p, c_p, c_i, c_p, c_p, c_p, c_p, c_i, c_p, c_i, c_f, c_f, c_p, c_p,
                                                     c_p, c_sz, c_p, c_p]),
+    "vieo_track_local_queries_compact_batch_device": (c_i, [c_p, c_p, c_p, c_i, c_p, c_p, c_p, c_p, c_i, c_p, c_i, c_f, c_f,
+                                                            c_p, c_p, c_p, c_p, c_sz, c_p, c_p]),
     "vieo_pose_optimization_vio_batch_device_ex": (c_i, [c_p, c_i, c_p, c_p, c_p, c_i, c_i, c_p]),
     "vieo_pose_optimization_batch_device_ex": (c_i, [c_p, c_i, c_p, c_p, c_p, c_i, c_p]),
     "vieo_get_device": (c_i, []),
@@ -116,6 +118,12 @@
     "vieo_search_by_projection": (c_i, [c_i, c_p, c_i, c_p, c_p, c_p, c_p, c_i, c_p, c_f, c_i, c_p, c_p]),
     "vieo_search_by_projection_batch_device": (c_i, [c_i, c_p, c_p, c_i, c_i, c_p, c_p, c_p, c_p, c_p, c_i, c_i, c_i, c_p, c_f, c_i, c_p, c_p, c_p]),
     "vieo_sbp_project_last_frame_batch_device": (c_i, [c_p, c_p, c_i, c_i, c_p, c_p, c_p]),
+    "vieo_sbp_project_last_frame_compact_batch_device": (c_i, [c_p, c_p, c_i, c_i, c_p, c_p, c_p, c_p, c_p]),
+    "vieo_sbp_project_last_frame_rig_compact_batch_device": (c_i, [c_p, c_p, c_i, c_i, c_p, c_p, c_i, c_p, c_p, c_p, c_p]),
+    "vieo_search_by_projection_indexed_batch_device": (c_i, [c_i, c_p, c_p, c_p, c_i, c_i, c_p, c_p, c_p, c_p, c_p, c_i, c_i,
+                                                             c_i, c_p, c_f, c_i, c_p, c_p, c_p]),
+    "vieo_search_by_projection_rig_indexed_batch_device": (c_i, [c_i, c_p, c_p, c_p, c_i, c_i, c_p, c_p, c_p, c_p, c_p, c_i,
+                                                                 c_p, c_i, c_f, c_i, c_p, c_p, c_p]),
     "vieo_pose_optimization": (c_i, [c_p, c_p, c_p, c_p]),
     "vieo_pose_optimization_batch_device": (c_i, [c_p, c_i, c_p, c_p, c_p, c_p]),
     "vieo_pose_optimization_vio": (c_i, [c_p, c_p, c_p, c_p]),
diff --git a/vieo_slam_amd/csrc/mappoint.hip b/vieo_slam_amd/csrc/mappoint.hip
--- a/vieo_slam_amd/csrc/mappoint.hip
+++ b/vieo_slam_amd/csrc/mappoint.hip
@@ -1,6 +1,7 @@
 #include <climits>
 
 #include "ba_device.h"
+#include "wave_ops.h"
 
 namespace vieo {
 
@@ -79,6 +80,60 @@
   out[m] = T;
 }
 
+__device__ __forceinline__ void track_local_frame(vieo_frustum_frame& sF, const FrustumDev& tmpl,
+                                                  const vieo_pose_frame* __restrict__ frame,
+                                                  const vieo_pose_result* __restrict__ result) {
+  sF = tmpl.F;
+  const vieo_navstate& nav = result->status == 0 ? result->nav : frame->nav;
+  double Rwb[9];
+  {
+    const double qw = nav.q[0], qx = nav.q[1], qy = nav.q[2], qz = nav.q[3];
+    const double tx = 2 * qx, ty = 2 * qy, tz = 2 * qz;
+    const double twx = tx * qw, twy = ty * qw, twz = tz * qw, txx = tx * qx, txy = ty * qx, txz = tz * qx;
+    const double tyy = ty * qy, tyz = tz * qy, tzz = tz * qz;
+    Rwb[0] = 1 - (tyy + tzz), Rwb[1] = txy - twz, Rwb[2] = txz + twy;
+    Rwb[3] = txy + twz, Rwb[4] = 1 - (txx + tzz), Rwb[5] = tyz - twx;
+    Rwb[6] = txz - twy, Rwb[7] = tyz + twx, Rwb[8] = 1 - (txx + tyy);
+  }
+  const double* Rcb = frame->Rcb;
+  double Rcw[9], tcw[3];
+  for (int r = 0; r < 3; ++r)
+    for (int c = 0; c < 3; ++c) Rcw[r * 3 + c] = Rcb[r * 3] * Rwb[c * 3] + Rcb[r * 3 + 1] * Rwb[c * 3 + 1] + Rcb[r * 3 + 2] * Rwb[c * 3 + 2];
+  for (int r = 0; r < 3; ++r)
+    tcw[r] = frame->tcb[r] - (Rcw[r * 3] * nav.p[0] + Rcw[r * 3 + 1] * nav.p[1] + Rcw[r * 3 + 2] * nav.p[2]);
+  for (int i = 0; i < 9; ++i) sF.Rcrw[i] = (float)Rcw[i];
+  for (int r = 0; r < 3; ++r) {
+    sF.tcrw[r] = (float)tcw[r];
+    sF.Ow[r] = (float)(-(Rcw[r] * tcw[0] + Rcw[3 + r] * tcw[1] + Rcw[6 + r] * tcw[2]));
+  }
+}
+
+__device__ __forceinline__ int track_local_live(const vieo_frustum_frame& sF, const FrustumDev& tmpl, const vieo_frustum_point& P,
+                                                const int32_t* __restrict__ alias, const uint8_t* __restrict__ held, int held_cap,
+                                                int m, float th_far, vieo_track_info& T) {
+  frustum_eval(sF, tmpl.cams, P, T);
+  int cnt = T.n;
+  if (th_far > 0.f && T.track_depth > th_far) cnt = 0;
+  if (alias && alias[m] >= 0 && alias[m] < held_cap && held[alias[m]]) cnt = 0;
+  return cnt;
+}
+
+__device__ __forceinline__ void track_local_record(const vieo_track_info& T, int k, float th, const float* __restrict__ scale,
+                                                   const uint4& d0, const uint4& d1, vieo_proj_query& q) {
+  float u = 0, v = 0, ur = 0, vc = 0;
+  int lvl = 0, cam = 0;
+#pragma unroll
+  for (int j = 0; j < 4; ++j)
+    if (j == k) u = T.u[j], v = T.v[j], ur = T.ur[j], vc = T.viewcos[j], lvl = T.level[j], cam = T.cam[j];
+  float r = vc > 0.998f ? 2.5f : 4.0f;
+  if (th != 1.0f) r = r * th;
+  q.u = u, q.v = v, q.ur = ur;
+  q.radius = r * scale[lvl];
+  q.level_min = lvl - 1, q.level_max = lvl, q.angle = 0.f;
+  q.flags = 3 | (cam << 8);
+  ((uint4*)q.desc)[0] = d0, ((uint4*)q.desc)[1] = d1;
+}
+
 __device__ __forceinline__ void track_local_queries_body(vieo_frustum_frame& sF, const FrustumDev& tmpl,
                                                          const vieo_pose_frame* __restrict__ frame,
                                                          const vieo_pose_result* __restrict__ result,
@@ -88,29 +143,7 @@
                                                          vieo_proj_query* __restrict__ queries, float* __restrict__ track_depth,
                                                          int32_t* __restrict__ nq) {
   if (threadIdx.x == 0) {
-    sF = tmpl.F;
-    const vieo_navstate& nav = result->status == 0 ? result->nav : frame->nav;
-    double Rwb[9];
-    {
-      const double qw = nav.q[0], qx = nav.q[1], qy = nav.q[2], qz = nav.q[3];
-      const double tx = 2 * qx, ty = 2 * qy, tz = 2 * qz;
-      const double twx = tx * qw, twy = ty * qw, twz = tz * qw, txx = tx * qx, txy = ty * qx, txz = tz * qx;
-      const double tyy = ty * qy, tyz = tz * qy, tzz = tz * qz;
-      Rwb[0] = 1 - (tyy + tzz), Rwb[1] = txy - twz, Rwb[2] = txz + twy;
-      Rwb[3] = txy + twz, Rwb[4] = 1 - (txx + tzz), Rwb[5] = tyz - twx;
-      Rwb[6] = txz - twy, Rwb[7] = tyz + twx, Rwb[8] = 1 - (txx + tyy);
-    }
-    const double* Rcb = frame->Rcb;
-    double Rcw[9], tcw[3];
-    for (int r = 0; r < 3; ++r)
-      for (int c = 0; c < 3; ++c) Rcw[r * 3 + c] = Rcb[r * 3] * Rwb[c * 3] + Rcb[r * 3 + 1] * Rwb[c * 3 + 1] + Rcb[r * 3 + 2] * Rwb[c * 3 + 2];
-    for (int r = 0; r < 3; ++r)
-      tcw[r] = frame->tcb[r] - (Rcw[r * 3] * nav.p[0] + Rcw[r * 3 + 1] * nav.p[1] + Rcw[r * 3 + 2] * nav.p[2]);
-    for (int i = 0; i < 9; ++i) sF.Rcrw[i] = (float)Rcw[i];
-    for (int r = 0; r < 3; ++r) {
-      sF.tcrw[r] = (float)tcw[r];
-      sF.Ow[r] = (float)(-(Rcw[r] * tcw[0] + Rcw[3 + r] * tcw[1] + Rcw[6 + r] * tcw[2]));
-    }
+    track_local_frame(sF, tmpl, frame, result);
     if (blockIdx.x == 0) *nq = n * tmpl.F.n_cams;
   }
   __syncthreads();
@@ -118,31 +151,15 @@
   if (m >= n) return;
   const vieo_frustum_point P = pts[m];
   vieo_track_info T;
-  frustum_eval(sF, tmpl.cams, P, T);
+  const int cnt = track_local_live(sF, tmpl, P, alias, held, held_cap, m, th_far, T);
   const int S = sF.n_cams;
-  int cnt = T.n;
-  if (th_far > 0.f && T.track_depth > th_far) cnt = 0;
-  if (alias && alias[m] >= 0 && alias[m] < held_cap && held[alias[m]]) cnt = 0;
   track_depth[m] = T.track_depth;
   const uint4* d = (const uint4*)(desc + (size_t)m * 32);
   const uint4 d0 = d[0], d1 = d[1];
   for (int k = 0; k < S; ++k) {
     vieo_proj_query q;
     memset(&q, 0, sizeof(q));
-    if (k < cnt) {
-      float u = 0, v = 0, ur = 0, vc = 0;
-      int lvl = 0, cam = 0;
-#pragma unroll
-      for (int j = 0; j < 4; ++j)
-        if (j == k) u = T.u[j], v = T.v[j], ur = T.ur[j], vc = T.viewcos[j], lvl = T.level[j], cam = T.cam[j];
-      float r = vc > 0.998f ? 2.5f : 4.0f;
-      if (th != 1.0f) r = r * th;
-      q.u = u, q.v = v, q.ur = ur;
-      q.radius = r * scale[lvl];
-      q.level_min = lvl - 1, q.level_max = lvl, q.angle = 0.f;
-      q.flags = 3 | (cam << 8);
-      ((uint4*)q.desc)[0] = d0, ((uint4*)q.desc)[1] = d1;
-    }
+    if (k < cnt) track_local_record(T, k, th, scale, d0, d1, q);
     queries[(size_t)m * S + k] = q;
   }
 }
@@ -168,6 +185,57 @@
                            queries, track_depth, nq);
 }
 
+template <int NT>
+__global__ void __launch_bounds__(NT)
+k_track_local_queries_compact(FrustumDev tmpl, const vieo_vio_frame* __restrict__ frame, const vieo_vio_result* __restrict__ result,
+                              const vieo_frustum_point* __restrict__ pts, const uint8_t* __restrict__ desc,
+                              const int32_t* __restrict__ alias, const uint8_t* __restrict__ held, int held_cap, float th,
+                              float th_far, const float* __restrict__ scale, vieo_proj_query* __restrict__ queries,
+                              int32_t* __restrict__ qidx, float* __restrict__ track_depth, int32_t* __restrict__ nq, int p_cap,
+                              const int32_t* __restrict__ counts, size_t depth_stride) {
+  __shared__ vieo_frustum_frame sF;
+  __shared__ int s_part[2][NT / 64];
+  const size_t f = blockIdx.x;
+  const int tid = threadIdx.x;
+  frame += f, result += f;
+  pts += f * p_cap, desc += f * p_cap * 32;
+  if (alias) alias += f * p_cap, held += f * held_cap;
+  queries += f * p_cap * tmpl.F.n_cams, qidx += f * p_cap * tmpl.F.n_cams, track_depth += f * depth_stride;
+  const int n = min(counts[f], p_cap);
+  if (tid == 0) track_local_frame(sF, tmpl, &frame->base, &result->base);
+  __syncthreads();
+  const int S = sF.n_cams;
+  int base = 0;
+  vieo_frustum_point Pn = {};
+  if (tid < n) Pn = pts[tid];
+  for (int m0 = 0, it = 0; m0 < n; m0 += NT, ++it) {
+    const int m = m0 + tid;
+    const vieo_frustum_point P = Pn;
+    if (m + NT < n) Pn = pts[m + NT];
+    vieo_track_info T;
+    int cnt = 0;
+    if (m < n) {
+      cnt = track_local_live(sF, tmpl, P, alias, held, held_cap, m, th_far, T);
+      track_depth[m] = T.track_depth;
+    }
+    int total;
+    const int off = base + block_excl_scan_i32<NT / 64>(cnt, s_part[it & 1], &total);
+    if (cnt > 0) {
+      const uint4* d = (const uint4*)(desc + (size_t)m * 32);
+      const uint4 d0 = d[0], d1 = d[1];
+      for (int k = 0; k < cnt; ++k) {
+        vieo_proj_query q;
+        memset(&q, 0, sizeof(q));
+        track_local_record(T, k, th, scale, d0, d1, q);
+        queries[off + k] = q;
+        qidx[off + k] = m * S + k;
+      }
+    }
+    base += total;
+  }
+  if (tid == 0) nq[f] = base;
+}
+
 __global__ void __launch_bounds__(256)
 k_track_local_queries_slot(FrustumDev tmpl, const uint8_t* __restrict__ frames, size_t frame_stride,
                            const uint8_t* __restrict__ results, size_t result_stride, const int32_t* __restrict__ pos_slot,
@@ -391,6 +459,42 @@
   hipLaunchKernelGGL(k_track_local_queries, dim3((p_cap + 255) / 256, n_frames), dim3(256), 0, (hipStream_t)stream, fd, d_frames,
                      d_results, d_points, d_desc, d_alias, d_held, held_cap, 0, th, th_far, d_scale, d_queries, d_track_depth,
                      d_nq, p_cap, d_counts, depth_stride);
+  VIEO_HIP_CHECK(hipGetLastError());
+  return VIEO_OK;
+}
+
+int vieo_track_local_queries_compact_batch_device(const vieo_frustum_frame* h_frame, const vieo_vio_frame* d_frames,
+                                                  const vieo_vio_result* d_results, int n_frames,
+                                                  const vieo_frustum_point* d_points, const uint8_t* d_desc,
+                                                  const int32_t* d_alias, const int32_t* d_counts, int p_cap,
+                                                  const uint8_t* d_held, int held_cap, float th, float th_far,
+                                                  const float* d_scale, vieo_proj_query* d_queries, int32_t* d_qidx,
+                                                  float* d_track_depth, size_t depth_stride, int32_t* d_nq, void* stream) {
+  if (!h_frame || !d_frames || !d_results || n_frames <= 0 || p_cap <= 0 || !d_counts || !d_scale || !d_nq || !d_points ||
+      !d_desc || !d_queries || !d_qidx || !d_track_depth || (d_alias && (!d_held || held_cap <= 0)))
+    return VIEO_E_INVALID;
+  if (h_frame->n_cams < 1 || h_frame->n_cams > 4 || !h_frame->cams || h_frame->n_levels <= 0) {
+    set_error("SearchLocalPoints: n_cams = %d (1..4) with cameras and n_levels > 0", h_frame->n_cams);
+    return VIEO_E_INVALID;
+  }
+  if ((long long)p_cap * h_frame->n_cams > INT_MAX) {
+    set_error("SearchLocalPoints: %d candidates x %d cameras do not fit a slot index", p_cap, h_frame->n_cams);
+    return VIEO_E_CAPACITY;
+  }
+  int rc = require_device();
+  if (rc != VIEO_OK) return rc;
+  FrustumDev fd;
+  memset(&fd, 0, sizeof(fd));
+  fd.F = *h_frame;
+  fd.F.cams = nullptr;
+  for (int c = 0; c < h_frame->n_cams; ++c)
+    if (!cam_from_abi(h_frame->cams[c], fd.cams[c])) {
+      set_error("SearchLocalPoints: camera %d has an unknown model or coefficient count", c);
+      return VIEO_E_INVALID;
+    }
+  hipLaunchKernelGGL(k_track_local_queries_compact<1024>, dim3(n_frames), dim3(1024), 0, (hipStream_t)stream, fd, d_frames,
+                     d_results, d_points, d_desc, d_alias, d_held, held_cap, th, th_far, d_scale, d_queries, d_qidx,
+                     d_track_depth, d_nq, p_cap, d_counts, depth_stride);
   VIEO_HIP_CHECK(hipGetLastError());
   return VIEO_OK;
 }
diff --git a/vieo_slam_amd/csrc/proj_search.hip b/vieo_slam_amd/csrc/proj_search.hip
--- a/vieo_slam_amd/csrc/proj_search.hip
+++ b/vieo_slam_amd/csrc/proj_search.hip
@@ -29,23 +29,8 @@
   }
 }
 
-__global__ void __launch_bounds__(256)
-k_sbp_project(const vieo_last_frame_point* __restrict__ pts, const int* __restrict__ n_pts,
-              int p_cap, const vieo_sbp_camera* __restrict__ cams, const vieo_sbp_rig* __restrict__ rigs,
-              int n_cams, vieo_proj_query* __restrict__ out) {
-  const int f = blockIdx.y;
-  const int t = blockIdx.x * blockDim.x + threadIdx.x;
-  if (t >= p_cap * n_cams) return;
-  const int i = t / n_cams, camj = t - i * n_cams;
-  vieo_proj_query q;
-  memset(&q, 0, sizeof(q));
-  vieo_proj_query* dst = out + (size_t)f * p_cap * n_cams + t;
-  if (i >= n_pts[f]) {
-    *dst = q;
-    return;
-  }
-  const vieo_sbp_camera& C = cams[f];
-  const vieo_last_frame_point p = pts[(size_t)f * p_cap + i];
+__device__ __forceinline__ bool sbp_project_one(const vieo_last_frame_point& p, const vieo_sbp_camera& C,
+                                                const vieo_sbp_rig* __restrict__ rigs, int f, int camj, vieo_proj_query& q) {
   bool ok = p.flags & 1;
   const double* Tc = C.Tcw_cur;
   const double* Tl = C.Tcw_last;
@@ -96,7 +81,55 @@
     q.flags = 1 | (p.flags & 2) | (camj << 8);
     for (int k = 0; k < 32; k++) q.desc[k] = p.desc[k];
   }
+  return ok;
+}
+
+__global__ void __launch_bounds__(256)
+k_sbp_project(const vieo_last_frame_point* __restrict__ pts, const int* __restrict__ n_pts,
+              int p_cap, const vieo_sbp_camera* __restrict__ cams, const vieo_sbp_rig* __restrict__ rigs,
+              int n_cams, vieo_proj_query* __restrict__ out) {
+  const int f = blockIdx.y;
+  const int t = blockIdx.x * blockDim.x + threadIdx.x;
+  if (t >= p_cap * n_cams) return;
+  const int i = t / n_cams, camj = t - i * n_cams;
+  vieo_proj_query q;
+  memset(&q, 0, sizeof(q));
+  vieo_proj_query* dst = out + (size_t)f * p_cap * n_cams + t;
+  if (i >= n_pts[f]) {
+    *dst = q;
+    return;
+  }
+  const vieo_last_frame_point p = pts[(size_t)f * p_cap + i];
+  (void)sbp_project_one(p, cams[f], rigs, f, camj, q);
   *dst = q;
+}
+
+template <int NT>
+__global__ void __launch_bounds__(NT)
+k_sbp_project_compact(const vieo_last_frame_point* __restrict__ pts, const int* __restrict__ n_pts, int p_cap,
+                      const vieo_sbp_camera* __restrict__ cams, const vieo_sbp_rig* __restrict__ rigs, int n_cams,
+                      vieo_proj_query* __restrict__ out, int* __restrict__ qidx, int* __restrict__ nq) {
+  __shared__ int s_part[2][NT / 64];
+  const int f = blockIdx.x, tid = threadIdx.x;
+  const int n_slots = min(max(n_pts[f], 0), p_cap) * n_cams;
+  pts += (size_t)f * p_cap, out += (size_t)f * p_cap * n_cams, qidx += (size_t)f * p_cap * n_cams;
+  int base = 0;
+  for (int t0 = 0, it = 0; t0 < n_slots; t0 += NT, ++it) {
+    const int t = t0 + tid;
+    vieo_proj_query q;
+    memset(&q, 0, sizeof(q));
+    bool ok = false;
+    if (t < n_slots) {
+      const int i = t / n_cams, camj = t - i * n_cams;
+      const vieo_last_frame_point p = pts[i];
+      ok = sbp_project_one(p, cams[f], rigs, f, camj, q);
+    }
+    int total;
+    const int off = base + block_excl_scan_i32<NT / 64>(ok ? 1 : 0, s_part[it & 1], &total);
+    if (ok) out[off] = q, qidx[off] = t;
+    base += total;
+  }
+  if (tid == 0) nq[f] = base;
 }
 
 __global__ void __launch_bounds__(256)
@@ -163,6 +196,7 @@
   const vieo_proj_query* queries;
   const int* nq;
   int q_cap;
+  const int* qidx;
   const vieo_keypoint* keys;
   const float* uright;
   const uint8_t* desc;
@@ -194,6 +228,10 @@
          __popc(a1.x ^ b1.x) + __popc(a1.y ^ b1.y) + __popc(a1.z ^ b1.z) + __popc(a1.w ^ b1.w);
 }
 
+__device__ __forceinline__ int sbp_report(const SbpArgs& A, int f, int v) {
+  return (A.qidx && v >= 0) ? A.qidx[(size_t)f * A.q_cap + v] : v;
+}
+
 static const int kGridCells = kGridCols * kGridRows;
 
 __device__ __forceinline__ void cam_range(const SbpArgs& A, int f, int cam, int* k0, int* k1) {
@@ -277,19 +315,6 @@
     rec[i] = make_float4(k.x, k.y, uright[j], __int_as_float((j + k0) | (k.octave << 16)));
     ang[i] = k.angle;
   }
-}
-
-__device__ __forceinline__ int wave_excl_scan_i(int v, int lane, int* total) {
-  int x = v;
-  x += __builtin_amdgcn_update_dpp(0, x, 0x111, 0xF, 0xF, true);
-  x += __builtin_amdgcn_update_dpp(0, x, 0x112, 0xF, 0xF, true);
-  x += __builtin_amdgcn_update_dpp(0, x, 0x114, 0xF, 0xF, true);
-  x += __builtin_amdgcn_update_dpp(0, x, 0x118, 0xF, 0xF, true);
-  x += VIEO_DPP(0, x, VIEO_DPP_ROW_BCAST15, 0xA);
-  x += VIEO_DPP(0, x, VIEO_DPP_ROW_BCAST31, 0xC);
-  (void)lane;
-  *total = __builtin_amdgcn_readlane(x, 63);
-  return x - v;
 }
 
 static const int kSbpBlocks = 8;
@@ -510,7 +535,7 @@
       seg_l = cs[col + max_celly + 1] - seg_s;
     }
     int n_ent;
-    const int seg_o = wave_excl_scan_i(seg_l, lane, &n_ent);
+    const int seg_o = wave_excl_scan_i32(seg_l, &n_ent);
     if (nx <= 16 && n_ent <= 64) continue;
     auto test = [&](int t, int* slot, int* packed) -> bool {
       int sl = -1;
@@ -717,7 +742,7 @@
         for (int i = 0; i < kHistoLen; i++)
           if (i != ind1 && i != ind2 && i != ind3) nmatches -= s_hist[i];
       }
-      for (int k = tid; k < N; k += 1024) assign[k] = (s_bins[k] & losers) ? VIEO_SBP_ERASED : s_asg[k];
+      for (int k = tid; k < N; k += 1024) assign[k] = (s_bins[k] & losers) ? VIEO_SBP_ERASED : sbp_report(A, f, s_asg[k]);
       if (tid == 0) A.nmatches[f] = s_overflow ? -1 : nmatches;
       break;
     }
@@ -815,7 +840,7 @@
       }
       if (lane == 0) {
         s_state[bestIdx] = 1 | ((ny >> 16) ? 2 : 0);
-        assign[bestIdx] = q;
+        assign[bestIdx] = sbp_report(A, f, q);
       }
       nmatches++;
       if (ori) {
@@ -1012,7 +1037,7 @@
           }
         if (nm) atomicAdd(&s_nm, nm);
         __syncthreads();
-        for (int i = tid; i < Nc; i += 1024) assign[k0 + i] = s_asg[i], KB[k0 + i] = s_bins[i];
+        for (int i = tid; i < Nc; i += 1024) assign[k0 + i] = sbp_report(A, f, s_asg[i]), KB[k0 + i] = s_bins[i];
         if (ori && tid < kHistoLen && s_hist[tid]) atomicAdd(&F[tid], s_hist[tid]);
         if (tid == 0 && s_nm) atomicAdd(&F[32], s_nm);
         break;
@@ -1222,7 +1247,8 @@
   bool built;
 };
 
-static int run_search(SbpArgs& A, int n_frames, hipStream_t st, bool keep_grid, SbpGridRef* ext_grid = nullptr) {
+static int run_search(SbpArgs& A, int n_frames, hipStream_t st, bool keep_grid, SbpGridRef* ext_grid = nullptr,
+                      bool fresh_pool = false) {
   int rc;
   SbpScratch& S = g_sbp;
   if (A.n_cams < 1 || A.n_cams > kMaxCams) {
@@ -1268,7 +1294,7 @@
       hipLaunchKernelGGL(k_sbp_grid<256>, dim3(n_frames * A.n_cams), dim3(256), 0, st, A, (int*)A.cell_start, (float4*)A.cell_rec,
                          (float*)A.cell_ang);
   }
-  else if (ext_grid)
+  else if (ext_grid || fresh_pool)
     VIEO_HIP_CHECK(hipMemsetAsync(A.cursor, 0, (size_t)n_frames * 4, st));
   if (!ext_grid) {
     g_grid.valid = true, g_grid.keys = A.keys, g_grid.ur = A.uright;
@@ -1357,7 +1383,8 @@
                         const vieo_keypoint* d_keys, const float* d_uright, const uint8_t* d_desc,
                         const uint8_t* d_taken, const int32_t* d_counts, const int32_t* d_cam_first, int key_cap,
                         int img_first, int img_step, const float* h_bounds, int n_cams, float nn_ratio,
-                        int check_orientation, int32_t* d_assign, int32_t* d_nmatches, void* stream) {
+                        int check_orientation, int32_t* d_assign, int32_t* d_nmatches, void* stream,
+                        const int32_t* d_qidx = nullptr, bool fresh_pool = false) {
   const bool keep_grid = take_grid_keep();
   if (!d_queries || !d_nq || q_cap <= 0 || n_frames <= 0 || !d_keys || !d_uright || !d_desc ||
       (!d_counts && !d_cam_first) || !h_bounds || !d_assign || !d_nmatches || key_cap <= 0 ||
@@ -1368,14 +1395,14 @@
   SbpArgs A;
   memset(&A, 0, sizeof(A));
   A.mode = mode;
-  A.queries = d_queries, A.nq = d_nq, A.q_cap = q_cap;
+  A.queries = d_queries, A.nq = d_nq, A.q_cap = q_cap, A.qidx = d_qidx;
   A.keys = d_keys, A.uright = d_uright, A.desc = d_desc, A.taken = d_taken, A.counts = d_counts;
   A.key_cap = key_cap, A.img_first = img_first, A.img_step = img_step;
   A.n_cams = n_cams, A.cam_first = d_cam_first;
   if (n_cams >= 1 && n_cams <= kMaxCams) memcpy(A.bounds, h_bounds, sizeof(float) * 4 * n_cams);
   A.nn_ratio = nn_ratio, A.check_ori = check_orientation;
   A.assign = d_assign, A.nmatches = d_nmatches;
-  return run_search(A, n_frames, (hipStream_t)stream, keep_grid);
+  return run_search(A, n_frames, (hipStream_t)stream, keep_grid, nullptr, fresh_pool);
 }
 
 int vieo_search_by_projection_batch_device(int mode, const vieo_proj_query* d_queries,
@@ -1402,6 +1429,56 @@
   if (!d_cam_first) return VIEO_E_INVALID;
   return search_batch(mode, d_queries, d_nq, q_cap, n_frames, d_keys, d_uright, d_desc, d_taken, nullptr, d_cam_first,
                       key_cap, 0, 1, h_bounds, n_cams, nn_ratio, check_orientation, d_assign, d_nmatches, stream);
+}
+
+int vieo_search_by_projection_indexed_batch_device(int mode, const vieo_proj_query* d_queries, const int32_t* d_nq,
+                                                   const int32_t* d_qidx, int q_cap, int n_frames,
+                                                   const vieo_keypoint* d_keys, const float* d_uright,
+                                                   const uint8_t* d_desc, const uint8_t* d_taken, const int32_t* d_counts,
+                                                   int key_cap, int img_first, int img_step, const float* h_bounds,
+                                                   float nn_ratio, int check_orientation, int32_t* d_assign,
+                                                   int32_t* d_nmatches, void* stream) {
+  if (!d_counts) return VIEO_E_INVALID;
+  return search_batch(mode, d_queries, d_nq, q_cap, n_frames, d_keys, d_uright, d_desc, d_taken, d_counts, nullptr,
+                      key_cap, img_first, img_step, h_bounds, 1, nn_ratio, check_orientation, d_assign, d_nmatches,
+                      stream, d_qidx, true);
+}
+
+int vieo_search_by_projection_rig_indexed_batch_device(int mode, const vieo_proj_query* d_queries, const int32_t* d_nq,
+                                                       const int32_t* d_qidx, int q_cap, int n_frames,
+                                                       const vieo_keypoint* d_keys, const float* d_uright,
+                                                       const uint8_t* d_desc, const uint8_t* d_taken,
+                                                       const int32_t* d_cam_first, int key_cap, const float* h_bounds,
+                                                       int n_cams, float nn_ratio, int check_orientation,
+                                                       int32_t* d_assign, int32_t* d_nmatches, void* stream) {
+  if (!d_cam_first) return VIEO_E_INVALID;
+  return search_batch(mode, d_queries, d_nq, q_cap, n_frames, d_keys, d_uright, d_desc, d_taken, nullptr, d_cam_first,
+                      key_cap, 0, 1, h_bounds, n_cams, nn_ratio, check_orientation, d_assign, d_nmatches, stream, d_qidx,
+                      true);
+}
+
+int vieo_sbp_project_last_frame_rig_compact_batch_device(const vieo_last_frame_point* d_points, const int32_t* d_n,
+                                                         int p_cap, int n_frames, const vieo_sbp_camera* d_cams,
+                                                         const vieo_sbp_rig* d_rigs, int n_cams,
+                                                         vieo_proj_query* d_queries, int32_t* d_qidx, int32_t* d_nq,
+                                                         void* stream) {
+  if (!d_points || !d_n || p_cap <= 0 || n_frames <= 0 || !d_cams || !d_queries || !d_qidx || !d_nq || n_cams < 1 ||
+      n_cams > kMaxCams || (!d_rigs && n_cams != 1) || (long long)p_cap * n_cams > INT_MAX)
+    return VIEO_E_INVALID;
+  int rc = require_device();
+  if (rc != VIEO_OK) return rc;
+  hipLaunchKernelGGL(k_sbp_project_compact<1024>, dim3(n_frames), dim3(1024), 0, (hipStream_t)stream, d_points, d_n, p_cap,
+                     d_cams, d_rigs, n_cams, d_queries, d_qidx, d_nq);
+  VIEO_HIP_CHECK(hipGetLastError());
+  return VIEO_OK;
+}
+
+int vieo_sbp_project_last_frame_compact_batch_device(const vieo_last_frame_point* d_points, const int32_t* d_n, int p_cap,
+                                                     int n_frames, const vieo_sbp_camera* d_cams,
+                                                     vieo_proj_query* d_queries, int32_t* d_qidx, int32_t* d_nq,
+                                                     void* stream) {
+  return vieo_sbp_project_last_frame_rig_compact_batch_device(d_points, d_n, p_cap, n_frames, d_cams, nullptr, 1, d_queries,
+                                                              d_qidx, d_nq, stream);
 }
 
 static int project_host(const void* h_points, int n, const vieo_sbp_camera* h_cam, const vieo_sbp_rig* h_rig,
diff --git a/vieo_slam_amd/csrc/wave_ops.h b/vieo_slam_amd/csrc/wave_ops.h
--- a/vieo_slam_amd/csrc/wave_ops.h
+++ b/vieo_slam_amd/csrc/wave_ops.h
@@ -30,6 +30,36 @@
   v = min(v, (unsigned)VIEO_DPP(v, v, VIEO_DPP_ROW_BCAST15, 0xA));
   v = min(v, (unsigned)VIEO_DPP(v, v, VIEO_DPP_ROW_BCAST31, 0xC));
   return (unsigned)__builtin_amdgcn_readlane((int)v, 63);
+}
+
+__device__ __forceinline__ int wave_excl_scan_i32(int v, int* total) {
+  int x = v;
+  x += __builtin_amdgcn_update_dpp(0, x, 0x111, 0xF, 0xF, true);
+  x += __builtin_amdgcn_update_dpp(0, x, 0x112, 0xF, 0xF, true);
+  x += __builtin_amdgcn_update_dpp(0, x, 0x114, 0xF, 0xF, true);
+  x += __builtin_amdgcn_update_dpp(0, x, 0x118, 0xF, 0xF, true);
+  x += VIEO_DPP(0, x, VIEO_DPP_ROW_BCAST15, 0xA);
+  x += VIEO_DPP(0, x, VIEO_DPP_ROW_BCAST31, 0xC);
+  *total = __builtin_amdgcn_readlane(x, 63);
+  return x - v;
+}
+
+template <int NW>
+__device__ __forceinline__ int block_excl_scan_i32(int v, int* s_part, int* total) {
+  const int wave = __builtin_amdgcn_readfirstlane((int)(threadIdx.x >> 6));
+  int wtot;
+  int x = wave_excl_scan_i32(v, &wtot);
+  if ((threadIdx.x & 63) == 0) s_part[wave] = wtot;
+  __syncthreads();
+  int before = 0, all = 0;
+#pragma unroll
+  for (int w = 0; w < NW; w++) {
+    const int t = s_part[w];
+    if (w < wave) before += t;
+    all += t;
+  }
+  *total = all;
+  return x + before;
 }
 
 __device__ __forceinline__ double wave_sum_f64(double v) {
diff --git a/vieo_slam_amd/pipeline.py b/vieo_slam_amd/pipeline.py
--- a/vieo_slam_amd/pipeline.py
+++ b/vieo_slam_amd/pipeline.py
@@ -1,4 +1,5 @@
 import ctypes
+import os
 
 import numpy as np
 
@@ -117,6 +118,10 @@
         else:
             self.d_q1, self.d_q2 = D(B * cap * 64), D(q2.nbytes)
             self.d_q2.upload(q2)
+        self.d_qidx1, self.d_nq1 = D(B * cap * 4), D(B * 4)
+        if workload == "r3":
+            self.d_qidx2 = D(B * self.ccap * 4)
+        self.keep_grid = os.environ.get("VIEO_PIPE_KEEP_GRID", "1") != "0"
         self.d_assign, self.d_nm = D(B * cap * 4), D(B * 4)
         self.d_mpref, self.d_taken = D(B * cap * 4), D(B * cap)
         if workload == "r3":
@@ -234,12 +239,13 @@
                                                          self.d_cnt.ptr, cap, sc.BASELINE, sc.BF,
                                                          self.d_ur.ptr, self.d_dp.ptr), "stereo")
         self._stamp(2)
-        check(L.vieo_sbp_project_last_frame_batch_device(self.d_pts.ptr, self.d_npts.ptr, cap, B,
-                                                         self.d_cams.ptr, self.d_q1.ptr, st), "project")
-        check(L.vieo_search_by_projection_batch_device(0, self.d_q1.ptr, self.d_npts.ptr, cap, B,
-                                                       self.d_kp.ptr, self.d_ur.ptr, self.d_desc.ptr,
-                                                       None, self.d_cnt.ptr, cap, 0, 2, self.bounds, 0.9,
-                                                       1, self.d_assign.ptr, self.d_nm.ptr, st), "sbp1")
+        check(L.vieo_sbp_project_last_frame_compact_batch_device(self.d_pts.ptr, self.d_npts.ptr, cap, B, self.d_cams.ptr,
+                                                                 self.d_q1.ptr, self.d_qidx1.ptr, self.d_nq1.ptr, st),
+              "project")
+        check(L.vieo_search_by_projection_indexed_batch_device(0, self.d_q1.ptr, self.d_nq1.ptr, self.d_qidx1.ptr, cap, B,
+                                                               self.d_kp.ptr, self.d_ur.ptr, self.d_desc.ptr,
+                                                               None, self.d_cnt.ptr, cap, 0, 2, self.bounds, 0.9,
+                                                               1, self.d_assign.ptr, self.d_nm.ptr, st), "sbp1")
         self._stamp(3)
         check(L.vieo_track_merge_assign_batch_device(self.d_assign.ptr, self.d_mpref.ptr, self.d_cnt.ptr,
                                                      cap, B, 0, 2, 0, 1, st))
@@ -257,19 +263,22 @@
         if self.workload == "r3":
             check(L.vieo_track_mark_held_batch_device(self.d_mpref.ptr, self.d_cnt.ptr, cap, B, 0, 2, self.d_held.ptr,
                                                       self.pcap, st))
-            check(L.vieo_track_local_queries_batch_device(self.ff.ctypes.data, self.d_f1.ptr, self.d_r1.ptr, B, self.d_cpt.ptr,
-                                                          self.d_cdesc.ptr, self.d_alias.ptr, self.d_ncand.ptr, self.ccap,
-                                                          self.d_held.ptr, self.pcap, 2.0, 0.0, self.d_scale.ptr,
-                                                          self.d_q2.ptr, self.d_cdep.ptr, self.ccap, self.d_nq.ptr, st),
-                  "local queries")
-            nq, qcap, ptab = self.d_nq.ptr, self.ccap, self.pcap
+            check(L.vieo_track_local_queries_compact_batch_device(self.ff.ctypes.data, self.d_f1.ptr, self.d_r1.ptr, B,
+                                                                  self.d_cpt.ptr, self.d_cdesc.ptr, self.d_alias.ptr,
+                                                                  self.d_ncand.ptr, self.ccap, self.d_held.ptr, self.pcap,
+                                                                  2.0, 0.0, self.d_scale.ptr, self.d_q2.ptr,
+                                                                  self.d_qidx2.ptr, self.d_cdep.ptr, self.ccap,
+                                                                  self.d_nq.ptr, st), "local queries")
+            nq, qidx, qcap, ptab = self.d_nq.ptr, self.d_qidx2.ptr, self.ccap, self.pcap
         else:
-            nq, qcap, ptab = self.d_npts.ptr, cap, 2 * cap
-        check(L.vieo_search_by_projection_batch_device(1, self.d_q2.ptr, nq, qcap, B,
-                                                       self.d_kp.ptr, self.d_ur.ptr, self.d_desc.ptr,
-                                                       self.d_taken.ptr, self.d_cnt.ptr, cap, 0, 2,
-                                                       self.bounds, 0.8, 1, self.d_assign.ptr,
-                                                       self.d_nm.ptr, st), "sbp2")
+            nq, qidx, qcap, ptab = self.d_npts.ptr, None, cap, 2 * cap
+        if self.keep_grid:
+            check(L.vieo_sbp_keep_grid(1))
+        check(L.vieo_search_by_projection_indexed_batch_device(1, self.d_q2.ptr, nq, qidx, qcap, B,
+                                                               self.d_kp.ptr, self.d_ur.ptr, self.d_desc.ptr,
+                                                               self.d_taken.ptr, self.d_cnt.ptr, cap, 0, 2,
+                                                               self.bounds, 0.8, 1, self.d_assign.ptr,
+                                                               self.d_nm.ptr, st), "sbp2")
         self._stamp(5)
         check(L.vieo_track_merge_assign_batch_device(self.d_assign.ptr, self.d_mpref.ptr, self.d_cnt.ptr,
                                                      cap, B, 0, 2, cap, 0, st))
diff --git a/vieo_slam_amd/pipeline_rig_batch.py b/vieo_slam_amd/pipeline_rig_batch.py
--- a/vieo_slam_amd/pipeline_rig_batch.py
+++ b/vieo_slam_amd/pipeline_rig_batch.py
@@ -1,4 +1,5 @@
 import ctypes
+import os
 
 import numpy as np
 
@@ -44,7 +45,7 @@
         self.pcap = pcap = kc + ccap
         imgs = np.zeros((B, nc, H, W), np.uint8)
         pts = np.zeros((B, kc), LAST_FRAME_POINT_DTYPE)
-        n_last, n_q1 = np.zeros(B, np.int32), np.zeros(B, np.int32)
+        n_last = np.zeros(B, np.int32)
         xyz = np.zeros((B, pcap, 3), np.float32)
         dep = np.full((B, pcap), np.inf, np.float32)
         cpt = np.zeros((B, ccap), FRUSTUM_POINT_DTYPE)
@@ -67,7 +68,7 @@
                 imgs[b, c] = im
             n0 = pr["fr0"].N
             pts[b, :n0] = pr["pts"]
-            n_last[b], n_q1[b] = n0, n0 * nc
+            n_last[b] = n0
             has = pr["mps"]["key_mp"] >= 0
             xyz[b, :n0][has] = pr["mps"]["Xw"][pr["mps"]["key_mp"][has]]
             dep[b, :n0] = pr["last_depth"]
@@ -107,11 +108,12 @@
         self.d_depth, self.d_ur, self.d_kg = D(B * kc * 4), D(B * kc * 4), D(B * kc * 4)
         self.d_gidx, self.d_good, self.d_p3d, self.d_hdr = D(B * gcap * nc * 4), D(B * gcap), D(B * gcap * 24), D(B * 32)
         self.d_pts, self.d_cams, self.d_rigs = D(pts.nbytes), D(cams.nbytes), D(rigs.nbytes)
-        self.d_n_last, self.d_n_q1 = D(n_last.nbytes), D(n_q1.nbytes)
+        self.d_n_last = D(n_last.nbytes)
         self.d_pts.upload(pts), self.d_cams.upload(cams), self.d_rigs.upload(rigs)
-        self.d_n_last.upload(n_last), self.d_n_q1.upload(n_q1)
-        self.d_q1, self.d_q1c, self.d_qsrc, self.d_nq1 = D(B * kc * nc * 64), D(B * kc * nc * 64), D(B * kc * nc * 4), D(B * 4)
-        self.d_q2, self.d_nq2 = D(B * ccap * nc * 64), D(B * 4)
+        self.d_n_last.upload(n_last)
+        self.d_q1, self.d_qidx1, self.d_nq1 = D(B * kc * nc * 64), D(B * kc * nc * 4), D(B * 4)
+        self.d_q2, self.d_qidx2, self.d_nq2 = D(B * ccap * nc * 64), D(B * ccap * nc * 4), D(B * 4)
+        self.keep_grid = os.environ.get("VIEO_PIPE_KEEP_GRID", "1") != "0"
         self.d_assign, self.d_nm = D(B * kc * 4), D(B * 4)
         self.d_mpref, self.d_taken, self.d_held = D(B * kc * 4), D(B * kc), D(B * pcap)
         self.d_xyz, self.d_dep = D(xyz.nbytes), D(dep.nbytes)
@@ -174,17 +176,16 @@
                                                        self.d_depth.ptr, self.d_ur.ptr, self.d_kg.ptr, self.d_gidx.ptr,
                                                        self.d_good.ptr, self.d_p3d.ptr, self.d_hdr.ptr, st), "fisheye")
         self._stamp(2)
-        check(L.vieo_sbp_project_last_frame_rig_batch_device(self.d_pts.ptr, self.d_n_last.ptr, kc, B, self.d_cams.ptr,
-                                                             self.d_rigs.ptr, nc, self.d_q1.ptr, st), "project")
-        check(L.vieo_track_compact_queries_batch_device(self.d_q1.ptr, self.d_n_q1.ptr, kc * nc, B, self.d_q1c.ptr, self.d_qsrc.ptr,
-                                                        self.d_nq1.ptr, st), "compact")
-        check(L.vieo_search_by_projection_rig_batch_device(0, self.d_q1c.ptr, self.d_nq1.ptr, kc * nc, B, self.d_kcat.ptr,
-                                                           self.d_ur.ptr, self.d_dcat.ptr, None, self.d_first.ptr, kc,
-                                                           self.bounds.ctypes.data, nc, 0.9, 1, self.d_assign.ptr, self.d_nm.ptr,
-                                                           st), "sbp1")
+        check(L.vieo_sbp_project_last_frame_rig_compact_batch_device(self.d_pts.ptr, self.d_n_last.ptr, kc, B, self.d_cams.ptr,
+                                                                     self.d_rigs.ptr, nc, self.d_q1.ptr, self.d_qidx1.ptr,
+                                                                     self.d_nq1.ptr, st), "project")
+        check(L.vieo_search_by_projection_rig_indexed_batch_device(0, self.d_q1.ptr, self.d_nq1.ptr, self.d_qidx1.ptr, kc * nc, B,
+                                                                   self.d_kcat.ptr, self.d_ur.ptr, self.d_dcat.ptr, None,
+                                                                   self.d_first.ptr, kc, self.bounds.ctypes.data, nc, 0.9, 1,
+                                                                   self.d_assign.ptr, self.d_nm.ptr, st), "sbp1")
         self._stamp(3)
         check(L.vieo_track_merge_assign_rig_batch_device(self.d_assign.ptr, self.d_mpref.ptr, self.d_fcnt.ptr, kc, B, 0, 1, 0, 1, nc,
-                                                         self.d_pts.ptr, self.d_qsrc.ptr, kc * nc, st))
+                                                         self.d_pts.ptr, None, 0, st))
         check(L.vieo_track_build_obs_rig_batch_device(self.d_mpref.ptr, self.d_xyz.ptr, self.d_dep.ptr, self.close, self.pcap,
                                                       self.d_kcat.ptr, self.d_ur.ptr, self.d_fcnt.ptr, self.d_first.ptr, nc, kc, B,
                                                       self.d_consts.ptr, self.d_obs.ptr, self.d_obskey.ptr, self.d_f1.ptr, 1, st))
@@ -194,15 +195,19 @@
         check(L.vieo_track_after_pose_batch_device(self.d_mpref.ptr, self.d_obskey.ptr, self.d_outl.ptr, self.d_f1.ptr,
                                                    self.d_r1.ptr, 1, kc, B, self.d_f2.ptr, self.d_taken.ptr, st))
         check(L.vieo_track_mark_held_batch_device(self.d_mpref.ptr, self.d_fcnt.ptr, kc, B, 0, 1, self.d_held.ptr, self.pcap, st))
-        check(L.vieo_track_local_queries_batch_device(self.ff.ctypes.data, self.d_f1.ptr, self.d_r1.ptr, B, self.d_cpt.ptr,
-                                                      self.d_cdesc.ptr, self.d_alias.ptr, self.d_ncand.ptr, self.ccap,
-                                                      self.d_held.ptr, self.pcap, self.fe.th_local, 0.0, self.d_consts.ptr + 64,
-                                                      self.d_q2.ptr, self.d_dep.ptr + 4 * kc, self.pcap, self.d_nq2.ptr, st),
+        check(L.vieo_track_local_queries_compact_batch_device(self.ff.ctypes.data, self.d_f1.ptr, self.d_r1.ptr, B, self.d_cpt.ptr,
+                                                              self.d_cdesc.ptr, self.d_alias.ptr, self.d_ncand.ptr, self.ccap,
+                                                              self.d_held.ptr, self.pcap, self.fe.th_local, 0.0,
+                                                              self.d_consts.ptr + 64, self.d_q2.ptr, self.d_qidx2.ptr,
+                                                              self.d_dep.ptr + 4 * kc, self.pcap, self.d_nq2.ptr, st),
               "local queries")
-        check(L.vieo_search_by_projection_rig_batch_device(1, self.d_q2.ptr, self.d_nq2.ptr, self.ccap * nc, B, self.d_kcat.ptr,
-                                                           self.d_ur.ptr, self.d_dcat.ptr, self.d_taken.ptr, self.d_first.ptr, kc,
-                                                           self.bounds.ctypes.data, nc, self.fe.nn_local, 1, self.d_assign.ptr,
-                                                           self.d_nm.ptr, st), "sbp2")
+        if self.keep_grid:
+            check(L.vieo_sbp_keep_grid(1))
+        check(L.vieo_search_by_projection_rig_indexed_batch_device(1, self.d_q2.ptr, self.d_nq2.ptr, self.d_qidx2.ptr,
+                                                                   self.ccap * nc, B, self.d_kcat.ptr, self.d_ur.ptr,
+                                                                   self.d_dcat.ptr, self.d_taken.ptr, self.d_first.ptr, kc,
+                                                                   self.bounds.ctypes.data, nc, self.fe.nn_local, 1,
+                                                                   self.d_assign.ptr, self.d_nm.ptr, st), "sbp2")
         self._stamp(5)
         check(L.vieo_track_merge_assign_rig_batch_device(self.d_assign.ptr, self.d_mpref.ptr, self.d_fcnt.ptr, kc, B, 0, 1, kc, 0, nc,
                                                          None, None, 0, st))
```

Measured after the change: 62950, median of 4. +2.9%, better.
